# PKU-MARL/HARL

Hardware: NVIDIA B200
Metric: env-steps/sec (whole box) HAPPO update loop (higher is better)
Workload: dtype f32

## Files before the change

harl_b200/_lib.py:

```python
import ctypes as C
import os

HERE = os.path.dirname(os.path.abspath(__file__))
LIB_PATH = os.path.join(HERE, "_C", "libharl_b200.so")

HB_MAX_LAYERS = 4
HB_MAX_AGENTS = 32
HB_MAX_TENSORS = 40

ACTIVATIONS = {"relu": 0, "tanh": 1, "sigmoid": 2, "leaky_relu": 3, "selu": 4, "hardswish": 5, "identity": 6}
HEAD_DISCRETE, HEAD_BOX, HEAD_VALUE = 0, 1, 2


class NetDesc(C.Structure):
    _fields_ = [
        ("in_dim", C.c_int32), ("n_layers", C.c_int32), ("hidden", C.c_int32 * HB_MAX_LAYERS),
        ("feature_norm", C.c_int32), ("activation", C.c_int32), ("rnn_layers", C.c_int32),
        ("head", C.c_int32), ("out_dim", C.c_int32), ("std_x_coef", C.c_float), ("std_y_coef", C.c_float),
    ]


class NetLayout(C.Structure):
    _fields_ = [
        ("n_tensors", C.c_int32), ("total", C.c_int32),
        ("offset", C.c_int32 * HB_MAX_TENSORS), ("rows", C.c_int32 * HB_MAX_TENSORS),
        ("cols", C.c_int32 * HB_MAX_TENSORS), ("names", (C.c_char * 48) * HB_MAX_TENSORS),
        ("prepared_total", C.c_int32),
    ]


class InsertArgs(C.Structure):
    _fields_ = [
        ("n_envs", C.c_int32), ("n_agents", C.c_int32), ("state_type_fp", C.c_int32),
        ("actor_rnn_row", C.c_int32), ("critic_rnn_row", C.c_int32),
        ("dones", C.c_void_p), ("bad_transition", C.c_void_p),
        ("actor_masks_next", C.c_void_p * HB_MAX_AGENTS), ("actor_active_next", C.c_void_p * HB_MAX_AGENTS),
        ("actor_rnn_next", C.c_void_p * HB_MAX_AGENTS),
        ("critic_masks_next", C.c_void_p), ("critic_bad_next", C.c_void_p), ("critic_rnn_next", C.c_void_p),
        ("rewards", C.c_void_p), ("reward_stride_n", C.c_int64), ("reward_stride_a", C.c_int64),
        ("ep_return", C.c_void_p), ("done_sum", C.c_void_p),
    ]


class CollectArgs(C.Structure):
    _fields_ = [
        ("n_agents", C.c_int32), ("deterministic", C.c_int32), ("rows", C.c_int64), ("offset", C.c_uint64),
        ("actor_desc", C.POINTER(NetDesc) * HB_MAX_AGENTS), ("actor_prepared", C.c_void_p * HB_MAX_AGENTS),
        ("obs", C.c_void_p * HB_MAX_AGENTS), ("avail", C.c_void_p * HB_MAX_AGENTS),
        ("actions", C.c_void_p * HB_MAX_AGENTS), ("logp", C.c_void_p * HB_MAX_AGENTS),
        ("seed", C.c_uint64 * HB_MAX_AGENTS),
        ("critic_desc", C.POINTER(NetDesc)), ("critic_prepared", C.c_void_p), ("share_obs", C.c_void_p),
        ("critic_rows", C.c_int64), ("values", C.c_void_p), ("offset_base", C.c_void_p),
        ("actor_rnn", C.c_void_p * HB_MAX_AGENTS), ("actor_rnn_out", C.c_void_p * HB_MAX_AGENTS),
        ("actor_masks", C.c_void_p * HB_MAX_AGENTS),
        ("critic_rnn", C.c_void_p), ("critic_rnn_out", C.c_void_p), ("critic_masks", C.c_void_p),
    ]


class PPOHyper(C.Structure):
    _fields_ = [("clip_param", C.c_float), ("entropy_coef", C.c_float), ("use_policy_active_masks", C.c_int32),
                ("action_aggregation_prod", C.c_int32), ("use_clip", C.c_int32)]


class ActorBatch(C.Structure):
    _fields_ = [("obs", C.c_void_p), ("actions", C.c_void_p), ("old_logp", C.c_void_p), ("adv", C.c_void_p),
                ("factor", C.c_void_p), ("active", C.c_void_p), ("avail", C.c_void_p), ("index", C.c_void_p),
                ("rows", C.c_int64), ("rnn_states", C.c_void_p), ("masks", C.c_void_p), ("seq_len", C.c_int64)]


class ValueHyper(C.Structure):
    _fields_ = [("clip_param", C.c_float), ("huber_delta", C.c_float), ("value_loss_coef", C.c_float),
                ("use_huber_loss", C.c_int32), ("use_clipped_value_loss", C.c_int32)]


class CriticBatch(C.Structure):
    _fields_ = [("share_obs", C.c_void_p), ("value_preds", C.c_void_p), ("returns", C.c_void_p),
                ("index", C.c_void_p), ("rows", C.c_int64), ("rnn_states", C.c_void_p), ("masks", C.c_void_p),
                ("seq_len", C.c_int64)]


class AdamHyper(C.Structure):
    _fields_ = [("lr", C.c_float), ("beta1", C.c_float), ("beta2", C.c_float), ("eps", C.c_float),
                ("weight_decay", C.c_float), ("max_grad_norm", C.c_float), ("use_max_grad_norm", C.c_int32),
                ("step", C.c_int32)]


HB_MPE_MAX_AGENTS = 8


class CopySeg(C.Structure):
    _fields_ = [("dst", C.c_void_p), ("src", C.c_void_p), ("bytes", C.c_int64)]


def copy_segments(dsts, srcs, src_pinned=False, dst_pinned=False):
    n = len(dsts)
    if n == 0 or n > 16:
        return False
    segs = (CopySeg * n)()
    for i, (d, s) in enumerate(zip(dsts, srcs)):
        nbytes = d.numel() * d.element_size()
        if not ((d.is_cuda or dst_pinned or d.is_pinned()) and (s.is_cuda or src_pinned or s.is_pinned()) and (d.is_cuda or s.is_cuda)
                and d.is_contiguous() and s.is_contiguous() and d.dtype == s.dtype
                and d.numel() == s.numel() and nbytes % 4 == 0 and d.data_ptr() % 16 == 0 and s.data_ptr() % 16 == 0):
            return False
        segs[i].dst, segs[i].src, segs[i].bytes = d.data_ptr(), s.data_ptr(), nbytes
    call("hb_copy_segments", segs, n, stream_ptr())
    return True


class MpeArgs(C.Structure):
    _fields_ = [("n_envs", C.c_int32), ("n_agents", C.c_int32), ("n_landmarks", C.c_int32), ("continuous", C.c_int32),
                ("max_cycles", C.c_int32), ("reset_all", C.c_int32), ("seed", C.c_uint64),
                ("pos", C.c_void_p), ("vel", C.c_void_p), ("landmarks", C.c_void_p), ("step_count", C.c_void_p),
                ("episode", C.c_void_p), ("actions", C.c_void_p * HB_MPE_MAX_AGENTS),
                ("obs_out", C.c_void_p * HB_MPE_MAX_AGENTS), ("share_obs_out", C.c_void_p), ("rewards_out", C.c_void_p),
                ("rewards_na_out", C.c_void_p), ("dones_out", C.c_void_p), ("bad_out", C.c_void_p)]


P = C.c_void_p
SIGNATURES = {
    "hb_version": (C.c_int, []),
    "hb_last_error": (C.c_char_p, []),
    "hb_sync_check": (C.c_int, []),
    "hb_kernel_launch_count": (C.c_uint64, []),
    "hb_profile_begin": (C.c_int, [P]),
    "hb_profile_end": (C.c_int, [C.c_char_p, C.c_int]),
    "hb_set_gemm_impl": (C.c_int, [C.c_int]),
    "hb_get_gemm_impl": (C.c_int, []),
    "hb_set_fused_update": (C.c_int, [C.c_int]),
    "hb_get_fused_update": (C.c_int, []),
    "hb_fused_timing_enable": (C.c_int, [C.c_int]),
    "hb_fused_timing_read": (C.c_int, [P]),
    "hb_net_layout_of": (C.c_int, [C.POINTER(NetDesc), C.POINTER(NetLayout)]),
    "hb_net_prepare": (C.c_int, [C.POINTER(NetDesc), P, P, P]),
    "hb_workspace_bytes": (C.c_size_t, [C.POINTER(NetDesc), C.c_int64, C.c_int]),
    "hb_rollout_insert_masks": (C.c_int, [C.POINTER(InsertArgs), P]),
    "hb_rollout_collect": (C.c_int, [C.POINTER(CollectArgs), P, C.c_size_t, P]),
    "hb_counter_add": (C.c_int, [P, C.c_uint64, P]),
    "hb_policy_act": (C.c_int, [C.POINTER(NetDesc), P, P, C.c_int64, P, C.c_int, C.c_uint64, C.c_uint64, P, P, P,
                                C.c_size_t, P]),
    "hb_value_forward": (C.c_int, [C.POINTER(NetDesc), P, P, C.c_int64, P, P, C.c_size_t, P]),
    "hb_copy_segments": (C.c_int, [P, C.c_int32, P]),
    "hb_comm_create": (C.c_int, [C.c_int32, C.c_int32, C.c_size_t, C.POINTER(C.c_void_p), P]),
    "hb_comm_open_peers": (C.c_int, [P, P]),
    "hb_allreduce_bucket": (C.c_int, [P, P, C.c_int64, C.c_int32, P]),
    "hb_comm_status": (C.c_int, [P]),
    "hb_comm_destroy": (C.c_int, [P]),
    "hb_set_gae_impl": (C.c_int, [C.c_int]),
    "hb_get_gae_impl": (C.c_int, []),
    "hb_gae_returns": (C.c_int, [P, P, P, P, P, P, P, C.c_int32, C.c_int64, C.c_float, C.c_float, C.c_int, C.c_int,
                                 P, P]),
    "hb_masked_moments": (C.c_int, [P, P, C.c_int64, P, P]),
    "hb_normalize_by_moments": (C.c_int, [P, P, C.c_int64, P, P]),
    "hb_valuenorm_update": (C.c_int, [P, P, C.c_double, P]),
    "hb_valuenorm_apply": (C.c_int, [P, P, P, C.c_int64, C.c_int, P]),
    "hb_policy_evaluate": (C.c_int, [C.POINTER(NetDesc), P, C.POINTER(ActorBatch), P, P, P, C.c_int, P, C.c_size_t, P]),
    "hb_ppo_actor_grad": (C.c_int, [C.POINTER(NetDesc), P, P, C.POINTER(ActorBatch), C.POINTER(PPOHyper), P, P, P, P,
                                    C.c_size_t, P]),
    "hb_ppo_actor_grad_logp": (C.c_int, [C.POINTER(NetDesc), P, P, C.POINTER(ActorBatch), C.POINTER(PPOHyper), P, P, P, P, P,
                                         C.c_size_t, P]),
    "hb_value_grad": (C.c_int, [C.POINTER(NetDesc), P, P, C.POINTER(CriticBatch), C.POINTER(ValueHyper), P,
                                C.c_double, P, P, P, C.c_size_t, P]),
    "hb_clip_adam_step": (C.c_int, [C.POINTER(NetDesc), P, P, P, P, P, C.POINTER(AdamHyper), P, P]),
    "hb_policy_act_rnn": (C.c_int, [C.POINTER(NetDesc), P, P, C.c_int64, P, P, P, C.c_int, C.c_uint64, C.c_uint64, P, P, P,
                                    P, P, C.c_size_t, P]),
    "hb_value_forward_rnn": (C.c_int, [C.POINTER(NetDesc), P, P, C.c_int64, P, P, P, P, P, C.c_size_t, P]),
    "hb_set_trpo_jvp_impl": (C.c_int, [C.c_int]),
    "hb_get_trpo_jvp_impl": (C.c_int, []),
    "hb_set_rnn_impl": (C.c_int, [C.c_int]),
    "hb_get_rnn_impl": (C.c_int, []),
    "hb_trpo_workspace_bytes": (C.c_size_t, [C.POINTER(NetDesc), C.c_int64]),
    "hb_trpo_old_dist": (C.c_int, [C.POINTER(NetDesc), P, C.POINTER(ActorBatch), P, P, C.c_size_t, P]),
    "hb_trpo_fvp": (C.c_int, [C.POINTER(NetDesc), P, P, C.POINTER(ActorBatch), P, P, C.c_double, C.c_int, P, P,
                              C.c_size_t, P]),
    "hb_trpo_fvp_finish": (C.c_int, [C.POINTER(NetDesc), P, P, P, C.c_float, P]),
    "hb_trpo_eval": (C.c_int, [C.POINTER(NetDesc), P, C.POINTER(ActorBatch), C.POINTER(PPOHyper), P, P, P, P,
                               C.c_size_t, P]),
    "hb_trpo_cg_init": (C.c_int, [P, P, P, P, P, C.c_int, P]),
    "hb_trpo_cg_step": (C.c_int, [P, P, P, P, P, C.c_int, C.c_float, P]),
    "hb_trpo_full_step": (C.c_int, [P, P, P, C.c_float, P, P, C.c_int, P]),
    "hb_trpo_apply_step": (C.c_int, [P, P, P, C.c_float, C.c_int, P]),
    "hb_vec_scale": (C.c_int, [P, C.c_float, C.c_int, P]),
    "hb_mpe_spread_step": (C.c_int, [C.POINTER(MpeArgs), P]),
}

if not os.path.exists(LIB_PATH):
    raise ImportError(
        f"{LIB_PATH} is missing: build it with `python -m harl_b200.build` (or __graft_entry__.build()). "
        "harl_b200 has no CPU fallback.")

lib = C.CDLL(LIB_PATH)
for _name, (_res, _args) in SIGNATURES.items():
    _fn = getattr(lib, _name)
    _fn.restype = _res
    _fn.argtypes = _args

HB_ERR_UNSUPPORTED = -2
GEMM_IMPLS = {"fp32": 0, "3xtf32": 1}
if os.environ.get("HB_GEMM_IMPL"):
    lib.hb_set_gemm_impl(GEMM_IMPLS[os.environ["HB_GEMM_IMPL"]])
_NO_CHECK = {"hb_version", "hb_last_error", "hb_workspace_bytes", "hb_trpo_workspace_bytes", "hb_kernel_launch_count", "hb_profile_end", "hb_get_gemm_impl", "hb_get_rnn_impl", "hb_get_trpo_jvp_impl", "hb_get_fused_update", "hb_get_gae_impl", "hb_comm_status"}

call_count = 0


def check(rc, what=""):
    if rc == 0:
        return
    msg = lib.hb_last_error().decode(errors="replace")
    if rc == HB_ERR_UNSUPPORTED:
        raise NotImplementedError(f"harl_b200 {what}: {msg}")
    raise RuntimeError(f"harl_b200 {what} failed ({rc}): {msg}")


def call(name, *args):
    global call_count
    call_count += 1
    check(getattr(lib, name)(*args), name)


def ptr(t):
    if t is None:
        return None
    assert t.is_contiguous(), "harl_b200 kernels need contiguous tensors"
    return t.data_ptr()


def stream_ptr():
    import torch

    return torch.cuda.current_stream().cuda_stream
```

harl_b200/algorithms/actors/happo.py:

```python
import torch

from ... import _lib as L
from ... import dist
from ...common import seq_index
from ...nets import DeviceNet
from .on_policy_base import OnPolicyBase, to_device


class HAPPO(OnPolicyBase):
    use_clip = True

    def __init__(self, args, obs_space, act_space, device=torch.device("cpu")):
        super().__init__(args, obs_space, act_space, device)
        self.clip_param = args["clip_param"]
        self.ppo_epoch = args.get("ppo_epoch", args.get("a2c_epoch"))
        self.actor_num_mini_batch = args["actor_num_mini_batch"]
        self.entropy_coef = args["entropy_coef"]
        self.use_max_grad_norm = args["use_max_grad_norm"]
        self.max_grad_norm = args["max_grad_norm"]

    first_epoch_logp = True

    def _hyper(self):
        return L.PPOHyper(float(self.clip_param), float(self.entropy_coef), int(bool(self.use_policy_active_masks)),
                          int(self.action_aggregation == "prod"), int(self.use_clip))

    def _step(self, batch, norm3, scalars_row, logp_out=None):
        hooks = getattr(self, "grad_hooks", None)
        if hooks is not None:
            hooks[0]()
        self.actor.actor_grad(batch, self._hyper(), norm3, scalars_row, logp_out)
        if hooks is not None:
            hooks[1]()
        dist.all_reduce_sum_(self.actor.grad)
        self.actor.adam_step(self.cur_lr, self.opti_eps, self.weight_decay, self.max_grad_norm, self.use_max_grad_norm)

    def update(self, sample):
        (obs, _rnn, actions, _masks, active, old_lp, adv, avail, factor) = sample
        d = self.device
        obs, actions, active, old_lp, adv, factor, avail = (to_device(x, d) for x in
                                                             (obs, actions, active, old_lp, adv, factor, avail))
        rnn = mk = None
        seq_len = 0
        if self.recurrent:
            rnn = to_device(_rnn, d)
            rnn = rnn.reshape(rnn.shape[0], -1)
            mk = to_device(_masks, d).reshape(-1)
            seq_len = obs.shape[0] // rnn.shape[0]
        batch = DeviceNet.actor_batch(obs, actions, old_lp, adv.reshape(-1), factor.reshape(-1), active.reshape(-1), avail,
                                      rnn_states=rnn, masks=mk, seq_len=seq_len)
        norm3 = torch.zeros(3, dtype=torch.float64, device=d)
        norm3[2] = active.sum().double() if self.use_policy_active_masks else float(obs.shape[0])
        dist.all_reduce_sum_(norm3)
        scal = torch.zeros(4, dtype=torch.float64, device=d)
        self._step(batch, norm3, scal)
        dist.all_reduce_sum_(scal)
        s, n = scal.cpu().numpy(), norm3[2].item()
        return s[0] / n, s[1] / n, self.actor.grad_norm.item(), s[2] / s[3]

    def train(self, actor_buffer, advantages, state_type, moments=None, old_logp_out=None):
        self.old_logp_filled = False
        info = dict(policy_loss=0.0, dist_entropy=0.0, actor_grad_norm=0.0, ratio=0.0)
        d = self.device
        buf = actor_buffer
        T, N = buf.actions.shape[:2]
        rows = T * N
        adv = to_device(advantages, d).reshape(rows)
        active = buf.active_masks[:-1].reshape(rows)
        if moments is not None:
            m3, n_active = moments
        else:
            m3 = torch.zeros(3, dtype=torch.float64, device=d)
            L.call("hb_masked_moments", L.ptr(adv), L.ptr(active), rows, L.ptr(m3), L.stream_ptr())
            dist.all_reduce_sum_(m3)
            n_active = m3[2].item()
        if n_active == 0:
            return info
        if state_type == "EP":
            adv_n = torch.empty_like(adv)
            L.call("hb_normalize_by_moments", L.ptr(adv), L.ptr(adv_n), rows, L.ptr(m3), L.stream_ptr())
            adv = adv_n
        nmb = self.actor_num_mini_batch
        n_up = self.ppo_epoch * nmb
        scal = torch.zeros(n_up, 4, dtype=torch.float64, device=d)
        gnorm = torch.zeros(n_up, dtype=torch.float32, device=d)
        norms = torch.zeros(n_up, 3, dtype=torch.float64, device=d)
        fl = lambda a: a.reshape(rows, *a.shape[2:])
        obs, actions, old_lp = fl(buf.obs[:-1]), fl(buf.actions), fl(buf.action_log_probs)
        avail = None if buf.available_actions is None else fl(buf.available_actions[:-1])
        factor = None if buf.factor is None else buf.factor.reshape(rows)
        rnn = buf.rnn_states.reshape((T + 1) * N, -1) if self.recurrent else None
        masks = buf.masks.reshape((T + 1) * N) if self.recurrent else None
        mode = seq_index.mode_of(self.use_recurrent_policy, self.use_naive_recurrent_policy)
        world = dist.world_size()
        u = 0
        for _ in range(self.ppo_epoch):
            for idx, nrows, seq_len in seq_index.minibatches(T, N, nmb, mode, self.data_chunk_length, d):
                if idx is None or nrows == rows:
                    norms[u, 2] = n_active if self.use_policy_active_masks else float(rows * world)
                else:
                    if self.use_policy_active_masks:
                        norms[u, 2] = active[idx.long()].sum().double()
                    else:
                        norms[u, 2] = float(nrows)
                    dist.all_reduce_sum_(norms[u])
                batch = DeviceNet.actor_batch(obs, actions, old_lp, adv, factor, active, avail, idx, nrows,
                                              rnn_states=rnn, masks=masks, seq_len=seq_len)
                first = u == 0 and old_logp_out is not None and (idx is None) and nrows == rows
                self._step(batch, norms[u], scal[u], old_logp_out if first else None)
                self.old_logp_filled = self.old_logp_filled or first
                gnorm[u] = self.actor.grad_norm[0]
                u += 1
        dist.all_reduce_sum_(scal)
        s = scal.cpu().numpy()
        nr = norms[:, 2].cpu().numpy()
        info["policy_loss"] = float((s[:, 0] / nr).mean())
        info["dist_entropy"] = float((s[:, 1] / nr).mean())
        info["ratio"] = float((s[:, 2] / s[:, 3]).mean())
        info["actor_grad_norm"] = float(gnorm.mean().item())
        return info
```

harl_b200/algorithms/critics/v_critic.py:

```python
import torch

from ... import _lib as L
from ... import dist
from ...common import seq_index
from ...nets import DeviceNet
from ...utils.envs_tools import get_shape_from_obs_space
from ...utils.models_tools import linear_schedule_lr
from ..actors.on_policy_base import to_device


class VCritic:
    def __init__(self, args, cent_obs_space, device=torch.device("cpu")):
        self.args = args
        self.device = torch.device(device)
        self.tpdv = dict(dtype=torch.float32, device=self.device)
        self.clip_param = args["clip_param"]
        self.critic_epoch = args["critic_epoch"]
        self.critic_num_mini_batch = args["critic_num_mini_batch"]
        self.data_chunk_length = args["data_chunk_length"]
        self.value_loss_coef = args["value_loss_coef"]
        self.max_grad_norm = args["max_grad_norm"]
        self.huber_delta = args["huber_delta"]
        self.use_recurrent_policy = args["use_recurrent_policy"]
        self.use_naive_recurrent_policy = args["use_naive_recurrent_policy"]
        self.use_max_grad_norm = args["use_max_grad_norm"]
        self.use_clipped_value_loss = args["use_clipped_value_loss"]
        self.use_huber_loss = args["use_huber_loss"]
        self.use_policy_active_masks = args["use_policy_active_masks"]
        self.critic_lr = args["critic_lr"]
        self.opti_eps = args["opti_eps"]
        self.weight_decay = args["weight_decay"]
        self.share_obs_space = cent_obs_space
        shp = get_shape_from_obs_space(cent_obs_space)
        if len(shp) == 3:
            raise NotImplementedError("CNN state trunks are outside the B200 hot path")
        self.critic = DeviceNet(args, shp[0], L.HEAD_VALUE, 1, self.device)
        self.cur_lr = self.critic_lr

    def lr_decay(self, episode, episodes):
        self.cur_lr = linear_schedule_lr(episode, episodes, self.critic_lr)

    @property
    def recurrent(self):
        return bool(self.use_recurrent_policy or self.use_naive_recurrent_policy)

    def get_values(self, cent_obs, rnn_states_critic, masks, values_out=None, rnn_out=None):
        x = to_device(cent_obs, self.device)
        v = values_out if values_out is not None else torch.empty(x.shape[0], 1, **self.tpdv)
        if self.recurrent:
            rnn_in = to_device(rnn_states_critic, self.device)
            mk = to_device(masks, self.device).reshape(x.shape[0])
            rnn_new = rnn_out if rnn_out is not None else torch.empty_like(rnn_in)
            self.critic.values(x, v, rnn_in, mk, rnn_new)
            return v, rnn_new
        self.critic.values(x, v)
        rnn = rnn_states_critic if torch.is_tensor(rnn_states_critic) else to_device(rnn_states_critic, self.device)
        return v, rnn

    def _hyper(self):
        return L.ValueHyper(float(self.clip_param), float(self.huber_delta), float(self.value_loss_coef),
                            int(bool(self.use_huber_loss)), int(bool(self.use_clipped_value_loss)))

    def _step(self, share_obs, value_preds, returns, index, rows, global_rows, value_normalizer, scalars_row,
              rnn_states=None, masks=None, seq_len=0, whole=None):
        d = self.device
        if value_normalizer is not None:
            m3 = whole.get("m3") if whole is not None and index is None else None
            if m3 is None:
                m3 = torch.zeros(3, dtype=torch.float64, device=d)
                src = returns if index is None else returns[index.long()]
                L.call("hb_masked_moments", L.ptr(src.contiguous()), None, rows, L.ptr(m3), L.stream_ptr())
                dist.all_reduce_sum_(m3)
                if whole is not None and index is None:
                    whole["m3"] = m3
            value_normalizer.update_from_moments(m3)
        cb = DeviceNet.critic_batch(share_obs, value_preds, returns, index, rows, rnn_states, masks, seq_len)
        vn = value_normalizer.state if value_normalizer is not None else None
        self.critic.value_grad(cb, self._hyper(), vn, 1.0 / global_rows, scalars_row)
        if getattr(self, "after_grad_hook", None) is not None:
            self.after_grad_hook()
        dist.all_reduce_sum_(self.critic.grad)
        self.critic.adam_step(self.cur_lr, self.opti_eps, self.weight_decay, self.max_grad_norm, self.use_max_grad_norm)

    def update(self, sample, value_normalizer=None):
        share_obs, _rnn, value_preds, returns, _masks = sample
        d = self.device
        so, vp, rt = (to_device(x, d) for x in (share_obs, value_preds, returns))
        rows = so.shape[0]
        scal = torch.zeros(4, dtype=torch.float64, device=d)
        rnn = mk = None
        seq_len = 0
        if self.recurrent:
            rnn = to_device(_rnn, d)
            rnn = rnn.reshape(rnn.shape[0], -1)
            mk = to_device(_masks, d).reshape(-1)
            seq_len = rows // rnn.shape[0]
        self._step(so, vp.reshape(-1), rt.reshape(-1), None, rows, float(rows * dist.world_size()), value_normalizer, scal,
                   rnn, mk, seq_len)
        dist.all_reduce_sum_(scal)
        s = scal.cpu().numpy()
        return s[0] / s[1], self.critic.grad_norm.item()

    def train_steps(self, critic_buffer, value_normalizer=None):
        d = self.device
        buf = critic_buffer
        T = buf.episode_length
        rows = buf.value_preds[:-1].numel()
        Cn = rows // T
        so = buf.share_obs[:-1].reshape(rows, -1)
        vp = buf.value_preds[:-1].reshape(rows)
        rt = buf.returns[:-1].reshape(rows)
        rnn = buf.rnn_states_critic.reshape((T + 1) * Cn, -1) if self.recurrent else None
        masks = buf.masks.reshape((T + 1) * Cn) if self.recurrent else None
        mode = seq_index.mode_of(self.use_recurrent_policy, self.use_naive_recurrent_policy)
        nmb = self.critic_num_mini_batch
        n_up = self.critic_epoch * nmb
        scal = torch.zeros(n_up, 4, dtype=torch.float64, device=d)
        gnorm = torch.zeros(n_up, dtype=torch.float32, device=d)
        u = 0
        whole = {}
        for _ in range(self.critic_epoch):
            for idx, n, seq_len in seq_index.minibatches(T, Cn, nmb, mode, self.data_chunk_length, d):
                self._step(so, vp, rt, idx, n, float(n * dist.world_size()), value_normalizer, scal[u], rnn, masks, seq_len, whole)
                gnorm[u] = self.critic.grad_norm[0]
                u += 1
                yield u
        dist.all_reduce_sum_(scal)

        def finish():
            s = scal.cpu().numpy()
            return dict(value_loss=float((s[:, 0] / s[:, 1]).mean()), critic_grad_norm=float(gnorm.mean().item()))

        self.finish_train = finish

    def train(self, critic_buffer, value_normalizer=None, defer=False):
        for _ in self.train_steps(critic_buffer, value_normalizer):
            pass
        return self.finish_train if defer else self.finish_train()

    def prep_training(self):
        pass

    def prep_rollout(self):
        pass
```

harl_b200/csrc/capi.cu:

```cuda
#include <stdlib.h>

#include <atomic>

#include "common.cuh"
#include "kernels.cuh"
#include "rnn.cuh"
#include "trpo.cuh"

#include "fused_args.cuh"

namespace hb {

constexpr int64_t CHUNK_ROWS = (int64_t)1 << 20;

struct Work {
  float* x0;
  float* Z[HB_MAX_LAYERS];
  float* Y[HB_MAX_LAYERS];
  float* stats[HB_MAX_LAYERS];
  float* dA;
  float* dB;
  float* dwpart;
  int ptotal;
  RnnWork rnn;
// ... 148 lines not shown

static void head_base(const hb_net_desc* d, const PrepLayout& Q, const float* prep, HeadArgs* a) {
  memset(a, 0, sizeof(*a));
  a->h = Q.n[Q.n_layers - 1];
  a->out = d->out_dim;
  a->hw = prep + Q.hw;
  a->hbias = prep + Q.hbias;
  a->log_std = prep + Q.log_std;
  a->std_x = d->std_x_coef;
  a->std_y = d->std_y_coef;
}

static void head_batch(const hb_net_desc* d, const hb_actor_batch* b, int64_t c0, int64_t rows, HeadArgs* a) {
  const int ad = d->head == HB_HEAD_DISCRETE ? 1 : d->out_dim;
  const int64_t o = b->index ? 0 : c0;
  a->rows = rows;
  a->index = b->index ? b->index + c0 : nullptr;
  a->actions = b->actions ? b->actions + o * ad : nullptr;
  a->avail = b->avail ? b->avail + o * d->out_dim : nullptr;
  a->old_logp = b->old_logp ? b->old_logp + o * ad : nullptr;
  a->adv = b->adv ? b->adv + o : nullptr;
  a->factor = b->factor ? b->factor + o : nullptr;
  a->active = b->active ? b->active + o : nullptr;
}

}

extern "C" {

size_t hb_workspace_bytes(const hb_net_desc* d, int64_t rows, int mode) {
  hb::PrepLayout Q;
  hb::ParamLayout P;
  if (hb::make_layouts(d, &P, &Q, nullptr)) return 0;
  const int64_t ch = hb::chunk_of(d, rows);
  return hb::work_floats(Q, ch, mode, P.total) * sizeof(float);
}

static int policy_act_impl(const hb_net_desc* d, const float* prepared, const float* obs, int64_t rows,
                           const float* avail, const float* h_in, const float* masks, int deterministic, uint64_t seed,
                           uint64_t offset, const uint64_t* offset_base, float* actions, float* logp, float* h_out,
                           void* ws, size_t ws_bytes, void* stream) {
  using namespace hb;
  HB_CHECK_ARG(prepared && obs && actions && logp && rows >= 0, "bad argument");
  PrepLayout Q;
  int rc = check_net(d, nullptr, &Q, nullptr, 1);
  if (rc) return rc;
  HB_CHECK_ARG(!d->rnn_layers || (h_in && masks && h_out), "recurrent policy: rnn_states, masks and rnn_states_out are required");
  cudaStream_t st = (cudaStream_t)stream;
  const int64_t ch = chunk_of(d, rows);
  if (rows == 0) return HB_OK;
  if (!d->rnn_layers && fused_enabled()) {
    fz::ActArgs F;
    memset(&F, 0, sizeof(F));
    bool ok = false;
    if ((rc = fused_act_fill(&F.net[0], d, prepared, obs, avail, actions, logp, seed, rows, &ok))) return rc;
    if (ok) {
      F.n_nets = 1; F.H = d->hidden[0]; F.act = d->activation; F.deterministic = deterministic;
      F.offset = offset; F.offset_base = reinterpret_cast<const unsigned long long*>(offset_base);
      return launch_fused_act(F, st);
    }
  }
  Work w;
  if ((rc = carve(Q, ch, 0, ws, ws_bytes, &w))) return rc;
  const int ad = d->head == HB_HEAD_DISCRETE ? 1 : d->out_dim;
  for (int64_t c0 = 0; c0 < rows; c0 += ch) {
    const int64_t n = rows - c0 < ch ? rows - c0 : ch;
    SeqCtx seq = {h_in, masks, 1, h_out};
    const float* feat = nullptr;
    if ((rc = features_forward(d, Q, prepared, obs, nullptr, c0, n, d->rnn_layers ? &seq : nullptr, w, st, &feat))) return rc;
    HeadArgs a;
    head_base(d, Q, prepared, &a);
    a.feat = feat;
    a.rows = n;
    a.avail = avail ? avail + c0 * d->out_dim : nullptr;
    a.deterministic = deterministic;
    a.seed = seed;
    a.offset = offset + (uint64_t)c0 * 0x9E3779B97F4A7C15ull;
    a.offset_base = reinterpret_cast<const unsigned long long*>(offset_base);
    a.actions_out = actions + c0 * ad;
    a.logp_out = logp + c0 * ad;
    if ((rc = launch_policy_head(d->head, MODE_ACT, a, st))) return rc;
  }
  return HB_OK;
}

static int value_forward_impl(const hb_net_desc* d, const float* prepared, const float* cent_obs, int64_t rows,
                              const float* h_in, const float* masks, float* values, float* h_out, void* ws,
                              size_t ws_bytes, void* stream) {
  using namespace hb;
  HB_CHECK_ARG(prepared && cent_obs && values && rows >= 0, "bad argument");
  PrepLayout Q;
  int rc = check_net(d, nullptr, &Q, nullptr, 0);
  if (rc) return rc;
  HB_CHECK_ARG(!d->rnn_layers || (h_in && masks && h_out), "recurrent critic: rnn_states, masks and rnn_states_out are required");
  cudaStream_t st = (cudaStream_t)stream;
  if (rows == 0) return HB_OK;
  if (!d->rnn_layers && fused_enabled()) {
    fz::ActArgs F;
    memset(&F, 0, sizeof(F));
    bool ok = false;
    if ((rc = fused_act_fill(&F.net[0], d, prepared, cent_obs, nullptr, values, nullptr, 0ull, rows, &ok))) return rc;
    if (ok) {
      F.n_nets = 1; F.H = d->hidden[0]; F.act = d->activation;
      return launch_fused_act(F, st);
    }
  }
  const int64_t ch = chunk_of(d, rows);
  Work w;
  if ((rc = carve(Q, ch, 0, ws, ws_bytes, &w))) return rc;
  for (int64_t c0 = 0; c0 < rows; c0 += ch) {
    const int64_t n = rows - c0 < ch ? rows - c0 : ch;
    SeqCtx seq = {h_in, masks, 1, h_out};
    const float* feat = nullptr;
    if ((rc = features_forward(d, Q, prepared, cent_obs, nullptr, c0, n, d->rnn_layers ? &seq : nullptr, w, st, &feat))) return rc;
    ValueArgs a;
    memset(&a, 0, sizeof(a));
    a.feat = feat;
    a.h = Q.n[Q.n_layers - 1];
    a.hw = prepared + Q.hw;
    a.hbias = prepared + Q.hbias;
    a.rows = n;
    a.values_out = values + c0;
    if ((rc = launch_value_head(0, a, st))) return rc;
  }
  return HB_OK;
}

int hb_policy_act(const hb_net_desc* d, const float* prepared, const float* obs, int64_t rows, const float* avail,
                  int deterministic, uint64_t seed, uint64_t offset, float* actions, float* logp, void* ws,
                  size_t ws_bytes, void* stream) {
  return policy_act_impl(d, prepared, obs, rows, avail, nullptr, nullptr, deterministic, seed, offset, nullptr, actions,
                         logp, nullptr, ws, ws_bytes, stream);
}

int hb_policy_act_rnn(const hb_net_desc* d, const float* prepared, const float* obs, int64_t rows, const float* avail,
                      const float* rnn_states, const float* masks, int deterministic, uint64_t seed, uint64_t offset,
                      const uint64_t* offset_base, float* actions, float* logp, float* rnn_states_out, void* ws,
                      size_t ws_bytes, void* stream) {
  return policy_act_impl(d, prepared, obs, rows, avail, rnn_states, masks, deterministic, seed, offset, offset_base, actions,
                         logp, rnn_states_out, ws, ws_bytes, stream);
}

int hb_value_forward(const hb_net_desc* d, const float* prepared, const float* cent_obs, int64_t rows, float* values,
                     void* ws, size_t ws_bytes, void* stream) {
  return value_forward_impl(d, prepared, cent_obs, rows, nullptr, nullptr, values, nullptr, ws, ws_bytes, stream);
}

int hb_value_forward_rnn(const hb_net_desc* d, const float* prepared, const float* cent_obs, int64_t rows,
                         const float* rnn_states, const float* masks, float* values, float* rnn_states_out, void* ws,
                         size_t ws_bytes, void* stream) {
  return value_forward_impl(d, prepared, cent_obs, rows, rnn_states, masks, values, rnn_states_out, ws, ws_bytes, stream);
}

int hb_policy_evaluate(const hb_net_desc* d, const float* prepared, const hb_actor_batch* b, float* logp_out,
                       const float* logp_ref, float* factor_inout, int action_aggregation_prod, void* ws,
                       size_t ws_bytes, void* stream) {
  using namespace hb;
  HB_CHECK_ARG(prepared && b && b->obs && b->actions && b->rows >= 0, "bad argument");
  HB_CHECK_ARG(!factor_inout || (logp_ref && !b->index), "factor update needs logp_ref and an identity batch");
  PrepLayout Q;
  int rc = check_net(d, nullptr, &Q, nullptr, 1);
  if (rc) return rc;
  cudaStream_t st = (cudaStream_t)stream;
  const int64_t rows = b->rows;
  if (rows == 0) return HB_OK;
  if (Q.fz_ok && fused_enabled()) {
    ParamLayout P;
    if ((rc = make_layouts(d, &P, nullptr, nullptr))) return rc;
    fz::Args fa;
    memset(&fa, 0, sizeof(fa));
    fa.obs = b->obs; fa.index = b->index; fa.rows = rows;
    fa.actions = b->actions; fa.avail = b->avail;
    fa.logp_out = logp_out; fa.logp_ref = logp_ref; fa.factor_inout = factor_inout;
    fa.agg_prod = action_aggregation_prod;
    return launch_fused_update(d, Q, P, prepared, fa, 1, nullptr, st);
  }
  const int64_t ch = chunk_of(d, rows);
  Work w;
  if ((rc = carve(Q, ch, 0, ws, ws_bytes, &w))) return rc;
  const int ad = d->head == HB_HEAD_DISCRETE ? 1 : d->out_dim;
  for (int64_t c0 = 0; c0 < rows; c0 += ch) {
    const int64_t n = rows - c0 < ch ? rows - c0 : ch;
    SeqCtx seq = {b->rnn_states, b->masks, b->seq_len, nullptr};
    const float* feat = nullptr;
    if ((rc = features_forward(d, Q, prepared, b->obs, b->index, c0, n, d->rnn_layers ? &seq : nullptr, w, st, &feat))) return rc;
    HeadArgs a;
    head_base(d, Q, prepared, &a);
    head_batch(d, b, c0, n, &a);
    a.feat = feat;
    a.logp_out = logp_out ? logp_out + c0 * ad : nullptr;
    a.logp_ref = logp_ref ? logp_ref + c0 * ad : nullptr;
    a.factor_inout = factor_inout ? factor_inout + c0 : nullptr;
    a.agg_prod = action_aggregation_prod;
    if ((rc = launch_policy_head(d->head, MODE_EVAL, a, st))) return rc;
  }
  return HB_OK;
}

int hb_ppo_actor_grad(const hb_net_desc* d, const float* params, const float* prepared, const hb_actor_batch* b,
                      const hb_ppo_hyper* h, const double* norm3, float* grad, double* scalars, void* ws,
                      size_t ws_bytes, void* stream) {
  return hb_ppo_actor_grad_logp(d, params, prepared, b, h, norm3, grad, scalars, nullptr, ws, ws_bytes, stream);
}

int hb_ppo_actor_grad_logp(const hb_net_desc* d, const float* params, const float* prepared, const hb_actor_batch* b,
                           const hb_ppo_hyper* h, const double* norm3, float* grad, double* scalars, float* logp_out, void* ws,
                           size_t ws_bytes, void* stream) {
  using namespace hb;
  HB_CHECK_ARG(params && prepared && b && h && norm3 && grad && scalars, "NULL argument");
  HB_CHECK_ARG(b->obs && b->actions && b->old_logp && b->adv && b->active && b->rows >= 0, "incomplete batch");
  HB_CHECK_ARG(!logp_out || !b->index, "logp_out needs an identity batch (rows of the batch = rows of logp_out)");
  ParamLayout P;
  PrepLayout Q;
  hb_net_layout L;
  int rc = check_net(d, &P, &Q, &L, 1);
  if (rc) return rc;
  cudaStream_t st = (cudaStream_t)stream;
  if (Q.fz_ok && fused_enabled() && b->rows > 0) {
    const size_t need = (size_t)fused_max_slots() * L.total * sizeof(float);
    if (ws == nullptr || ws_bytes < need) { set_error("hb_ppo_actor_grad: workspace too small: need %zu bytes, have %zu", need, ws_bytes); return HB_ERR_WORKSPACE; }
    fz::Args fa;
    memset(&fa, 0, sizeof(fa));
    fa.obs = b->obs; fa.index = b->index; fa.rows = b->rows;
    fa.actions = b->actions; fa.avail = b->avail; fa.old_logp = b->old_logp; fa.adv = b->adv; fa.factor = b->factor; fa.active = b->active;
    fa.clip = h->clip_param; fa.entropy_coef = h->entropy_coef; fa.use_active = h->use_policy_active_masks;
    fa.use_clip = h->use_clip; fa.agg_prod = h->action_aggregation_prod;
    fa.part = (float*)ws; fa.part_stride = L.total; fa.scalars = scalars;
    fa.logp_out = logp_out;
    int slots = 0;
    if ((rc = launch_fused_update(d, Q, P, prepared, fa, 0, &slots, st))) return rc;
    return launch_fused_finish(d, P, params, grad, (const float*)ws, slots, L.total, norm3, 1.0, st);
  }
  if (logp_out && b->rows > 0) {
    rc = hb_policy_evaluate(d, prepared, b, logp_out, nullptr, nullptr, h->action_aggregation_prod, ws, ws_bytes, stream);
    if (rc) return rc;
  }
  cudaError_t ce = cudaMemsetAsync(grad, 0, (size_t)L.total * sizeof(float), st);
  if (ce != cudaSuccess) return cuda_fail(ce, "hb_ppo_actor_grad(memset)");
  const int64_t rows = b->rows;
  if (rows == 0) return HB_OK;
  const int64_t ch = chunk_of(d, rows);
  Work w;
  if ((rc = carve(Q, ch, 1, ws, ws_bytes, &w, L.total))) return rc;
  {
    ce = cudaMemsetAsync(w.dwpart, 0, (size_t)tc_dw_splits() * L.total * sizeof(float), st);
    if (ce != cudaSuccess) return cuda_fail(ce, "hb_ppo_actor_grad(memset split buffer)");
  }
  const bool rnn = d->rnn_layers != 0;
  for (int64_t c0 = 0; c0 < rows; c0 += ch) {
    const int64_t n = rows - c0 < ch ? rows - c0 : ch;
    SeqCtx seq = {b->rnn_states, b->masks, b->seq_len, nullptr};
    const float* feat = nullptr;
    if ((rc = features_forward(d, Q, prepared, b->obs, b->index, c0, n, rnn ? &seq : nullptr, w, st, &feat))) return rc;
    HeadArgs a;
    head_base(d, Q, prepared, &a);
    head_batch(d, b, c0, n, &a);
    a.feat = feat;
    a.agg_prod = h->action_aggregation_prod;
    a.clip = h->clip_param;
    a.entropy_coef = h->entropy_coef;
    a.use_active = h->use_policy_active_masks;
    a.use_clip = h->use_clip;
    a.norm3 = norm3;
    a.dfeat = w.dA;
    a.g_hw = grad + P.hw;
    a.g_hbias = grad + P.hbias;
    a.g_log_std = d->head == HB_HEAD_BOX ? grad + P.log_std : nullptr;
    a.scalars = scalars;
    a.ln_z = w.Z[Q.n_layers - 1]; a.ln_stats = w.stats[Q.n_layers - 1]; a.ln_w = prepared + Q.lnw[Q.n_layers - 1];
    a.g_ln_w = grad + P.lnw[Q.n_layers - 1]; a.g_ln_b = grad + P.lnb[Q.n_layers - 1]; a.ln_act = d->activation;
    if (rnn) {
      a.dfeat = w.rnn.dtop;
      a.ln_z = w.rnn.hs[d->rnn_layers - 1]; a.ln_stats = w.rnn.stats; a.ln_w = prepared + Q.rnn_lnw;
      a.g_ln_w = grad + P.rnn_lnw; a.g_ln_b = grad + P.rnn_lnb; a.ln_act = HB_ACT_IDENTITY;
    }
    a.part_delta = w.dwpart - grad; a.part_stride = w.ptotal;
    if ((rc = launch_policy_head(d->head, MODE_GRAD, a, st))) return rc;
    if (rnn && (rc = rnn_to_trunk_backward(d, P, Q, params, prepared, grad, n, &seq, w, st))) return rc;
    if ((rc = trunk_backward(d, P, Q, params, prepared, grad, n, w, st))) return rc;
  }
  if ((rc = launch_dw_reduce(grad, w.dwpart, L.total, st))) return rc;
  return launch_featnorm_fold(d, params, grad, st);
}

int hb_value_grad(const hb_net_desc* d, const float* params, const float* prepared, const hb_critic_batch* b,
                  const hb_value_hyper* h, const float* vn_state, double inv_count, float* grad, double* scalars,
                  void* ws, size_t ws_bytes, void* stream) {
  using namespace hb;
  HB_CHECK_ARG(params && prepared && b && h && grad && scalars, "NULL argument");
  HB_CHECK_ARG(b->share_obs && b->value_preds && b->returns && b->rows >= 0, "incomplete batch");
  ParamLayout P;
  PrepLayout Q;
  hb_net_layout L;
  int rc = check_net(d, &P, &Q, &L, 0);
  if (rc) return rc;
  cudaStream_t st = (cudaStream_t)stream;
  if (Q.fz_ok && fused_enabled() && b->rows > 0) {
    const size_t need = (size_t)fused_max_slots() * L.total * sizeof(float);
    if (ws == nullptr || ws_bytes < need) { set_error("hb_value_grad: workspace too small: need %zu bytes, have %zu", need, ws_bytes); return HB_ERR_WORKSPACE; }
    fz::Args fa;
    memset(&fa, 0, sizeof(fa));
    fa.obs = b->share_obs; fa.index = b->index; fa.rows = b->rows;
    fa.value_preds = b->value_preds; fa.returns = b->returns; fa.vn_state = vn_state;
    fa.clip = h->clip_param; fa.huber_delta = h->huber_delta; fa.vcoef = h->value_loss_coef;
    fa.use_huber = h->use_huber_loss; fa.use_clipped = h->use_clipped_value_loss;
    fa.part = (float*)ws; fa.part_stride = L.total; fa.scalars = scalars;
    int slots = 0;
    if ((rc = launch_fused_update(d, Q, P, prepared, fa, 0, &slots, st))) return rc;
    return launch_fused_finish(d, P, params, grad, (const float*)ws, slots, L.total, nullptr, inv_count, st);
  }
  cudaError_t ce = cudaMemsetAsync(grad, 0, (size_t)L.total * sizeof(float), st);
  if (ce != cudaSuccess) return cuda_fail(ce, "hb_value_grad(memset)");
  const int64_t rows = b->rows;
  if (rows == 0) return HB_OK;
  const int64_t ch = chunk_of(d, rows);
  Work w;
  if ((rc = carve(Q, ch, 1, ws, ws_bytes, &w, L.total))) return rc;
  {
    ce = cudaMemsetAsync(w.dwpart, 0, (size_t)tc_dw_splits() * L.total * sizeof(float), st);
    if (ce != cudaSuccess) return cuda_fail(ce, "hb_value_grad(memset split buffer)");
  }
  const bool rnn = d->rnn_layers != 0;
  for (int64_t c0 = 0; c0 < rows; c0 += ch) {
    const int64_t n = rows - c0 < ch ? rows - c0 : ch;
    SeqCtx seq = {b->rnn_states, b->masks, b->seq_len, nullptr};
    const float* feat = nullptr;
    if ((rc = features_forward(d, Q, prepared, b->share_obs, b->index, c0, n, rnn ? &seq : nullptr, w, st, &feat))) return rc;
    ValueArgs a;
    memset(&a, 0, sizeof(a));
    a.feat = feat;
    a.h = Q.n[Q.n_layers - 1];
    a.hw = prepared + Q.hw;
    a.hbias = prepared + Q.hbias;
    a.rows = n;
    const int64_t o = b->index ? 0 : c0;
    a.index = b->index ? b->index + c0 : nullptr;
    a.value_preds = b->value_preds + o;
    a.returns = b->returns + o;
    a.vn_state = vn_state;
    a.clip = h->clip_param;
    a.huber_delta = h->huber_delta;
    a.coef = (float)((double)h->value_loss_coef * inv_count);
    a.use_huber = h->use_huber_loss;
    a.use_clipped = h->use_clipped_value_loss;
    a.dfeat = w.dA;
    a.g_hw = grad + P.hw;
    a.g_hbias = grad + P.hbias;
    a.scalars = scalars;
    a.ln_z = w.Z[Q.n_layers - 1]; a.ln_stats = w.stats[Q.n_layers - 1]; a.ln_w = prepared + Q.lnw[Q.n_layers - 1];
    a.g_ln_w = grad + P.lnw[Q.n_layers - 1]; a.g_ln_b = grad + P.lnb[Q.n_layers - 1]; a.ln_act = d->activation;
    if (rnn) {
      a.dfeat = w.rnn.dtop;
      a.ln_z = w.rnn.hs[d->rnn_layers - 1]; a.ln_stats = w.rnn.stats; a.ln_w = prepared + Q.rnn_lnw;
      a.g_ln_w = grad + P.rnn_lnw; a.g_ln_b = grad + P.rnn_lnb; a.ln_act = HB_ACT_IDENTITY;
    }
    a.part_delta = w.dwpart - grad; a.part_stride = w.ptotal;
    if ((rc = launch_value_head(1, a, st))) return rc;
    if (rnn && (rc = rnn_to_trunk_backward(d, P, Q, params, prepared, grad, n, &seq, w, st))) return rc;
    if ((rc = trunk_backward(d, P, Q, params, prepared, grad, n, w, st))) return rc;
  }
  if ((rc = launch_dw_reduce(grad, w.dwpart, L.total, st))) return rc;
  return launch_featnorm_fold(d, params, grad, st);
}

namespace {
struct TrpoExtra { float* tprep; float* yd[2]; float* ttiles; };

size_t trpo_extra_floats(const hb::PrepLayout& Q, int64_t ch) {
  return (size_t)hb::round_up(Q.tk[0], 4) + 2 * (size_t)ch * hb::hmax_of(Q) + hb::rnn_jvp_floats(Q, ch) +
         (size_t)hb::round_up(Q.total - Q.tk[0], 4);
}

int trpo_jvp_default() {
  const char* e = getenv("HB_TRPO_JVP_IMPL");
  return e ? (atoi(e) != 0) : 1;
}
std::atomic<int> g_trpo_jvp_impl{trpo_jvp_default()};


}

size_t hb_trpo_workspace_bytes(const hb_net_desc* d, int64_t rows) {
  hb::PrepLayout Q;
  hb::ParamLayout P;
  if (hb::make_layouts(d, &P, &Q, nullptr)) return 0;
  const int64_t ch = hb::chunk_of(d, rows);
  return (hb::work_floats(Q, ch, 1, P.total) + trpo_extra_floats(Q, ch)) * sizeof(float);
}

int hb_trpo_old_dist(const hb_net_desc* d, const float* prepared, const hb_actor_batch* b, float* old_dist, void* ws,
                     size_t ws_bytes, void* stream) {
  using namespace hb;
  HB_CHECK_ARG(prepared && b && b->obs && old_dist && b->rows >= 0, "bad argument");
  PrepLayout Q;
  int rc = check_net(d, nullptr, &Q, nullptr, 1);
  if (rc) return rc;
  cudaStream_t st = (cudaStream_t)stream;
  const int64_t rows = b->rows;
  if (rows == 0) return HB_OK;
  const int64_t ch = chunk_of(d, rows);
  Work w;
  if ((rc = carve(Q, ch, 0, ws, ws_bytes, &w))) return rc;
  for (int64_t c0 = 0; c0 < rows; c0 += ch) {
    const int64_t n = rows - c0 < ch ? rows - c0 : ch;
    SeqCtx seq = {b->rnn_states, b->masks, b->seq_len, nullptr};
    const float* feat = nullptr;
    if ((rc = features_forward(d, Q, prepared, b->obs, b->index, c0, n, d->rnn_layers ? &seq : nullptr, w, st, &feat))) return rc;
    TrpoHeadArgs a;
    memset(&a, 0, sizeof(a));
    a.feat = feat;
    a.h = Q.n[Q.n_layers - 1]; a.out = d->out_dim;
    a.hw = prepared + Q.hw; a.hbias = prepared + Q.hbias; a.log_std = prepared + Q.log_std;
    a.std_x = d->std_x_coef; a.std_y = d->std_y_coef;
    a.rows = n;
    a.index = b->index ? b->index + c0 : nullptr;
    a.avail = b->avail ? b->avail + (b->index ? 0 : c0) * d->out_dim : nullptr;
    a.old_dist_out = old_dist + c0 * d->out_dim;
    if ((rc = launch_trpo_head(d->head, TR_OLD, a, st))) return rc;
  }
  return HB_OK;
}

int hb_trpo_fvp(const hb_net_desc* d, const float* params, const float* prepared, const hb_actor_batch* b,
                const float* old_dist, const float* v, double inv_rows, int reuse_forward, float* out, void* ws,
                size_t ws_bytes, void* stream) {
  using namespace hb;
  HB_CHECK_ARG(params && prepared && b && b->obs && old_dist && v && out && b->rows >= 0, "bad argument");
  ParamLayout P;
  PrepLayout Q;
  hb_net_layout L;
  int rc = check_net(d, &P, &Q, &L, 1);
  if (rc) return rc;
  cudaStream_t st = (cudaStream_t)stream;
  cudaError_t ce = cudaMemsetAsync(out, 0, (size_t)L.total * sizeof(float), st);
  if (ce != cudaSuccess) return cuda_fail(ce, "hb_trpo_fvp(memset)");
  const int64_t rows = b->rows;
  if (rows == 0) return HB_OK;
  const int64_t ch = chunk_of(d, rows);
  const bool rnn = d->rnn_layers != 0;
  const size_t base = work_floats(Q, ch, 1, L.total);
  if ((base + trpo_extra_floats(Q, ch)) * sizeof(float) > ws_bytes || ws == nullptr) {
    set_error("hb_trpo_fvp: workspace too small: need %zu bytes, have %zu", (base + trpo_extra_floats(Q, ch)) * sizeof(float), ws_bytes);
    return HB_ERR_WORKSPACE;
  }
  Work w;
  if ((rc = carve(Q, ch, 1, ws, base * sizeof(float), &w, L.total))) return rc;
  TrpoExtra x;
  x.tprep = (float*)ws + base;
  x.yd[0] = x.tprep + round_up(Q.tk[0], 4);
  x.yd[1] = x.yd[0] + (size_t)ch * hmax_of(Q);
  RnnJvpWork jw;
  carve_rnn_jvp(Q, ch, x.yd[1] + (size_t)ch * hmax_of(Q), &jw);
  x.ttiles = x.yd[1] + (size_t)ch * hmax_of(Q) + rnn_jvp_floats(Q, ch);
  const bool tc_jvp = g_trpo_jvp_impl.load(std::memory_order_relaxed) == 1 && gemm_impl() != 0;
  ce = cudaMemsetAsync(w.dwpart, 0, (size_t)tc_dw_splits() * L.total * sizeof(float), st);
// ... 183 lines not shown
```

harl_b200/csrc/fused_args.cuh:

```cuda
#pragma once
#include <cuda_fp16.h>

#include "common.cuh"

namespace hb {
namespace fz {

struct Args {
  int H, K0p, in_dim, out, act, nch0;
  const __half* img0; const __half* img1; const __half* img1b; const __half* imgh;
  const float* bias0; const float* bias1; const float* biash;
  const float* scales;
  const float* log_std; float std_x, std_y;
  const float* obs; const int32_t* index; long long rows;
  int stage_obs;
  const float* actions; const float* avail; const float* old_logp; const float* adv; const float* factor; const float* active;
  const float* value_preds; const float* returns; const float* vn_state;
  float clip, entropy_coef, huber_delta, vcoef;
  int use_active, use_clip, agg_prod, use_huber, use_clipped;
  float* part; long long part_stride;
  int pw0, pb0, pw1, pb1, phw, phb, plogstd;
  double* scalars;
  float* logp_out; const float* logp_ref; float* factor_inout;
};

constexpr int ACT_MAX_NETS = 24;
struct ActNet {
  const float* prep; const float* obs; const float* avail;
  float* out0;
  float* out1;
  unsigned long long seed;
  long long rows;
  int in_dim, out, head, K0p, nch0;
  int o_w0, o_w1, o_hw, o_b0, o_b1, o_bh, o_sc, o_ls;
  float std_x, std_y;
  int tile0, stage;
};
struct ActArgs {
  int n_nets, H, act, deterministic, K0p_max, pad_;
  unsigned long long offset;
  const unsigned long long* offset_base;
  ActNet net[ACT_MAX_NETS];
};

}

bool fused_enabled();
struct hb_collect_args;
int launch_fused_act(fz::ActArgs& A, cudaStream_t st);
int fused_act_fill(fz::ActNet* n, const hb_net_desc* d, const float* prepared, const float* obs, const float* avail, float* out0,
                   float* out1, unsigned long long seed, long long rows, bool* ok);
void set_fused_enabled(int on);
inline int fused_max_slots() { return 148; }
int launch_fused_update(const hb_net_desc* d, const PrepLayout& Q, const ParamLayout& P, const float* prepared, fz::Args a, int mode,
                        int* grid_out, cudaStream_t st);
int launch_fused_finish(const hb_net_desc* d, const ParamLayout& P, const float* params, float* grad, const float* part, int slots,
                        long long stride, const double* norm3, double host_scale, cudaStream_t st);

int fused_timing_enable(int on);
int fused_timing_read(unsigned long long* out);

}
```

harl_b200/csrc/fused_update.cu:

```cuda
#include <cuda_fp16.h>

#include <atomic>

#include "common.cuh"
#include "head_rows.cuh"
#include "kernels.cuh"
#include "row_helpers.cuh"
#include "fused_args.cuh"
#include "umma.cuh"

namespace hb {

int launch_featnorm_fold_at(const float* params, float* grad, int w0, int b0, int gw, int gb, int N, int K, cudaStream_t st);

namespace fz {

constexpr float XS = 16.f;
constexpr float DZS = 16.f;
constexpr int TILE = 128;
constexpr int NH = 16;
constexpr int MAX_STAGES = 3;
constexpr int STAGE_BYTES = 16384;
constexpr int THREADS = 320;
enum { M_GRAD = 0, M_EVAL = 1 };
// ... 39 lines not shown
  const int A_ = ACT >= 0 ? ACT : act_rt;
  switch (A_) {
    case HB_ACT_RELU: return zpos ? 1.f : 0.f;
    case HB_ACT_TANH: return 1.f - a * a;
    case HB_ACT_SIGMOID: return a * (1.f - a);
    case HB_ACT_LEAKY_RELU: return zpos ? 1.f : 0.01f;
    case HB_ACT_SELU: {
      const float al = 1.6732632423543772848170429916717f, s = 1.0507009873554804934193349852946f;
      return zpos ? s : a + s * al;
    }
    default: return 1.f;
  }
}
template <int ACT>
__device__ __forceinline__ float act_f(int act_rt, float z) {
  if (ACT >= 0) return act_fwd<(ACT >= 0 ? ACT : 0)>(z);
  return act_fwd_rt(act_rt, z);
}

struct RowPair {
  float* xch;
  int half, r, bar_id;
  __device__ __forceinline__ void put(int slot, float v) const { xch[(half * TILE + r) * 2 + slot] = v; }
  __device__ __forceinline__ void sync() const { asm volatile("bar.sync %0, 64;" ::"r"(bar_id) : "memory"); }
  __device__ __forceinline__ float total(int slot, float mine) const {
    const float other = xch[((half ^ 1) * TILE + r) * 2 + slot];
    return half == 0 ? mine + other : other + mine;
  }
};


struct NoMid { __device__ __forceinline__ void operator()() const {} };
template <int ACT, typename Mid = NoMid>
__device__ __forceinline__ void fwd_epilogue(int act_rt, uint32_t tacc, int H, const float* __restrict__ sbias, float descale,
                                             unsigned char* img, uint32_t img_bytes, int wch, const RowPair& P, float& mu, float& rstd,
                                             uint32_t (&mask)[2], Mid mid = Mid()) {
  const int r = P.r, nc = H >> 1, cb = P.half * nc;
  const float inv_n = 1.f / (float)H;
  uint32_t va[16], vb[16];
  float s0 = 0.f, s1 = 0.f, q0 = 0.f, q1 = 0.f;
  uint32_t mk0 = 0u, mk1 = 0u;
  um::tmem_ld16_issue(tacc + cb, va);
#define HB_STEP(CC, CUR, NXT)                                                                              \
  if ((CC) * 16 < nc) {                                                                                    \
    um::tmem_ld_wait16(CUR);                                                                               \
    if (((CC) + 1) * 16 < nc) um::tmem_ld16_issue(tacc + cb + ((CC) + 1) * 16, NXT);                      \
    uint32_t m_ = 0u;                                                                                      \
    _Pragma("unroll") for (int q = 0; q < 2; ++q) {                                                        \
      const float4 ba = *reinterpret_cast<const float4*>(sbias + cb + (CC) * 16 + q * 8);                  \
      const float4 bb = *reinterpret_cast<const float4*>(sbias + cb + (CC) * 16 + q * 8 + 4);              \
      const float bq[8] = {ba.x, ba.y, ba.z, ba.w, bb.x, bb.y, bb.z, bb.w};                                \
      float x[8];                                                                                          \
      _Pragma("unroll") for (int j = 0; j < 8; ++j) {                                                      \
        const float z = fmaf(__uint_as_float(CUR[q * 8 + j]), descale, bq[j]);                             \
        m_ |= z > 0.f ? (1u << (q * 8 + j)) : 0u;                                                          \
        x[j] = act_f<ACT>(act_rt, z);                                                                      \
      }                                                                                                    \
      _Pragma("unroll") for (int j = 0; j < 8; j += 2) {                                                   \
        s0 += x[j]; s1 += x[j + 1];                                                                        \
        q0 = fmaf(x[j], x[j], q0); q1 = fmaf(x[j + 1], x[j + 1], q1);                                      \
      }                                                                                                    \
      uint4 hi, lo;                                                                                        \
      um::split8(x, hi, lo);                                                                               \
      const uint32_t off = img_off(r, (cb >> 3) + (CC) * 2 + q, wch);                                      \
      *reinterpret_cast<uint4*>(img + off) = hi;                                                           \
      *reinterpret_cast<uint4*>(img + img_bytes + off) = lo;                                               \
    }                                                                                                      \
    if ((CC) < 2) mk0 |= m_ << (16 * ((CC) & 1)); else mk1 |= m_ << (16 * ((CC) & 1));                     \
  }
  HB_STEP(0, va, vb) HB_STEP(1, vb, va) HB_STEP(2, va, vb) HB_STEP(3, vb, va)
#undef HB_STEP
  mask[0] = mk0; mask[1] = mk1;
  const float ps = s0 + s1, pq = q0 + q1;
  P.put(0, ps);
  P.put(1, pq);
  P.sync();
  mu = P.total(0, ps) * inv_n;
  rstd = rsqrtf(fmaxf(P.total(1, pq) * inv_n - mu * mu, 0.f) + 1e-5f);
  const float rs = rstd * XS, sh = -mu * rstd * XS;
  for (int c8 = 0; c8 < (nc >> 3); ++c8) {
    const uint32_t off = img_off(r, (cb >> 3) + c8, wch);
    float x[8];
    um::join8(*reinterpret_cast<const uint4*>(img + off), *reinterpret_cast<const uint4*>(img + img_bytes + off), x);
#pragma unroll
    for (int j = 0; j < 8; ++j) x[j] = fmaf(x[j], rs, sh);
    uint4 hi, lo;
    um::split8(x, hi, lo);
    *reinterpret_cast<uint4*>(img + off) = hi;
    *reinterpret_cast<uint4*>(img + img_bytes + off) = lo;
    if (c8 == (nc >> 4) - 1) mid();
  }
}

template <int ACT, typename Pre>
__device__ __forceinline__ void bwd_epilogue(int act_rt, uint32_t tacc, int H, float descale, unsigned char* img,
                                             uint32_t img_bytes, int wch, const RowPair& P, float mu, float rstd,
                                             const uint32_t (&mask)[2], bool row_ok, Pre pre) {
  const int r = P.r, nc = H >> 1, cb = P.half * nc;
  const float inv_n = 1.f / (float)H;
  float s1a = 0.f, s1b = 0.f, s2a = 0.f, s2b = 0.f;
  {
    uint32_t va[16], vb[16];
    um::tmem_ld16_issue(tacc + cb, va);
#define HB_STEP(CC, CUR, NXT)                                                                              \
    if ((CC) * 16 < nc) {                                                                                  \
      um::tmem_ld_wait16(CUR);                                                                             \
      if (((CC) + 1) * 16 < nc) um::tmem_ld16_issue(tacc + cb + ((CC) + 1) * 16, NXT);                    \
      _Pragma("unroll") for (int q = 0; q < 2; ++q) {                                                      \
        const uint32_t off = img_off(r, (cb >> 3) + (CC) * 2 + q, wch);                                    \
        float x[8];                                                                                        \
        um::join8(*reinterpret_cast<const uint4*>(img + off), *reinterpret_cast<const uint4*>(img + img_bytes + off), x); \
        _Pragma("unroll") for (int j = 0; j < 8; j += 2) {                                                 \
          const float g0 = __uint_as_float(CUR[q * 8 + j]), g1 = __uint_as_float(CUR[q * 8 + j + 1]);      \
          s1a += g0; s1b += g1;                                                                            \
          s2a = fmaf(g0, x[j], s2a); s2b = fmaf(g1, x[j + 1], s2b);                                        \
        }                                                                                                  \
      }                                                                                                    \
    }
    HB_STEP(0, va, vb) HB_STEP(1, vb, va) HB_STEP(2, va, vb) HB_STEP(3, vb, va)
#undef HB_STEP
  }
  const float p1 = s1a + s1b, p2 = s2a + s2b;
  P.put(0, p1);
  P.put(1, p2);
  P.sync();
  const float m1 = P.total(0, p1) * inv_n, m2 = P.total(1, p2) * inv_n * (1.f / (XS * XS));
  const float stdx = 1.f / (rstd * XS);
  const float k = row_ok ? rstd * descale * DZS : 0.f;
  pre();
  for (int cc = 0; cc * 16 < nc; ++cc) {
    uint32_t v[16];
    um::tmem_ld16_issue(tacc + cb + cc * 16, v);
    um::tmem_ld_wait16(v);
    const uint32_t mw = (cc < 2 ? mask[0] : mask[1]) >> (16 * (cc & 1));
#pragma unroll
    for (int q = 0; q < 2; ++q) {
      const uint32_t off = img_off(r, (cb >> 3) + cc * 2 + q, wch);
      float x[8], dz[8];
      um::join8(*reinterpret_cast<const uint4*>(img + off), *reinterpret_cast<const uint4*>(img + img_bytes + off), x);
#pragma unroll
      for (int j = 0; j < 8; ++j) {
        const float a = fmaf(x[j], stdx, mu);
        const float t = fmaf(-x[j], m2, __uint_as_float(v[q * 8 + j]) - m1);
        dz[j] = k * t * act_prime<ACT>(act_rt, a, (mw >> (q * 8 + j)) & 1u);
      }
      uint4 hi, lo;
      um::split8(dz, hi, lo);
      *reinterpret_cast<uint4*>(img + off) = hi;
      *reinterpret_cast<uint4*>(img + img_bytes + off) = lo;
    }
  }
}

__device__ __forceinline__ float huber_v(float e, float d, int use_huber, float* de) {
  if (!use_huber) { *de = e; return e * e / 2.f; }
  const float ae = fabsf(e);
  if (ae <= d) { *de = e; return e * e / 2.f; }
  *de = e > 0.f ? d : -d;
  return d * (ae - d / 2.f);
}

__device__ unsigned long long g_phase_cycles[148 * 16];
__device__ int g_phase_on;
struct PhaseClock {
  unsigned long long t;
  unsigned long long* acc;
  bool on;
  __device__ __forceinline__ void start(bool enable, unsigned long long* smem_acc) {
    on = enable; acc = smem_acc;
    if (on) { for (int i = 0; i < 16; ++i) acc[i] = 0ull; t = clock64(); }
  }
  __device__ __forceinline__ void lap(int slot) {
    if (on) { const unsigned long long n = clock64(); acc[slot] += n - t; t = n; }
  }
  __device__ __forceinline__ void flush() {
    if (on) for (int i = 0; i < 16; ++i) g_phase_cycles[blockIdx.x * 16 + i] += acc[i];
  }
};

template <int HEAD, int MODE, int ACT>
__global__ void __launch_bounds__(THREADS, 1) fused_update_kernel(const __grid_constant__ Args a) {
  extern __shared__ __align__(1024) unsigned char smem[];
  const int tid = threadIdx.x, warp = tid >> 5, lane = tid & 31;
  const int H = a.H, K0p = a.K0p;
  const int wch0 = K0p >> 3, wchx = 16, wchd = NH >> 3, wchh = H >> 3;
  const uint32_t x0_bytes = TILE * K0p * 2, x_bytes = TILE * 128 * 2, dl_bytes = TILE * NH * 2, wh_bytes = NH * H * 2;
  unsigned char* p = smem;
  unsigned char* X0 = p; p += 2 * x0_bytes;
  unsigned char* X1 = p; p += 2 * x_bytes;
  unsigned char* X2 = p; p += 2 * x_bytes;
  unsigned char* DL = p; p += 2 * dl_bytes;
  unsigned char* ONES = p; p += dl_bytes;
  unsigned char* WH = p; p += 2 * wh_bytes;
  const int STAGES = K0p <= 32 ? 3 : 2;
  unsigned char* ring = p; p += STAGES * STAGE_BYTES;
  float* sb0 = reinterpret_cast<float*>(p); p += 128 * 4;
  float* sb1 = reinterpret_cast<float*>(p); p += 128 * 4;
  float* sbh = reinterpret_cast<float*>(p); p += NH * 4;
  float* sstd = reinterpret_cast<float*>(p); p += 4 * NH * 4;
  float* sacc = reinterpret_cast<float*>(p); p += 2 * NH * 4;
  double* sred = reinterpret_cast<double*>(p); p += 4 * 4 * 8;
  float* xch = reinterpret_cast<float*>(p); p += 2 * TILE * 2 * 4;
  uint64_t* bars = reinterpret_cast<uint64_t*>(p); p += 12 * 8;
  unsigned long long* sclk = reinterpret_cast<unsigned long long*>(p); p += 16 * 8;
  uint32_t* tmem_slot = reinterpret_cast<uint32_t*>(p);
  uint64_t* w_full = bars;
  uint64_t* w_empty = bars + MAX_STAGES;
  uint64_t* e2m = bars + 2 * MAX_STAGES;
  uint64_t* m2e = e2m + 1;
  uint64_t* obs_free = e2m + 2;
  uint64_t* obs_full = e2m + 3;
  uint64_t* e2m_h = e2m + 4;
  uint64_t* m2e_b = e2m + 5;
  unsigned char* OBS = MODE == M_GRAD ? X2 : X1;
  const uint32_t obs_bytes = (uint32_t)TILE * (uint32_t)a.in_dim * 4u;
  const int aw = HEAD == HB_HEAD_BOX ? a.out : 1;
  uint32_t so = obs_bytes, o_act = 0, o_old = 0, o_adv = 0, o_fac = 0, o_w = 0, o_av = 0, o_vp = 0, o_ret = 0;
  if (HEAD != HB_HEAD_VALUE) {
    o_act = so; so += TILE * aw * 4;
    if (MODE == M_GRAD) {
      o_old = so; so += TILE * aw * 4;
      o_adv = so; so += TILE * 4;
      if (a.factor) { o_fac = so; so += TILE * 4; }
      if (a.use_active) { o_w = so; so += TILE * 4; }
    }
    if (HEAD == HB_HEAD_DISCRETE && a.avail != nullptr) { o_av = so; so += TILE * a.out * 4; }
  } else if (MODE == M_GRAD) {
    o_vp = so; so += TILE * 4;
    o_ret = so; so += TILE * 4;
  }
  const uint32_t stage_bytes = so;

  const long long ntiles = (a.rows + TILE - 1) / TILE;
  const int nch1 = H >> 5;
  constexpr bool GRAD = MODE == M_GRAD;

  if (H < 128) {
    for (int i = tid; i < (int)((2 * x_bytes) / 16); i += THREADS) {
      reinterpret_cast<uint4*>(X1)[i] = make_uint4(0, 0, 0, 0);
      reinterpret_cast<uint4*>(X2)[i] = make_uint4(0, 0, 0, 0);
    }
  }
  for (int i = tid; i < TILE * 2; i += THREADS)
    reinterpret_cast<uint4*>(ONES)[i] = ((i >> 3) & 1) ? make_uint4(0, 0, 0, 0) : make_uint4(0x00003C00u, 0, 0, 0);
  for (int i = tid; i < (int)((2 * wh_bytes) / 16); i += THREADS) reinterpret_cast<uint4*>(WH)[i] = reinterpret_cast<const uint4*>(a.imgh)[i];
  for (int i = tid; i < 128; i += THREADS) { sb0[i] = i < H ? a.bias0[i] : 0.f; sb1[i] = i < H ? a.bias1[i] : 0.f; }
  if (tid < NH) {
    sbh[tid] = a.biash[tid];
    sacc[tid] = sacc[NH + tid] = 0.f;
    float sd = 1.f, ls = 0.f, dsd = 0.f;
    if (HEAD == HB_HEAD_BOX && tid < a.out) {
      const float sig = 1.f / (1.f + expf(-a.log_std[tid] / a.std_x));
      sd = sig * a.std_y;
      ls = logf(sd);
      dsd = a.std_y * sig * (1.f - sig) / a.std_x;
    }
    sstd[tid] = sd; sstd[NH + tid] = ls; sstd[2 * NH + tid] = dsd; sstd[3 * NH + tid] = 1.f / (sd * sd);
  }
  if (tid < 16) sred[tid] = 0.0;
  if (tid == 0) {
    for (int i = 0; i < STAGES; ++i) { um::mbar_init(&w_full[i], 1); um::mbar_init(&w_empty[i], 1); }
    um::mbar_init(e2m, 8);
    um::mbar_init(e2m_h, 8);
    um::mbar_init(m2e_b, 1);
    um::mbar_init(m2e, 1);
    um::mbar_init(obs_free, 1);
    um::mbar_init(obs_full, 1);
    um::fence_mbarrier_init();
  }
  if (warp == 0) um::tmem_alloc(tmem_slot, TMEM_COLS);
  um::fence_async_smem();
  um::tc_fence_before();
  __syncthreads();
  um::tc_fence_after();
  const uint32_t tmem = *tmem_slot;
  const float ws0 = a.scales[0], ws1 = a.scales[1], wsh = a.scales[2];

  if (warp == 0) {
    if (lane == 0) {
      uint32_t it = 0, tl_ = 0;
      auto staged = [&](long long t) { return a.stage_obs && t < ntiles && (t + 1) * TILE <= a.rows; };
      auto load_obs = [&](long long t) {
        um::mbar_expect_tx(obs_full, stage_bytes);
        um::tma_bulk_g2s(OBS, a.obs + t * TILE * a.in_dim, obs_bytes, obs_full);
        const long long r0 = t * TILE;
        if (o_act) um::tma_bulk_g2s(OBS + o_act, a.actions + r0 * aw, TILE * aw * 4, obs_full);
        if (o_old) um::tma_bulk_g2s(OBS + o_old, a.old_logp + r0 * aw, TILE * aw * 4, obs_full);
        if (o_adv) um::tma_bulk_g2s(OBS + o_adv, a.adv + r0, TILE * 4, obs_full);
        if (o_fac) um::tma_bulk_g2s(OBS + o_fac, a.factor + r0, TILE * 4, obs_full);
        if (o_w) um::tma_bulk_g2s(OBS + o_w, a.active + r0, TILE * 4, obs_full);
        if (o_av) um::tma_bulk_g2s(OBS + o_av, a.avail + r0 * a.out, TILE * a.out * 4, obs_full);
        if (o_vp) um::tma_bulk_g2s(OBS + o_vp, a.value_preds + r0, TILE * 4, obs_full);
        if (o_ret) um::tma_bulk_g2s(OBS + o_ret, a.returns + r0, TILE * 4, obs_full);
      };
      if (staged(blockIdx.x)) load_obs(blockIdx.x);
      for (long long t = blockIdx.x; t < ntiles; t += gridDim.x, ++tl_) {
        for (int pass = 0; pass < (GRAD ? 3 : 2); ++pass) {
          const int layer = pass == 0 ? 0 : 1;
          const int nch = layer == 0 ? a.nch0 : nch1, kp = layer == 0 ? K0p : H;
          const unsigned char* src = reinterpret_cast<const unsigned char*>(pass == 0 ? a.img0 : (pass == 1 ? a.img1 : a.img1b));
          for (int ci = 0; ci < nch; ++ci, ++it) {
            const int c = (pass == 1 && nch == 4) ? ((ci & 1) * 2 + (ci >> 1)) : ci;
            const int kc = kp - 32 * c < 32 ? kp - 32 * c : 32;
            const uint32_t bytes = 2u * (uint32_t)H * (uint32_t)kc * 2u;
            const uint32_t st = it % STAGES, use = it / STAGES;
            if (use > 0) um::mbar_wait(&w_empty[st], (use - 1) & 1);
            um::mbar_expect_tx(&w_full[st], bytes);
            um::tma_bulk_g2s(ring + st * STAGE_BYTES, src + (size_t)c * (2u * H * 32u * 2u), bytes, &w_full[st]);
          }
        }
        um::mbar_wait(obs_free, tl_ & 1);
        if (staged(t + gridDim.x)) load_obs(t + gridDim.x);
      }
    }
    __syncwarp();
  } else if (warp == 1) {
    if (lane == 0) {
      uint32_t it = 0, pe = 0, peh = 0;
      bool first = true;
      const uint32_t X0a = um::smem_u32(X0), X1a = um::smem_u32(X1), X2a = um::smem_u32(X2), DLa = um::smem_u32(DL);
      const uint32_t ONa = um::smem_u32(ONES), WHa = um::smem_u32(WH), RGa = um::smem_u32(ring);
      for (long long t = blockIdx.x; t < ntiles; t += gridDim.x) {
        auto wait_e = [&]() { um::mbar_wait(e2m, pe); pe ^= 1; um::tc_fence_after(); };
        auto wait_eh = [&]() { um::mbar_wait(e2m_h, peh); peh ^= 1; um::tc_fence_after(); };
        auto chunk = [&](int kc, auto&& body) {
          const uint32_t st = it % STAGES, use = it / STAGES;
          um::mbar_wait(&w_full[st], use & 1);
          um::tc_fence_after();
          body(RGa + st * STAGE_BYTES, (uint32_t)H * (uint32_t)kc * 2u);
          um::commit(&w_empty[st]);
          ++it;
        };
        wait_e();
        for (int c = 0; c < a.nch0; ++c) {
          const int kc = K0p - 32 * c < 32 ? K0p - 32 * c : 32;
          chunk(kc, [&](uint32_t wb, uint32_t wimg) {
            gemm3(tmem + C_F, op_kmajor(X0a, x0_bytes, wch0, 4 * c), op_kmajor(wb, wimg, kc >> 3, 0), kc >> 4,
                  um::idesc_f16(H, 0, 0), c > 0);
          });
        }
        um::commit(m2e);
        wait_eh();
        if (nch1 == 4) {
          auto l1 = [&](int c, bool acc) {
            chunk(32, [&](uint32_t wb, uint32_t wimg) {
              gemm3(tmem + C_F, op_kmajor(X1a, x_bytes, wchx, 4 * c), op_kmajor(wb, wimg, 4, 0), 2, um::idesc_f16(H, 0, 0), acc);
            });
          };
          l1(0, false); l1(2, true);
          wait_e();
          l1(1, true); l1(3, true);
        } else {
          wait_e();
          for (int c = 0; c < nch1; ++c)
            chunk(32, [&](uint32_t wb, uint32_t wimg) {
              gemm3(tmem + C_F, op_kmajor(X1a, x_bytes, wchx, 4 * c), op_kmajor(wb, wimg, 4, 0), 2, um::idesc_f16(H, 0, 0), c > 0);
            });
        }
        um::commit(m2e);
        if (!GRAD) um::commit(obs_free);
        wait_eh();
        if (H == 128) {
          auto hd = [&](int q, bool acc) {
            gemm3(tmem + C_H, op_kmajor(X2a, x_bytes, wchx, 4 * q), op_kmajor(WHa, wh_bytes, wchh, 4 * q), 2, um::idesc_f16(NH, 0, 0), acc);
          };
          hd(0, false); hd(2, true);
          wait_e();
          hd(1, true); hd(3, true);
        } else {
          wait_e();
          gemm3(tmem + C_H, op_kmajor(X2a, x_bytes, wchx, 0), op_kmajor(WHa, wh_bytes, wchh, 0), H >> 4, um::idesc_f16(NH, 0, 0), false);
        }
        um::commit(m2e);
        if (GRAD) {
          wait_e();
          gemm3(tmem + C_F, op_kmajor(DLa, dl_bytes, wchd, 0), op_mnmajor(WHa, wh_bytes, wchh, 0), 1, um::idesc_f16(H, 0, 1), false);
          um::commit(m2e);
          gemm3(tmem + C_WH, op_mnmajor(X2a, x_bytes, wchx, 0), op_mnmajor(DLa, dl_bytes, wchd, 0), TILE >> 4,
                um::idesc_f16(NH, 1, 1), !first);
          gemm3(tmem + C_BH, op_mnmajor(DLa, dl_bytes, wchd, 0), op_mnmajor(ONa, dl_bytes, wchd, 0), TILE >> 4,
                um::idesc_f16(NH, 1, 1), !first, false);
          um::commit(m2e_b);
          wait_e();
          auto dx_chunk = [&](int c) {
            chunk(32, [&](uint32_t wb, uint32_t wimg) {
              gemm3(tmem + C_F, op_kmajor(X2a, x_bytes, wchx, 4 * c), op_mnmajor(wb, wimg, H >> 3, 0), 2,
                    um::idesc_f16(H, 0, 1), c > 0);
            });
          };
          const int nres = nch1 < STAGES ? nch1 : STAGES;
          for (int c = 0; c < nres; ++c) dx_chunk(c);
          gemm3(tmem + C_B1, op_mnmajor(X2a, x_bytes, wchx, 0), op_mnmajor(ONa, dl_bytes, wchd, 0), TILE >> 4,
                um::idesc_f16(NH, 1, 1), !first, false);
          for (int c = nres; c < nch1; ++c) dx_chunk(c);
          um::commit(m2e);
          gemm3(tmem + C_W1, op_mnmajor(X2a, x_bytes, wchx, 0), op_mnmajor(X1a, x_bytes, wchx, 0), TILE >> 4,
                um::idesc_f16(H, 1, 1), !first);
          um::commit(m2e_b);
          um::commit(obs_free);
          wait_e();
          gemm3(tmem + C_W0, op_mnmajor(X1a, x_bytes, wchx, 0), op_mnmajor(X0a, x0_bytes, wch0, 0), TILE >> 4,
                um::idesc_f16(K0p, 1, 1), !first);
          gemm3(tmem + C_B0, op_mnmajor(X1a, x_bytes, wchx, 0), op_mnmajor(ONa, dl_bytes, wchd, 0), TILE >> 4,
                um::idesc_f16(NH, 1, 1), !first, false);
          um::commit(m2e);
          first = false;
        }
      }
    }
    __syncwarp();
  } else {
    const int q = warp & 3, r = q * 32 + lane, half = (warp - 2) >> 2;
    const uint32_t tl = tmem + ((uint32_t)(q * 32) << 16);
    const RowPair RP{xch, half, r, 2 + q};
    uint32_t pm = 0, po = 0;
    auto wait_m = [&]() { um::mbar_wait(m2e, pm); pm ^= 1; um::tc_fence_after(); };
    auto signal = [&]() { um::fence_async_smem(); um::tc_fence_before(); __syncwarp(); if (lane == 0) um::mbar_arrive(e2m); };
    auto mid = [&]() { um::fence_async_smem(); um::tc_fence_before(); __syncwarp(); if (lane == 0) um::mbar_arrive(e2m_h); };
    uint32_t pmb = 0;
    auto wait_mb = [&]() { um::mbar_wait(m2e_b, pmb); pmb ^= 1; um::tc_fence_after(); };
    const int na = a.out;
    float s_loss = 0.f, s_ent = 0.f, s_ratio = 0.f, s_rows = 0.f;
    float vmean = 0.f, vstd = 1.f;
    if (HEAD == HB_HEAD_VALUE && a.vn_state != nullptr) {
      const float d = fmaxf(a.vn_state[2], 1e-5f);
      const float mu = a.vn_state[0] / d, msq = a.vn_state[1] / d;
      vmean = mu;
      vstd = sqrtf(fmaxf(msq - mu * mu, 1e-2f));
    }
    bool pending = false;
    PhaseClock pc;
    pc.start(g_phase_on != 0 && tid == 64, sclk);
    for (long long t = blockIdx.x; t < ntiles; t += gridDim.x) {
      const long long row = t * TILE + r;
      const bool ok = row < a.rows;
      const bool ld = ok && half == 0;
      const long long src = ld ? (a.index ? (long long)a.index[row] : row) : 0;
      const bool st_obs = a.stage_obs && (t + 1) * TILE <= a.rows;
      if (st_obs && half == 0) { um::mbar_wait(obs_full, po); po ^= 1; }
      const float* stg = reinterpret_cast<const float*>(OBS);
      const long long si = st_obs ? r : src;
      auto in = [&](const float* g, uint32_t off) -> const float* { return st_obs ? stg + (off >> 2) : g; };
      float in_act = 0.f, in_old = 0.f, in_adv = 0.f, in_fac = 1.f, in_w = 1.f, in_vp = 0.f, in_ret = 0.f;
      float in_actv[HEAD == HB_HEAD_BOX ? 8 : 1], in_oldv[HEAD == HB_HEAD_BOX ? 8 : 1];
      unsigned in_avm = 0xffffu;
      if (HEAD == HB_HEAD_DISCRETE) {
        if (ld) {
          in_act = in(a.actions, o_act)[si];
          if (GRAD) {
            in_old = in(a.old_logp, o_old)[si]; in_adv = in(a.adv, o_adv)[si];
            if (a.factor) in_fac = in(a.factor, o_fac)[si];
            if (a.use_active) in_w = in(a.active, o_w)[si];
          }
          if (a.avail != nullptr) {
            const float* av = in(a.avail, o_av) + si * a.out;
            in_avm = 0u;
#pragma unroll
            for (int j = 0; j < NH; ++j) in_avm |= (j < a.out && av[j < a.out ? j : 0] != 0.f) ? (1u << j) : 0u;
          }
        }
      } else if (HEAD == HB_HEAD_BOX) {
#pragma unroll
        for (int j = 0; j < (HEAD == HB_HEAD_BOX ? 8 : 1); ++j) {
          in_actv[j] = (ld && j < a.out) ? in(a.actions, o_act)[si * a.out + j] : 0.f;
          in_oldv[j] = (ld && GRAD && j < a.out) ? in(a.old_logp, o_old)[si * a.out + j] : 0.f;
        }
        if (ld && GRAD) {
          in_adv = in(a.adv, o_adv)[si];
          if (a.factor) in_fac = in(a.factor, o_fac)[si];
          if (a.use_active) in_w = in(a.active, o_w)[si];
        }
      } else if (ld && GRAD) {
        in_vp = in(a.value_preds, o_vp)[si]; in_ret = in(a.returns, o_ret)[si];
      }
      (void)in_vp; (void)in_ret; (void)in_act; (void)in_old; (void)in_actv; (void)in_oldv;
      {
        const long long tn = t + gridDim.x;
        const long long rown = tn * TILE + r;
        if (!a.stage_obs && a.index == nullptr && rown < a.rows && half == 0) {
          if (!a.stage_obs) {
            const float* on = a.obs + rown * a.in_dim;
            um::prefetch_l2(on);
            um::prefetch_l2(on + a.in_dim - 1);
          }
          if (lane == 0) {
            if (HEAD == HB_HEAD_VALUE) { if (GRAD) { um::prefetch_l2(a.value_preds + rown); um::prefetch_l2(a.returns + rown); } }
            else {
              if (HEAD == HB_HEAD_DISCRETE) um::prefetch_l2(a.actions + rown);
              if (GRAD) {
                um::prefetch_l2(a.adv + rown);
                if (HEAD == HB_HEAD_DISCRETE) um::prefetch_l2(a.old_logp + rown);
                if (a.factor) um::prefetch_l2(a.factor + rown);
                if (a.use_active) um::prefetch_l2(a.active + rown);
              }
            }
          }
          if (HEAD == HB_HEAD_DISCRETE && a.avail != nullptr) um::prefetch_l2(a.avail + rown * a.out);
          if (HEAD == HB_HEAD_BOX) { um::prefetch_l2(a.actions + rown * a.out); if (GRAD) um::prefetch_l2(a.old_logp + rown * a.out); }
        }
      }
      const float* o = st_obs ? stg + r * a.in_dim : a.obs + src * a.in_dim;
      float mean = 0.f, rs = 0.f;
      if (half == 0) {
        float s = 0.f;
        for (int k0 = 0; k0 < a.in_dim; k0 += 16) {
          float x[16];
#pragma unroll
          for (int j = 0; j < 16; ++j) x[j] = (ld && k0 + j < a.in_dim) ? o[k0 + j] : 0.f;
#pragma unroll
          for (int j = 0; j < 16; ++j) s += x[j];
        }
        mean = s / (float)a.in_dim;
        float qv = 0.f;
        for (int k0 = 0; k0 < a.in_dim; k0 += 16) {
          float x[16];
#pragma unroll
          for (int j = 0; j < 16; ++j) x[j] = (ld && k0 + j < a.in_dim) ? o[k0 + j] : 0.f;
#pragma unroll
          for (int j = 0; j < 16; ++j) { const float d = x[j] - mean; qv = k0 + j < a.in_dim ? fmaf(d, d, qv) : qv; }
        }
        rs = rsqrtf(qv / (float)a.in_dim + 1e-5f);
      }
      pc.lap(0);
      if (pending) { wait_m(); pending = false; }
      pc.lap(1);
      const float rsx = rs * XS;
      if (half == 0) {
        for (int k0 = 0; k0 < K0p; k0 += 16) {
          float x[16];
#pragma unroll
          for (int j = 0; j < 16; ++j) x[j] = (ld && k0 + j < a.in_dim) ? (o[k0 + j] - mean) * rsx : 0.f;
#pragma unroll
          for (int c = 0; c < 2; ++c) {
            const float xc[8] = {x[c * 8], x[c * 8 + 1], x[c * 8 + 2], x[c * 8 + 3], x[c * 8 + 4], x[c * 8 + 5], x[c * 8 + 6], x[c * 8 + 7]};
            uint4 hi, lo;
            um::split8(xc, hi, lo);
            const uint32_t off = img_off(r, (k0 >> 3) + c, wch0);
            *reinterpret_cast<uint4*>(X0 + off) = hi;
            *reinterpret_cast<uint4*>(X0 + x0_bytes + off) = lo;
          }
        }
      }
      signal();
      pc.lap(2);
      float mu0, rstd0, mu1, rstd1;
      uint32_t mask0[2] = {0, 0}, mask1[2] = {0, 0};
      wait_m();
      pc.lap(3);
      fwd_epilogue<ACT>(a.act, tl + C_F, H, sb0, 1.f / (XS * ws0), X1, x_bytes, wchx, RP, mu0, rstd0, mask0, mid);
      signal();
      pc.lap(4);
      wait_m();
      pc.lap(5);
      fwd_epilogue<ACT>(a.act, tl + C_F, H, sb1, 1.f / (XS * ws1), X2, x_bytes, wchx, RP, mu1, rstd1, mask1, mid);
      signal();
      pc.lap(6);
      wait_m();
      pc.lap(7);
      float dl[NH];
#pragma unroll
      for (int j = 0; j < NH; ++j) dl[j] = 0.f;
      if (half == 0) {
        float hv[NH];
        um::tmem_ld16(tl + C_H, hv);
        const float hdesc = 1.f / (XS * wsh);
        if (HEAD == HB_HEAD_DISCRETE) {
          float lg[NH], lp[NH], pj[NH];
#pragma unroll
          for (int j = 0; j < NH; ++j) lg[j] = hv[j] * hdesc;
          const unsigned avm = in_avm;
          const float ent = rows::categorical<NH>(lg, sbh, na, avm, lp, pj);
          const int act = ld ? (int)in_act : 0;
          const float lpa = rows::select<NH>(lp, act);
          if (MODE == M_EVAL) {
            if (ok) {
              if (a.logp_out) a.logp_out[row] = lpa;
              if (a.factor_inout) a.factor_inout[src] = a.factor_inout[src] * expf(lpa - a.logp_ref[src]);
            }
          } else {
            const float w = in_w, fac = in_fac, adv = in_adv, old = in_old;
            const float ratio = expf(lpa - old);
            float m;
            const float dm = dmin_dratio(ratio, adv, a.clip, a.use_clip, &m);
            const float okf = ok ? 1.f : 0.f;
            if (ok && a.logp_out) a.logp_out[row] = lpa;
            const float c_lp = -fac * w * dm * ratio * okf;
            const float c_h = a.entropy_coef * w * okf;
            if (ok) { s_loss += -fac * m * w; s_ent += ent * w; s_ratio += ratio; s_rows += 1.f; }
#pragma unroll
            for (int j = 0; j < NH; ++j) {
              const bool live = j < na && ((avm >> j) & 1u);
              dl[j] = live ? c_lp * ((j == act ? 1.f : 0.f) - pj[j]) + c_h * pj[j] * (lp[j] + ent) : 0.f;
            }
          }
        } else if (HEAD == HB_HEAD_BOX) {
          float lpj[NH], dlt[NH];
          float ent_row = 0.f;
#pragma unroll
          for (int j = 0; j < NH; ++j) {
            lpj[j] = 0.f; dlt[j] = 0.f;
            if (j < na) {
              const float mean_j = fmaf(hv[j], hdesc, sbh[j]);
              dlt[j] = (j < 8 ? in_actv[HEAD == HB_HEAD_BOX ? (j < 8 ? j : 0) : 0] : 0.f) - mean_j;
              lpj[j] = -(dlt[j] * dlt[j]) * 0.5f * sstd[3 * NH + j] - sstd[NH + j] - 0.5f * HB_LOG_2PI_F;
              ent_row += 0.5f + 0.5f * HB_LOG_2PI_F + sstd[NH + j];
            }
          }
          if (MODE == M_EVAL) {
            if (ok) {
              float agg = a.agg_prod ? 1.f : 0.f;
#pragma unroll
              for (int j = 0; j < NH; ++j) {
                if (j < na) {
                  if (a.logp_out) a.logp_out[row * na + j] = lpj[j];
                  if (a.factor_inout) {
                    const float e = expf(lpj[j] - a.logp_ref[src * na + j]);
                    agg = a.agg_prod ? agg * e : agg + e;
                  }
                }
              }
              if (a.factor_inout) a.factor_inout[src] = a.factor_inout[src] * (a.agg_prod ? agg : agg / (float)na);
            }
          } else {
            const float w = in_w, fac = in_fac, adv = in_adv;
            if (ok && a.logp_out) {
#pragma unroll
              for (int j = 0; j < NH; ++j)
                if (j < na) a.logp_out[row * na + j] = lpj[j];
            }
            float e[NH];
            float ratio = a.agg_prod ? 1.f : 0.f;
#pragma unroll
            for (int j = 0; j < NH; ++j) {
              e[j] = 0.f;
              if (j < na) {
                e[j] = expf(lpj[j] - (j < 8 ? in_oldv[HEAD == HB_HEAD_BOX ? (j < 8 ? j : 0) : 0] : 0.f));
                ratio = a.agg_prod ? ratio * e[j] : ratio + e[j];
              }
            }
            if (!a.agg_prod) ratio /= (float)na;
            float m;
            const float dm = dmin_dratio(ratio, adv, a.clip, a.use_clip, &m);
            const float okf = ok ? 1.f : 0.f;
            const float c_r = -fac * w * dm * okf;
            if (ok) { s_loss += -fac * m * w; s_ent += ent_row * w; s_ratio += ratio; s_rows += 1.f; }
#pragma unroll
            for (int j = 0; j < NH; ++j) {
              if (j < na) {
                const float sd = sstd[j], ivar = sstd[3 * NH + j];
                const float c_lp = c_r * (a.agg_prod ? ratio : e[j] / (float)na);
                const float dmean = c_lp * dlt[j] * ivar;
                const float dstd = c_lp * (dlt[j] * dlt[j] * ivar / sd - 1.f / sd) - a.entropy_coef * w * okf / sd;
                dl[j] = dmean;
                if (j < 8) dl[8 + j] = dstd * sstd[2 * NH + j];
              }
            }
          }
        } else {
          const float v = fmaf(hv[0], hdesc, sbh[0]);
          if (MODE == M_EVAL) {
            if (ok && a.logp_out) a.logp_out[row] = v;
          } else {
            const float vp = in_vp;
            float ret = in_ret;
            if (a.vn_state != nullptr) ret = (ret - vmean) / vstd;
            const float dv = v - vp;
            const float dc = fminf(fmaxf(dv, -a.clip), a.clip);
            const float vclip = vp + dc;
            const bool pass = dv >= -a.clip && dv <= a.clip;
            float de_c, de_o;
            const float l_c = huber_v(ret - vclip, a.huber_delta, a.use_huber, &de_c);
            const float l_o = huber_v(ret - v, a.huber_delta, a.use_huber, &de_o);
            const float g_o = -de_o, g_c = pass ? -de_c : 0.f;
            float loss = l_o, g = g_o;
            if (a.use_clipped) {
              if (l_c > l_o) { loss = l_c; g = g_c; }
              else if (l_c == l_o) { loss = l_o; g = 0.5f * (g_o + g_c); }
            }
            g = ok ? g * a.vcoef : 0.f;
            if (ok) { s_loss += loss; s_rows += 1.f; }
            dl[0] = g;
          }
        }
      }
      if (!GRAD) continue;
      if (half == 0) {
        float x[8];
        uint4 hi, lo;
#pragma unroll
        for (int ch = 0; ch < 2; ++ch) {
#pragma unroll
          for (int j = 0; j < 8; ++j) x[j] = dl[ch * 8 + j] * DZS;
          um::split8(x, hi, lo);
          const uint32_t off = img_off(r, ch, wchd);
          *reinterpret_cast<uint4*>(DL + off) = hi;
          *reinterpret_cast<uint4*>(DL + dl_bytes + off) = lo;
// ... 62 lines not shown
        const double s = sred[r] + sred[4 + r] + sred[8 + r] + sred[12 + r];
        if (HEAD == HB_HEAD_VALUE) { if (r == 0) atomicAdd(a.scalars, s); if (r == 3) atomicAdd(a.scalars + 1, s); }
        else atomicAdd(a.scalars + r, s);
      }
    }
  }
  um::tc_fence_before();
  __syncthreads();
  if (warp == 0) um::tmem_dealloc(tmem, TMEM_COLS);
}


constexpr uint32_t ACT_TMEM_COLS = 256;

template <int ACT>
__global__ void __launch_bounds__(THREADS, 1) fused_act_kernel(const __grid_constant__ ActArgs A) {
  extern __shared__ __align__(1024) unsigned char smem[];
  const int tid = threadIdx.x, warp = tid >> 5, lane = tid & 31;
  int ni = 0;
  for (int q = 1; q < A.n_nets; ++q) if ((int)blockIdx.x >= A.net[q].tile0) ni = q;
  const ActNet& N = A.net[ni];
  const long long t = (long long)blockIdx.x - N.tile0;
  const int H = A.H, K0p = N.K0p;
  const int wch0 = K0p >> 3, wchx = 16, wchh = H >> 3;
  const uint32_t x0_bytes = TILE * A.K0p_max * 2, x_bytes = TILE * 128 * 2, wh_bytes = NH * H * 2;
  unsigned char* p = smem;
  unsigned char* X0 = p; p += 2 * x0_bytes;
  unsigned char* X1 = p; p += 2 * x_bytes;
  unsigned char* X2 = p; p += 2 * x_bytes;
  unsigned char* WH = p; p += 2 * wh_bytes;
  unsigned char* ring = p; p += 2 * STAGE_BYTES;
  float* sb0 = reinterpret_cast<float*>(p); p += 128 * 4;
  float* sb1 = reinterpret_cast<float*>(p); p += 128 * 4;
  float* sbh = reinterpret_cast<float*>(p); p += NH * 4;
  float* xch = reinterpret_cast<float*>(p); p += 2 * TILE * 2 * 4;
  uint64_t* bars = reinterpret_cast<uint64_t*>(p); p += 8 * 8;
  uint32_t* tmem_slot = reinterpret_cast<uint32_t*>(p);
  uint64_t* w_full = bars;
  uint64_t* w_empty = bars + 2;
  uint64_t* e2m = bars + 4;
  uint64_t* m2e = bars + 5;
  uint64_t* obs_full = bars + 6;
  unsigned char* OBS = X2;
  constexpr int STG = 2;
  const __half* img0 = reinterpret_cast<const __half*>(N.prep + N.o_w0);
  const __half* img1 = reinterpret_cast<const __half*>(N.prep + N.o_w1);
  const int nch1 = H >> 5;
  const bool full = (t + 1) * TILE <= N.rows;
  const bool st_obs = N.stage && full;
  const uint32_t obs_bytes = (uint32_t)TILE * (uint32_t)N.in_dim * 4u;
  const uint32_t o_av = (N.head == HB_HEAD_DISCRETE && N.avail != nullptr) ? obs_bytes : 0u;
  const uint32_t stage_bytes = obs_bytes + (o_av ? (uint32_t)TILE * N.out * 4u : 0u);

  if (H < 128) {
    for (int i = tid; i < (int)((2 * x_bytes) / 16); i += THREADS) {
      reinterpret_cast<uint4*>(X1)[i] = make_uint4(0, 0, 0, 0);
      reinterpret_cast<uint4*>(X2)[i] = make_uint4(0, 0, 0, 0);
    }
  }
  for (int i = tid; i < (int)((2 * wh_bytes) / 16); i += THREADS)
    reinterpret_cast<uint4*>(WH)[i] = reinterpret_cast<const uint4*>(N.prep + N.o_hw)[i];
  for (int i = tid; i < 128; i += THREADS) { sb0[i] = i < H ? N.prep[N.o_b0 + i] : 0.f; sb1[i] = i < H ? N.prep[N.o_b1 + i] : 0.f; }
  if (tid < NH) sbh[tid] = N.prep[N.o_bh + tid];
  if (tid == 0) {
    for (int i = 0; i < STG; ++i) { um::mbar_init(&w_full[i], 1); um::mbar_init(&w_empty[i], 1); }
    um::mbar_init(e2m, 8);
    um::mbar_init(m2e, 1);
    um::mbar_init(obs_full, 1);
    um::fence_mbarrier_init();
  }
  if (warp == 0) um::tmem_alloc(tmem_slot, ACT_TMEM_COLS);
  um::fence_async_smem();
  um::tc_fence_before();
  __syncthreads();
  um::tc_fence_after();
  const uint32_t tmem = *tmem_slot;
  const float ws0 = N.prep[N.o_sc], ws1 = N.prep[N.o_sc + 1], wsh = N.prep[N.o_sc + 2];

  if (warp == 0) {
    if (lane == 0) {
      if (st_obs) {
        um::mbar_expect_tx(obs_full, stage_bytes);
        um::tma_bulk_g2s(OBS, N.obs + t * TILE * N.in_dim, obs_bytes, obs_full);
        if (o_av) um::tma_bulk_g2s(OBS + o_av, N.avail + t * TILE * N.out, TILE * N.out * 4, obs_full);
      }
      uint32_t it = 0;
      for (int pass = 0; pass < 2; ++pass) {
        const int nch = pass == 0 ? N.nch0 : nch1, kp = pass == 0 ? K0p : H;
        const unsigned char* src = reinterpret_cast<const unsigned char*>(pass == 0 ? img0 : img1);
        for (int c = 0; c < nch; ++c, ++it) {
          const int kc = kp - 32 * c < 32 ? kp - 32 * c : 32;
          const uint32_t bytes = 2u * (uint32_t)H * (uint32_t)kc * 2u;
          const uint32_t st = it % STG, use = it / STG;
          if (use > 0) um::mbar_wait(&w_empty[st], (use - 1) & 1);
          um::mbar_expect_tx(&w_full[st], bytes);
          um::tma_bulk_g2s(ring + st * STAGE_BYTES, src + (size_t)c * (2u * H * 32u * 2u), bytes, &w_full[st]);
        }
      }
    }
    __syncwarp();
  } else if (warp == 1) {
    if (lane == 0) {
      uint32_t it = 0, pe = 0;
      const uint32_t X0a = um::smem_u32(X0), X1a = um::smem_u32(X1), X2a = um::smem_u32(X2), WHa = um::smem_u32(WH), RGa = um::smem_u32(ring);
      auto wait_e = [&]() { um::mbar_wait(e2m, pe); pe ^= 1; um::tc_fence_after(); };
      auto chunk = [&](int kc, auto&& body) {
        const uint32_t st = it % STG, use = it / STG;
        um::mbar_wait(&w_full[st], use & 1);
        um::tc_fence_after();
        body(RGa + st * STAGE_BYTES, (uint32_t)H * (uint32_t)kc * 2u);
        um::commit(&w_empty[st]);
        ++it;
      };
      wait_e();
      for (int c = 0; c < N.nch0; ++c) {
        const int kc = K0p - 32 * c < 32 ? K0p - 32 * c : 32;
        chunk(kc, [&](uint32_t wb, uint32_t wimg) {
          gemm3(tmem + C_F, op_kmajor(X0a, x0_bytes, wch0, 4 * c), op_kmajor(wb, wimg, kc >> 3, 0), kc >> 4, um::idesc_f16(H, 0, 0), c > 0);
        });
      }
      um::commit(m2e);
      wait_e();
      for (int c = 0; c < nch1; ++c)
        chunk(32, [&](uint32_t wb, uint32_t wimg) {
          gemm3(tmem + C_F, op_kmajor(X1a, x_bytes, wchx, 4 * c), op_kmajor(wb, wimg, 4, 0), 2, um::idesc_f16(H, 0, 0), c > 0);
        });
      um::commit(m2e);
      wait_e();
      gemm3(tmem + 128, op_kmajor(X2a, x_bytes, wchx, 0), op_kmajor(WHa, wh_bytes, wchh, 0), H >> 4, um::idesc_f16(NH, 0, 0), false);
      um::commit(m2e);
    }
    __syncwarp();
  } else {
    const int q = warp & 3, r = q * 32 + lane, half = (warp - 2) >> 2;
    const uint32_t tl = tmem + ((uint32_t)(q * 32) << 16);
    const RowPair RP{xch, half, r, 2 + q};
    uint32_t pm = 0;
    auto wait_m = [&]() { um::mbar_wait(m2e, pm); pm ^= 1; um::tc_fence_after(); };
    auto signal = [&]() { um::fence_async_smem(); um::tc_fence_before(); __syncwarp(); if (lane == 0) um::mbar_arrive(e2m); };
    const long long row = t * TILE + r;
    const bool ok = row < N.rows;
    const bool ld = ok && half == 0;
    const int na = N.out;
    if (st_obs && half == 0) um::mbar_wait(obs_full, 0);
    const float* stg = reinterpret_cast<const float*>(OBS);
    unsigned avm = 0xffffu;
    if (N.head == HB_HEAD_DISCRETE && N.avail != nullptr && ld) {
      const float* av = st_obs ? stg + (o_av >> 2) + r * na : N.avail + row * na;
      avm = 0u;
#pragma unroll
      for (int j = 0; j < NH; ++j) avm |= (j < na && av[j < na ? j : 0] != 0.f) ? (1u << j) : 0u;
    }
    const float* o = st_obs ? stg + r * N.in_dim : N.obs + (ok ? row : 0) * N.in_dim;
    float mean = 0.f, rs = 0.f;
    if (half == 0) {
      float s = 0.f;
      for (int k0 = 0; k0 < N.in_dim; k0 += 16) {
        float x[16];
#pragma unroll
        for (int j = 0; j < 16; ++j) x[j] = (ld && k0 + j < N.in_dim) ? o[k0 + j] : 0.f;
#pragma unroll
        for (int j = 0; j < 16; ++j) s += x[j];
      }
      mean = s / (float)N.in_dim;
      float qv = 0.f;
      for (int k0 = 0; k0 < N.in_dim; k0 += 16) {
        float x[16];
#pragma unroll
        for (int j = 0; j < 16; ++j) x[j] = (ld && k0 + j < N.in_dim) ? o[k0 + j] : 0.f;
#pragma unroll
        for (int j = 0; j < 16; ++j) { const float d = x[j] - mean; qv = k0 + j < N.in_dim ? fmaf(d, d, qv) : qv; }
      }
      rs = rsqrtf(qv / (float)N.in_dim + 1e-5f);
      const float rsx = rs * XS;
      for (int k0 = 0; k0 < K0p; k0 += 16) {
        float x[16];
#pragma unroll
        for (int j = 0; j < 16; ++j) x[j] = (ld && k0 + j < N.in_dim) ? (o[k0 + j] - mean) * rsx : 0.f;
#pragma unroll
        for (int c = 0; c < 2; ++c) {
          const float xc[8] = {x[c * 8], x[c * 8 + 1], x[c * 8 + 2], x[c * 8 + 3], x[c * 8 + 4], x[c * 8 + 5], x[c * 8 + 6], x[c * 8 + 7]};
          uint4 hi, lo;
          um::split8(xc, hi, lo);
          const uint32_t off = img_off(r, (k0 >> 3) + c, wch0);
          *reinterpret_cast<uint4*>(X0 + off) = hi;
          *reinterpret_cast<uint4*>(X0 + x0_bytes + off) = lo;
        }
      }
    }
    signal();
    float mu0, rstd0, mu1, rstd1;
    uint32_t mask0[2], mask1[2];
    wait_m();
    fwd_epilogue<ACT>(A.act, tl + C_F, H, sb0, 1.f / (XS * ws0), X1, x_bytes, wchx, RP, mu0, rstd0, mask0);
    signal();
    wait_m();
    fwd_epilogue<ACT>(A.act, tl + C_F, H, sb1, 1.f / (XS * ws1), X2, x_bytes, wchx, RP, mu1, rstd1, mask1);
    signal();
    wait_m();
    if (half == 0) {
      float hv[NH];
      um::tmem_ld16(tl + 128, hv);
      const float hdesc = 1.f / (XS * wsh);
      const unsigned long long off = A.offset + (A.offset_base ? *A.offset_base : 0ull);
      if (N.head == HB_HEAD_VALUE) {
        if (ok) N.out0[row] = fmaf(hv[0], hdesc, sbh[0]);
      } else if (N.head == HB_HEAD_DISCRETE) {
        float lg[NH], lp[NH], pj[NH];
#pragma unroll
        for (int j = 0; j < NH; ++j) lg[j] = hv[j] * hdesc;
        rows::categorical<NH>(lg, sbh, na, avm, lp, pj);
        const int pick = rows::categorical_pick<NH>(pj, na, A.deterministic != 0, A.deterministic ? 0.f : rows::row_uniform(row, N.seed, off));
        const float lpp = rows::select<NH>(lp, pick);
        if (ok) { N.out0[row] = (float)pick; N.out1[row] = lpp; }
      } else {
        const float* log_std = N.prep + N.o_ls;
#pragma unroll
        for (int j = 0; j < 8; ++j) {
          if (j < na) {
            const float mean_j = fmaf(hv[j], hdesc, sbh[j]);
            const float sig = 1.f / (1.f + expf(-log_std[j] / N.std_x));
            const float sd = sig * N.std_y, lsd = logf(sd);
            float act = mean_j;
            if (!A.deterministic) {
              const uint4 rnd = philox4x32(make_uint4((uint32_t)row, (uint32_t)((unsigned long long)row >> 32), (uint32_t)j, (uint32_t)off),
                                           make_uint2((uint32_t)N.seed, (uint32_t)(N.seed >> 32) ^ (uint32_t)(off >> 32)));
              const float u1 = u01(rnd.x), u2 = u01(rnd.y);
              act = mean_j + sd * (sqrtf(-2.f * logf(u1)) * cospif(2.f * u2));
            }
            if (ok) {
              const float dv = act - mean_j;
              N.out0[row * na + j] = act;
              N.out1[row * na + j] = -(dv * dv) / (2.f * sd * sd) - lsd - 0.5f * HB_LOG_2PI_F;
            }
          }
        }
      }
    }
  }
  um::tc_fence_before();
  __syncthreads();
  if (warp == 0) um::tmem_dealloc(tmem, ACT_TMEM_COLS);
}

struct PackJob {
  const float* W; const float* gamma; const float* beta; const float* b;
  int N, K, Nimg, Kp, KC, RC;
  __half* img; float* bias_out; float* scale_out;
  int cta0, ctas;
};
struct PackJobs { PackJob j[4]; int n; };

__global__ void __launch_bounds__(256) fused_pack_kernel(PackJobs jobs) {
  __shared__ float smax[8];
  __shared__ float sscale;
  int ji = 0;
  for (int q = 1; q < jobs.n; ++q) if ((int)blockIdx.x >= jobs.j[q].cta0) ji = q;
  const PackJob& J = jobs.j[ji];
  const int cta = blockIdx.x - J.cta0;
  const float* __restrict__ W = J.W;
  const float* __restrict__ gamma = J.gamma;
  const int N = J.N, K = J.K, Nimg = J.Nimg, Kp = J.Kp, KC = J.KC, RC = J.RC;
  __half* __restrict__ img = J.img;
  float mx = 0.f;
  for (int i = threadIdx.x; i < N * K; i += 256) mx = fmaxf(mx, fabsf(W[i] * (gamma ? gamma[i % K] : 1.f)));
  mx = warp_max(mx);
  if ((threadIdx.x & 31) == 0) smax[threadIdx.x >> 5] = mx;
  __syncthreads();
  if (threadIdx.x == 0) {
    float m = 0.f;
    for (int i = 0; i < 8; ++i) m = fmaxf(m, smax[i]);
    int ex = 0;
    if (m > 0.f) frexpf(m, &ex);
    ex = ex < -20 ? -20 : (ex > 20 ? 20 : ex);
    sscale = m > 0.f ? exp2f((float)(8 - ex)) : 1.f;
    if (cta == 0 && J.scale_out != nullptr) *J.scale_out = sscale;
  }
  __syncthreads();
  const float sc = sscale;
  const int total = Nimg * Kp;
  for (int i = cta * 256 + threadIdx.x; i < total; i += J.ctas * 256) {
    const int n = i / Kp, k = i % Kp;
    const float v = (n < N && k < K) ? W[n * K + k] * (gamma ? gamma[k] : 1.f) * sc : 0.f;
    const __half hi = __float2half_rn(v);
    const __half lo = __float2half_rn(v - __half2float(hi));
    if (RC > 0) {
      const int c = n / RC, nl = n % RC;
      const size_t chunk0 = (size_t)c * (2u * RC * Kp);
      const size_t e = (size_t)((nl >> 3) * (Kp >> 3) + (k >> 3)) * 64 + (nl & 7) * 8 + (k & 7);
      img[chunk0 + e] = hi;
      img[chunk0 + (size_t)RC * Kp + e] = lo;
      continue;
    }
    const int c = k / KC, kl = k % KC;
    const int kc = Kp - KC * c < KC ? Kp - KC * c : KC;
    const size_t chunk0 = (size_t)c * (2u * Nimg * KC);
    const size_t e = (size_t)((n >> 3) * (kc >> 3) + (kl >> 3)) * 64 + (n & 7) * 8 + (kl & 7);
    img[chunk0 + e] = hi;
    img[chunk0 + (size_t)Nimg * kc + e] = lo;
  }
  if (J.bias_out != nullptr) {
    const int warp = threadIdx.x >> 5, lane = threadIdx.x & 31;
    for (int n = cta * 8 + warp; n < Nimg; n += J.ctas * 8) {
      float v = 0.f;
      if (n < N && J.beta)
        for (int k = lane; k < K; k += 32) v += W[n * K + k] * J.beta[k];
      for (int o = 16; o > 0; o >>= 1) v += __shfl_xor_sync(0xffffffffu, v, o);
      if (lane == 0) J.bias_out[n] = n < N ? J.b[n] + v : 0.f;
    }
  }
}

struct Regions { int n; int off[8]; int len[8]; float scale[8]; };
constexpr int SR_GROUPS = 8, SR_MAXPER = 16;
__global__ void __launch_bounds__(32 * SR_GROUPS, 6) fused_slot_reduce_kernel(float* __restrict__ grad, const float* __restrict__ part, int slots,
                                                                           long long stride, int total, const __grid_constant__ Regions R,
                                                                           const double* __restrict__ norm3, double host_scale) {
  __shared__ float sm[SR_GROUPS][32];
  const int lane = threadIdx.x & 31, g = threadIdx.x >> 5;
  const int i = blockIdx.x * 32 + lane;
  const int per = (slots + SR_GROUPS - 1) / SR_GROUPS;
  const int s0 = g * per, s1 = s0 + per < slots ? s0 + per : slots;
  float acc = 0.f;
  if (i < total) {
    for (int sb = s0; sb < s1; sb += SR_MAXPER) {
      float v[SR_MAXPER];
#pragma unroll
      for (int u = 0; u < SR_MAXPER; ++u) v[u] = sb + u < s1 ? part[(long long)(sb + u) * stride + i] : 0.f;
#pragma unroll
      for (int u = 0; u < SR_MAXPER; ++u) acc += v[u];
    }
  }
  sm[g][lane] = acc;
  __syncthreads();
  if (g != 0 || i >= total) return;
  float sc = 0.f;
  bool in = false;
  for (int q = 0; q < R.n; ++q)
    if (i >= R.off[q] && i < R.off[q] + R.len[q]) { sc = R.scale[q]; in = true; }
  if (!in) { grad[i] = 0.f; return; }
  float t = 0.f;
#pragma unroll
  for (int q = 0; q < SR_GROUPS; ++q) t += sm[q][lane];
  const double nrm = host_scale * (norm3 ? 1.0 / norm3[2] : 1.0);
  grad[i] = (float)((double)t * (double)sc * nrm);
}

struct Folds { int n; int w[3], b[3], gw[3], gb[3], N[3], K[3], col0[3]; };
__global__ void __launch_bounds__(128) fused_unfold_kernel(const float* __restrict__ params, float* __restrict__ grad, Folds F, int cols) {
  const int warp = (blockIdx.x * blockDim.x + threadIdx.x) >> 5, lane = threadIdx.x & 31;
  if (warp >= cols) return;
  int f = 0;
  for (int q = 1; q < F.n; ++q) if (warp >= F.col0[q]) f = q;
  const int k = warp - F.col0[f], N = F.N[f], K = F.K[f];
  const float gam = params[F.gw[f] + k], bet = params[F.gb[f] + k];
  double dg = 0.0, dbt = 0.0;
  for (int n = lane; n < N; n += 32) {
    const float w = params[F.w[f] + n * K + k];
    const float G = grad[F.w[f] + n * K + k];
    const float gb = grad[F.b[f] + n];
    dg += (double)w * (double)G;
    dbt += (double)w * (double)gb;
    grad[F.w[f] + n * K + k] = fmaf(gam, G, bet * gb);
  }
  dg = warp_sum_d(dg);
  dbt = warp_sum_d(dbt);
  if (lane == 0) { grad[F.gw[f] + k] = (float)dg; grad[F.gb[f] + k] = (float)dbt; }
}

static std::atomic<int> g_enabled{-1};

}

int fused_timing_enable(int on) {
  static const unsigned long long zeros[148 * 16] = {0};
  cudaError_t e = cudaMemcpyToSymbol(fz::g_phase_cycles, zeros, sizeof(zeros));
  if (e == cudaSuccess) e = cudaMemcpyToSymbol(fz::g_phase_on, &on, sizeof(int));
  return e == cudaSuccess ? HB_OK : cuda_fail(e, "fused_timing_enable");
}
int fused_timing_read(unsigned long long* out) {
  cudaError_t e = cudaDeviceSynchronize();
  if (e == cudaSuccess) e = cudaMemcpyFromSymbol(out, fz::g_phase_cycles, sizeof(unsigned long long) * 148 * 16);
  return e == cudaSuccess ? HB_OK : cuda_fail(e, "fused_timing_read");
}

bool fused_enabled() {
  int v = fz::g_enabled.load(std::memory_order_relaxed);
  if (v < 0) {
    const char* e = getenv("HB_FUSED");
    v = (e != nullptr && atoi(e) == 0) ? 0 : 1;
    fz::g_enabled.store(v);
  }
  return v != 0 && gemm_impl() != 0;
}
void set_fused_enabled(int v) { fz::g_enabled.store(v ? 1 : 0); }

bool fused_shape_ok(const hb_net_desc* d) {
  if (d->rnn_layers != 0 || d->n_layers != 2 || d->hidden[0] != d->hidden[1]) return false;
  const int H = d->hidden[0];
  if (H != 32 && H != 64 && H != 128) return false;
  if (!d->feature_norm || d->in_dim < 1 || d->in_dim > 64) return false;
  if (d->activation == HB_ACT_HARDSWISH) return false;
  if (d->out_dim < 1 || d->out_dim > (d->head == HB_HEAD_BOX ? 8 : fz::NH)) return false;
  return true;
}

int launch_fused_pack(const hb_net_desc* d, const ParamLayout& P, const PrepLayout& Q, const float* params, float* prepared,
                      cudaStream_t st) {
  const int H = d->hidden[0];
  float* sc = prepared + Q.fz_scale;
  fz::PackJobs jobs;
  memset(&jobs, 0, sizeof(jobs));
  int cta = 0;
  auto add = [&](const float* W, const float* g, const float* be, const float* b, int N, int K, int Nimg, int Kp, int KC, int RC,
                 float* img, float* bias_out, float* scale_out, int ctas) {
    fz::PackJob& J = jobs.j[jobs.n++];
    J.W = W; J.gamma = g; J.beta = be; J.b = b; J.N = N; J.K = K; J.Nimg = Nimg; J.Kp = Kp; J.KC = KC; J.RC = RC;
    J.img = reinterpret_cast<__half*>(img); J.bias_out = bias_out; J.scale_out = scale_out; J.cta0 = cta; J.ctas = ctas;
    cta += ctas;
  };
  add(params + P.w[0], params + P.fn_w, params + P.fn_b, params + P.b[0], H, d->in_dim, H, Q.fz_k0p, 32, 0, prepared + Q.fz_w[0],
      prepared + Q.fz_bias[0], sc + 0, 8);
  add(params + P.w[1], params + P.lnw[0], params + P.lnb[0], params + P.b[1], H, H, H, H, 32, 0, prepared + Q.fz_w[1],
      prepared + Q.fz_bias[1], sc + 1, 16);
  add(params + P.w[1], params + P.lnw[0], params + P.lnb[0], params + P.b[1], H, H, H, H, 32, 32, prepared + Q.fz_w1b, nullptr, nullptr, 16);
  add(params + P.hw, params + P.lnw[1], params + P.lnb[1], params + P.hbias, d->out_dim, H, fz::NH, H, H, 0, prepared + Q.fz_hw,
      prepared + Q.fz_hbias, sc + 2, 4);
  fz::fused_pack_kernel<<<cta, 256, 0, st>>>(jobs);
  HB_LAUNCH_DONE(st, "fused_pack");
  return HB_OK;
}


int fused_act_fill(fz::ActNet* n, const hb_net_desc* d, const float* prepared, const float* obs, const float* avail, float* out0,
                   float* out1, unsigned long long seed, long long rows, bool* ok) {
  PrepLayout Q;
  int rc = make_layouts(d, nullptr, &Q, nullptr);
  if (rc) return rc;
  *ok = Q.fz_ok != 0 && (d->head != HB_HEAD_BOX || d->out_dim <= 8);
  if (!*ok) return HB_OK;
  n->prep = prepared; n->obs = obs; n->avail = avail; n->out0 = out0; n->out1 = out1; n->seed = seed; n->rows = rows;
  n->in_dim = d->in_dim; n->out = d->out_dim; n->head = d->head; n->K0p = Q.fz_k0p; n->nch0 = Q.fz_chunks[0];
  n->o_w0 = Q.fz_w[0]; n->o_w1 = Q.fz_w[1]; n->o_hw = Q.fz_hw; n->o_b0 = Q.fz_bias[0]; n->o_b1 = Q.fz_bias[1]; n->o_bh = Q.fz_hbias;
  n->o_sc = Q.fz_scale; n->o_ls = Q.log_std; n->std_x = d->std_x_coef; n->std_y = d->std_y_coef;
  const uintptr_t bits = reinterpret_cast<uintptr_t>(obs) | reinterpret_cast<uintptr_t>(avail);
  n->stage = (bits & 15) == 0 ? 1 : 0;
  return HB_OK;
}

int launch_fused_act(fz::ActArgs& A, cudaStream_t st) {
  int tiles = 0, k0 = 16;
  for (int i = 0; i < A.n_nets; ++i) {
    A.net[i].tile0 = tiles;
    tiles += (int)((A.net[i].rows + fz::TILE - 1) / fz::TILE);
    k0 = A.net[i].K0p > k0 ? A.net[i].K0p : k0;
  }
  A.K0p_max = k0;
  if (tiles == 0) return HB_OK;
  const size_t smem = 2 * (size_t)fz::TILE * k0 * 2 + 2 * 2 * (size_t)fz::TILE * 128 * 2 + 2 * (size_t)fz::NH * A.H * 2 + 2 * fz::STAGE_BYTES +
                      2 * 128 * 4 + fz::NH * 4 + 2 * fz::TILE * 2 * 4 + 8 * 8 + 16 + 1024;
#define HB_FZA(ACTV)                                                                                  \
  {                                                                                                   \
    auto kern = fz::fused_act_kernel<ACTV>;                                                           \
    cudaFuncSetAttribute(kern, cudaFuncAttributeMaxDynamicSharedMemorySize, (int)smem);               \
    kern<<<tiles, fz::THREADS, smem, st>>>(A);                                                        \
  }
  if (A.act == HB_ACT_RELU) HB_FZA(HB_ACT_RELU)
  else if (A.act == HB_ACT_TANH) HB_FZA(HB_ACT_TANH)
  else HB_FZA(-1)
#undef HB_FZA
  HB_LAUNCH_DONE(st, "fused_act");
  return HB_OK;
}

size_t fused_smem_bytes(int H, int K0p) {
  size_t b = 2 * (size_t)fz::TILE * K0p * 2 + 2 * 2 * (size_t)fz::TILE * 128 * 2 + 3 * (size_t)fz::TILE * fz::NH * 2 +
             2 * (size_t)fz::NH * H * 2 + (size_t)(K0p <= 32 ? 3 : 2) * fz::STAGE_BYTES;
  b += 2 * 128 * 4 + fz::NH * 4 + 4 * fz::NH * 4 + 2 * fz::NH * 4 + 16 * 8 + 2 * fz::TILE * 2 * 4 + 10 * 8 + 16 * 8 + 16;
  return b + 1024;
}

template <int HEAD, int MODE>
static int launch_fused_act(const fz::Args& a, int grid, size_t smem, cudaStream_t st) {
#define HB_FZ(ACTV)                                                                                   \
  {                                                                                                   \
    auto kern = fz::fused_update_kernel<HEAD, MODE, ACTV>;                                            \
    cudaFuncSetAttribute(kern, cudaFuncAttributeMaxDynamicSharedMemorySize, (int)smem);               \
    kern<<<grid, fz::THREADS, smem, st>>>(a);                                                         \
  }
  if (a.act == HB_ACT_RELU) HB_FZ(HB_ACT_RELU)
  else if (a.act == HB_ACT_TANH) HB_FZ(HB_ACT_TANH)
  else HB_FZ(-1)
#undef HB_FZ
  return HB_OK;
}

int launch_fused_update(const hb_net_desc* d, const PrepLayout& Q, const ParamLayout& P, const float* prepared, fz::Args a, int mode,
                        int* grid_out, cudaStream_t st) {
  const int H = d->hidden[0];
  a.H = H; a.K0p = Q.fz_k0p; a.in_dim = d->in_dim; a.out = d->out_dim; a.act = d->activation; a.nch0 = Q.fz_chunks[0];
  a.img0 = reinterpret_cast<const __half*>(prepared + Q.fz_w[0]);
  a.img1 = reinterpret_cast<const __half*>(prepared + Q.fz_w[1]);
  a.img1b = reinterpret_cast<const __half*>(prepared + Q.fz_w1b);
  a.imgh = reinterpret_cast<const __half*>(prepared + Q.fz_hw);
  a.bias0 = prepared + Q.fz_bias[0]; a.bias1 = prepared + Q.fz_bias[1]; a.biash = prepared + Q.fz_hbias;
  a.scales = prepared + Q.fz_scale;
  a.log_std = prepared + Q.log_std; a.std_x = d->std_x_coef; a.std_y = d->std_y_coef;
  a.pw0 = P.w[0]; a.pb0 = P.b[0]; a.pw1 = P.w[1]; a.pb1 = P.b[1]; a.phw = P.hw; a.phb = P.hbias; a.plogstd = P.log_std;
  {
    const void* ptrs[] = {a.obs, a.actions, a.old_logp, a.adv, a.factor, a.active, a.avail, a.value_preds, a.returns};
    uintptr_t bits = 0;
    for (const void* q : ptrs) bits |= reinterpret_cast<uintptr_t>(q);
    a.stage_obs = (a.index == nullptr && (bits & 15) == 0) ? 1 : 0;
  }
  const long long ntiles = (a.rows + fz::TILE - 1) / fz::TILE;
  const int grid = (int)(ntiles < 148 ? ntiles : 148);
  if (grid_out) *grid_out = grid;
  const size_t smem = fused_smem_bytes(H, Q.fz_k0p);
  int rc;
  if (d->head == HB_HEAD_DISCRETE) rc = mode == 0 ? launch_fused_act<HB_HEAD_DISCRETE, fz::M_GRAD>(a, grid, smem, st) : launch_fused_act<HB_HEAD_DISCRETE, fz::M_EVAL>(a, grid, smem, st);
  else if (d->head == HB_HEAD_BOX) rc = mode == 0 ? launch_fused_act<HB_HEAD_BOX, fz::M_GRAD>(a, grid, smem, st) : launch_fused_act<HB_HEAD_BOX, fz::M_EVAL>(a, grid, smem, st);
  else rc = mode == 0 ? launch_fused_act<HB_HEAD_VALUE, fz::M_GRAD>(a, grid, smem, st) : launch_fused_act<HB_HEAD_VALUE, fz::M_EVAL>(a, grid, smem, st);
  if (rc) return rc;
  HB_LAUNCH_DONE(st, shape_label(mode == 0 ? (d->head == HB_HEAD_VALUE ? "fused_critic_update" : "fused_actor_update") : "fused_evaluate",
                                 a.rows, H, d->in_dim));
  return HB_OK;
}

int launch_fused_finish(const hb_net_desc* d, const ParamLayout& P, const float* params, float* grad, const float* part, int slots,
                        long long stride, const double* norm3, double host_scale, cudaStream_t st) {
  const int H = d->hidden[0];
  fz::Regions R;
  memset(&R, 0, sizeof(R));
  const float sw = 1.f / (fz::DZS * fz::XS), sb = 1.f / fz::DZS;
  int n = 0;
  auto add = [&](int off, int len, float s) { R.off[n] = off; R.len[n] = len; R.scale[n] = s; ++n; };
  add(P.w[0], H * d->in_dim, sw); add(P.b[0], H, sb);
  add(P.w[1], H * H, sw);         add(P.b[1], H, sb);
  add(P.hw, d->out_dim * H, sw);  add(P.hbias, d->out_dim, sb);
  if (d->head == HB_HEAD_BOX) add(P.log_std, d->out_dim, sb);
  R.n = n;
  fz::fused_slot_reduce_kernel<<<(P.total + 31) / 32, 32 * fz::SR_GROUPS, 0, st>>>(grad, part, slots, stride, P.total, R, norm3, host_scale);
  HB_LAUNCH_DONE(st, "fused_slot_reduce");
  fz::Folds F;
  memset(&F, 0, sizeof(F));
  int cols = 0;
  auto fold = [&](int w, int b, int gw, int gb, int N, int K) {
    const int q = F.n++;
    F.w[q] = w; F.b[q] = b; F.gw[q] = gw; F.gb[q] = gb; F.N[q] = N; F.K[q] = K; F.col0[q] = cols;
    cols += K;
  };
  fold(P.w[0], P.b[0], P.fn_w, P.fn_b, H, d->in_dim);
  fold(P.w[1], P.b[1], P.lnw[0], P.lnb[0], H, H);
  fold(P.hw, P.hbias, P.lnw[1], P.lnb[1], d->out_dim, H);
  fz::fused_unfold_kernel<<<(cols * 32 + 127) / 128, 128, 0, st>>>(params, grad, F, cols);
  HB_LAUNCH_DONE(st, "ln_affine_grad_fold");
  return HB_OK;
}

}
```

harl_b200/nets.py:

```python
import ctypes as C
from collections import OrderedDict

import torch

from . import _lib as L

_WORKSPACES = {}


def workspace(device, nbytes):
    key = (str(device), torch.cuda.current_stream(device).cuda_stream)
    ws = _WORKSPACES.get(key)
    if ws is None or ws.numel() < nbytes:
        ws = torch.empty(int(nbytes), dtype=torch.uint8, device=device)
        _WORKSPACES[key] = ws
    return ws


def _is_matrix(name):
    if name.startswith("rnn.rnn.weight") or name in (
            "act.action_out.linear.weight", "act.action_out.fc_mean.weight", "v_out.weight"):
        return True
    if name.startswith("base.mlp.fc.") and name.endswith(".weight"):
        return int(name.split(".")[3]) % 3 == 0
# ... 18 lines not shown
    d.head = head
    d.out_dim = int(out_dim)
    d.std_x_coef = float(args.get("std_x_coef", 1.0))
    d.std_y_coef = float(args.get("std_y_coef", 0.5))
    return d


class DeviceNet:
    def __init__(self, args, in_dim, head, out_dim, device, init=True):
        self.args = args
        self.device = torch.device(device)
        self.desc = make_desc(args, in_dim, head, out_dim)
        lay = L.NetLayout()
        L.check(L.lib.hb_net_layout_of(C.byref(self.desc), C.byref(lay)), "hb_net_layout_of")
        self.total = lay.total
        self.entries = OrderedDict()
        for i in range(lay.n_tensors):
            name = lay.names[i].value.decode()
            rows, cols = lay.rows[i], lay.cols[i]
            self.entries[name] = (lay.offset[i], (rows, cols) if _is_matrix(name) else (cols,))
        kw = dict(dtype=torch.float32, device=self.device)
        self.params = torch.zeros(self.total, **kw)
        self.grad = torch.zeros(self.total, **kw)
        self.exp_avg = torch.zeros(self.total, **kw)
        self.exp_avg_sq = torch.zeros(self.total, **kw)
        self.prepared = torch.zeros(lay.prepared_total, **kw)
        self.grad_norm = torch.zeros(1, **kw)
        self.adam_steps = 0
        self.head = head
        self.out_dim = int(out_dim)
        self.act_width = 1 if head == L.HEAD_DISCRETE else int(out_dim)
        if init:
            self.reset_parameters()

    def views(self, flat=None):
        flat = self.params if flat is None else flat
        out = OrderedDict()
        for name, (off, shape) in self.entries.items():
            n = 1
            for s in shape:
                n *= s
            out[name] = flat[off:off + n].view(*shape)
        return out

    def state_dict(self):
        return OrderedDict((k, v.clone()) for k, v in self.views().items())

    def load_state_dict(self, sd):
        v = self.views()
        missing = [k for k in v if k not in sd]
        if missing:
            raise KeyError(f"missing keys {missing}")
        with torch.no_grad():
            for k, dst in v.items():
                src = torch.as_tensor(sd[k], dtype=torch.float32)
                dst.copy_(src.reshape(dst.shape))
        self.prepare()

    def reset_parameters(self):
        a = self.args
        init = getattr(torch.nn.init, a["initialization_method"])
        gain = torch.nn.init.calculate_gain(a["activation_func"])
        d = self.desc
        sd = {}
        if d.feature_norm:
            sd["base.feature_norm.weight"] = torch.ones(d.in_dim)
            sd["base.feature_norm.bias"] = torch.zeros(d.in_dim)
        prev = d.in_dim
        for li in range(d.n_layers):
            h = d.hidden[li]
            lin = torch.nn.Linear(prev, h)
            init(lin.weight.data, gain=gain)
            sd[f"base.mlp.fc.{3 * li}.weight"] = lin.weight.data
            sd[f"base.mlp.fc.{3 * li}.bias"] = torch.zeros(h)
            sd[f"base.mlp.fc.{3 * li + 2}.weight"] = torch.ones(h)
            sd[f"base.mlp.fc.{3 * li + 2}.bias"] = torch.zeros(h)
            prev = h
        if d.rnn_layers:
            gru = torch.nn.GRU(prev, prev, num_layers=d.rnn_layers)
            for name, p in gru.named_parameters():
                if "bias" in name:
                    torch.nn.init.constant_(p, 0)
                elif "weight" in name:
                    init(p)
                sd["rnn.rnn." + name] = p.data
            sd["rnn.norm.weight"] = torch.ones(prev)
            sd["rnn.norm.bias"] = torch.zeros(prev)
        if self.head == L.HEAD_DISCRETE:
            lin = torch.nn.Linear(prev, d.out_dim)
            init(lin.weight.data, gain=a["gain"])
            sd["act.action_out.linear.weight"] = lin.weight.data
            sd["act.action_out.linear.bias"] = torch.zeros(d.out_dim)
        elif self.head == L.HEAD_BOX:
            lin = torch.nn.Linear(prev, d.out_dim)
            init(lin.weight.data, gain=a["gain"])
            sd["act.action_out.fc_mean.weight"] = lin.weight.data
            sd["act.action_out.fc_mean.bias"] = torch.zeros(d.out_dim)
            sd["act.action_out.log_std"] = torch.ones(d.out_dim) * a["std_x_coef"]
        else:
            lin = torch.nn.Linear(prev, 1)
            init(lin.weight.data)
            sd["v_out.weight"] = lin.weight.data
            sd["v_out.bias"] = torch.zeros(1)
        v = self.views()
        with torch.no_grad():
            for k, dst in v.items():
                dst.copy_(sd[k].reshape(dst.shape))
        if self.device.type == "cuda":
            self.prepare()

    def _need_cuda(self):
        if self.device.type != "cuda":
            raise RuntimeError("harl_b200 kernels need a CUDA device (no CPU fallback)")

    def prepare(self):
        self._need_cuda()
        L.call("hb_net_prepare", C.byref(self.desc), L.ptr(self.params), L.ptr(self.prepared), L.stream_ptr())

    def _ws(self, rows, mode):
        n = L.lib.hb_workspace_bytes(C.byref(self.desc), int(rows), mode)
        ws = workspace(self.device, n)
        return ws, ws.numel()

    @property
    def recurrent(self):
        return self.desc.rnn_layers > 0

    def act(self, obs, avail, deterministic, seed, offset, actions_out, logp_out, rnn_states=None, masks=None,
            rnn_out=None):
        self._need_cuda()
        rows = obs.shape[0]
        ws, n = self._ws(rows, 0)
        if self.recurrent:
            L.call("hb_policy_act_rnn", C.byref(self.desc), L.ptr(self.prepared), L.ptr(obs), rows, L.ptr(avail),
                   L.ptr(rnn_states), L.ptr(masks), int(bool(deterministic)), int(seed) & (2**64 - 1),
                   int(offset) & (2**64 - 1), None, L.ptr(actions_out), L.ptr(logp_out), L.ptr(rnn_out), L.ptr(ws), n,
                   L.stream_ptr())
            return
        L.call("hb_policy_act", C.byref(self.desc), L.ptr(self.prepared), L.ptr(obs), rows, L.ptr(avail),
               int(bool(deterministic)), int(seed) & (2**64 - 1), int(offset) & (2**64 - 1), L.ptr(actions_out),
               L.ptr(logp_out), L.ptr(ws), n, L.stream_ptr())

    def values(self, cent_obs, values_out, rnn_states=None, masks=None, rnn_out=None):
        self._need_cuda()
        rows = cent_obs.shape[0]
        ws, n = self._ws(rows, 0)
        if self.recurrent:
            L.call("hb_value_forward_rnn", C.byref(self.desc), L.ptr(self.prepared), L.ptr(cent_obs), rows,
                   L.ptr(rnn_states), L.ptr(masks), L.ptr(values_out), L.ptr(rnn_out), L.ptr(ws), n, L.stream_ptr())
            return
        L.call("hb_value_forward", C.byref(self.desc), L.ptr(self.prepared), L.ptr(cent_obs), rows,
               L.ptr(values_out), L.ptr(ws), n, L.stream_ptr())

    @staticmethod
    def actor_batch(obs, actions, old_logp=None, adv=None, factor=None, active=None, avail=None, index=None, rows=None,
                    rnn_states=None, masks=None, seq_len=0):
        b = L.ActorBatch()
        b.obs, b.actions, b.old_logp, b.adv = L.ptr(obs), L.ptr(actions), L.ptr(old_logp), L.ptr(adv)
        b.factor, b.active, b.avail, b.index = L.ptr(factor), L.ptr(active), L.ptr(avail), L.ptr(index)
        b.rows = int(rows if rows is not None else (index.shape[0] if index is not None else actions.shape[0]))
        b.rnn_states, b.masks, b.seq_len = L.ptr(rnn_states), L.ptr(masks), int(seq_len)
        b._keep = (obs, actions, old_logp, adv, factor, active, avail, index, rnn_states, masks)
        return b

    @staticmethod
    def critic_batch(share_obs, value_preds, returns, index=None, rows=None, rnn_states=None, masks=None, seq_len=0):
        b = L.CriticBatch(L.ptr(share_obs), L.ptr(value_preds), L.ptr(returns), L.ptr(index),
                          int(rows if rows is not None else (index.shape[0] if index is not None else value_preds.numel())),
                          L.ptr(rnn_states), L.ptr(masks), int(seq_len))
        b._keep = (share_obs, value_preds, returns, index, rnn_states, masks)
        return b

    def evaluate(self, batch, logp_out=None, logp_ref=None, factor_inout=None, agg_prod=True):
        self._need_cuda()
        ws, n = self._ws(batch.rows, 0)
        L.call("hb_policy_evaluate", C.byref(self.desc), L.ptr(self.prepared), C.byref(batch), L.ptr(logp_out),
               L.ptr(logp_ref), L.ptr(factor_inout), int(bool(agg_prod)), L.ptr(ws), n, L.stream_ptr())

    def actor_grad(self, batch, hyper, norm3, scalars, logp_out=None):
        self._need_cuda()
        ws, n = self._ws(batch.rows, 1)
        L.call("hb_ppo_actor_grad_logp", C.byref(self.desc), L.ptr(self.params), L.ptr(self.prepared), C.byref(batch),
               C.byref(hyper), L.ptr(norm3), L.ptr(self.grad), L.ptr(scalars), L.ptr(logp_out), L.ptr(ws), n, L.stream_ptr())

    def value_grad(self, batch, hyper, vn_state, inv_count, scalars):
        self._need_cuda()
        ws, n = self._ws(batch.rows, 1)
        L.call("hb_value_grad", C.byref(self.desc), L.ptr(self.params), L.ptr(self.prepared), C.byref(batch),
               C.byref(hyper), L.ptr(vn_state), float(inv_count), L.ptr(self.grad), L.ptr(scalars), L.ptr(ws), n,
               L.stream_ptr())

    def adam_step(self, lr, eps, weight_decay, max_grad_norm, use_max_grad_norm, betas=(0.9, 0.999)):
        self._need_cuda()
        self.adam_steps += 1
        h = L.AdamHyper(float(lr), betas[0], betas[1], float(eps), float(weight_decay), float(max_grad_norm),
                        int(bool(use_max_grad_norm)), self.adam_steps)
        L.call("hb_clip_adam_step", C.byref(self.desc), L.ptr(self.params), L.ptr(self.grad), L.ptr(self.exp_avg),
               L.ptr(self.exp_avg_sq), L.ptr(self.prepared), C.byref(h), L.ptr(self.grad_norm), L.stream_ptr())

    def _trpo_ws(self, rows):
        n = L.lib.hb_trpo_workspace_bytes(C.byref(self.desc), int(rows))
        ws = workspace(self.device, n)
        return ws, ws.numel()

    def trpo_old_dist(self, batch, old_dist):
        self._need_cuda()
        ws, n = self._trpo_ws(batch.rows)
        L.call("hb_trpo_old_dist", C.byref(self.desc), L.ptr(self.prepared), C.byref(batch), L.ptr(old_dist), L.ptr(ws), n,
               L.stream_ptr())

    def trpo_fvp(self, batch, old_dist, vec, inv_rows, out, reuse_forward=False):
        self._need_cuda()
        ws, n = self._trpo_ws(batch.rows)
        L.call("hb_trpo_fvp", C.byref(self.desc), L.ptr(self.params), L.ptr(self.prepared), C.byref(batch),
               L.ptr(old_dist), L.ptr(vec), float(inv_rows), int(bool(reuse_forward)), L.ptr(out), L.ptr(ws), n,
               L.stream_ptr())

    def trpo_fvp_finish(self, vec, out, damping=0.1):
        L.call("hb_trpo_fvp_finish", C.byref(self.desc), L.ptr(self.params), L.ptr(vec), L.ptr(out), float(damping),
               L.stream_ptr())

    def trpo_eval(self, batch, hyper, old_dist, params_old, scalars):
        self._need_cuda()
        ws, n = self._trpo_ws(batch.rows)
        L.call("hb_trpo_eval", C.byref(self.desc), L.ptr(self.prepared), C.byref(batch), C.byref(hyper), L.ptr(old_dist),
               L.ptr(params_old), L.ptr(scalars), L.ptr(ws), n, L.stream_ptr())
```

harl_b200/runners/on_policy_ha_runner.py:

```python
import os

import torch

from .. import _lib as L
from .. import dist
from ..nets import DeviceNet
from .on_policy_base_runner import OnPolicyBaseRunner


class OnPolicyHARunner(OnPolicyBaseRunner):
    def train(self):
        T = self.algo_args["train"]["episode_length"]
        N = self.n_local
        dev = self.device
        rows = T * N
        cb = self.critic_buffer
        factor = torch.ones(T, N, 1, dtype=torch.float32, device=dev)
        advantages = cb.advantages
        if self.state_type == "FP":
            active = torch.stack([b.active_masks[:-1] for b in self.actor_buffer], dim=2).contiguous()
            m3 = torch.zeros(3, dtype=torch.float64, device=dev)
            L.call("hb_masked_moments", L.ptr(advantages), L.ptr(active), advantages.numel(), L.ptr(m3), L.stream_ptr())
            dist.all_reduce_sum_(m3)
            adv_n = torch.empty_like(advantages)
            L.call("hb_normalize_by_moments", L.ptr(advantages), L.ptr(adv_n), advantages.numel(), L.ptr(m3), L.stream_ptr())
            advantages = adv_n
        if self.fixed_order:
            agent_order = list(range(self.num_agents))
        else:
            agent_order = list(torch.randperm(self.num_agents).numpy())
        self.last_agent_order = agent_order
        if self.world > 1 and not self.fixed_order:
            o = torch.tensor([int(a) for a in agent_order], dtype=torch.int64, device=dev)
            o0 = o.clone()
            torch.distributed.broadcast(o0, src=0)
            assert torch.equal(o, o0), "agent order differs across ranks (unsynchronised torch CPU generator)"
        infos = []
        agg_prod = self.action_aggregation == "prod"
        critic_pending = None
        overlap = getattr(self, "overlap_critic_update", True)
        inter = os.environ.get("HB_CRITIC_INTERLEAVE")
        interleave = overlap and all(hasattr(a, "first_epoch_logp") for a in self.actor) and \
            (inter == "1" or (inter is None and self.world > 1))
        main = torch.cuda.current_stream(dev)
        if overlap:
            side = getattr(self, "_side_stream", None)
            if side is None:
                side = self._side_stream = torch.cuda.Stream(device=dev)
            side.wait_stream(main)
        if overlap and not interleave:
            with torch.cuda.stream(side):
                critic_pending = self.critic.train(cb, self.value_normalizer, defer=True)
        ch = None
        if interleave:
            ch = dict(gen=self.critic.train_steps(cb, self.value_normalizer), k=0, wait=None, done=False)

            def after_critic_big():
                ev = torch.cuda.Event()
                ev.record(side)
                ch["wait"] = ev

            def before_actor_big():
                if ch["wait"] is not None:
                    main.wait_event(ch["wait"])
                    ch["wait"] = None

            def after_actor_big():
                ch["k"] += 1
                if not ch["done"] and ch["k"] % 3 == 1:
                    ev = torch.cuda.Event()
                    ev.record(main)
                    with torch.cuda.stream(side):
                        side.wait_event(ev)
                        if next(ch["gen"], None) is None:
                            ch["done"] = True

            self.critic.after_grad_hook = after_critic_big
            for a in self.actor:
                a.grad_hooks = (before_actor_big, after_actor_big)
        adv_m3 = torch.zeros(self.num_agents, 3, dtype=torch.float64, device=dev)
        for a in range(self.num_agents):
            adv_a = advantages if self.state_type == "EP" else advantages[:, :, a].contiguous()
            L.call("hb_masked_moments", L.ptr(adv_a), L.ptr(self.actor_buffer[a].active_masks[:-1]), rows, L.ptr(adv_m3[a]),
                   L.stream_ptr())
        dist.all_reduce_sum_(adv_m3)
        n_active = adv_m3[:, 2].cpu().numpy()
        for agent_id in agent_order:
            buf, actor = self.actor_buffer[agent_id], self.actor[agent_id]
            buf.update_factor(factor)
            fl = lambda a: a.reshape(rows, *a.shape[2:])
            avail = None if buf.available_actions is None else fl(buf.available_actions[:-1])
            if actor.recurrent:
                sweep = DeviceNet.actor_batch(fl(buf.obs[:-1]), fl(buf.actions), avail=avail,
                                              rnn_states=buf.rnn_states.reshape((T + 1) * N, -1),
                                              masks=buf.masks.reshape((T + 1) * N), seq_len=T)
            else:
                sweep = DeviceNet.actor_batch(fl(buf.obs[:-1]), fl(buf.actions), avail=avail)
            old_logp = torch.empty(rows, actor.actor.act_width, dtype=torch.float32, device=dev)
            adv_a = advantages if self.state_type == "EP" else advantages[:, :, agent_id].contiguous()
            fuse = (getattr(actor, "first_epoch_logp", False) and not actor.recurrent and getattr(actor, "actor_num_mini_batch", 0) == 1
                    and n_active[agent_id] > 0 and getattr(self, "fuse_old_logp", True))
            if not fuse:
                if ch is not None:
                    before_actor_big()
                actor.actor.evaluate(sweep, logp_out=old_logp)
                if ch is not None:
                    after_actor_big()
                infos.append(actor.train(buf, adv_a, self.state_type, moments=(adv_m3[agent_id], float(n_active[agent_id]))))
            else:
                infos.append(actor.train(buf, adv_a, self.state_type, moments=(adv_m3[agent_id], float(n_active[agent_id])),
                                         old_logp_out=old_logp))
                assert actor.old_logp_filled
            if ch is not None:
                before_actor_big()
            actor.actor.evaluate(sweep, logp_ref=old_logp, factor_inout=factor.reshape(rows), agg_prod=agg_prod)
            if ch is not None:
                after_actor_big()
        if ch is not None:
            with torch.cuda.stream(side):
                for _ in ch["gen"]:
                    pass
            self.critic.after_grad_hook = None
            for a in self.actor:
                a.grad_hooks = None
            critic_pending = self.critic.finish_train
        if critic_pending is not None:
            torch.cuda.current_stream(dev).wait_stream(self._side_stream)
            critic_info = critic_pending()
        else:
            critic_info = self.critic.train(cb, self.value_normalizer)
        ordered = [None] * self.num_agents
        for pos, agent_id in enumerate(agent_order):
            ordered[agent_id] = infos[pos]
        return ordered, critic_info
```

include/harl_b200.h:

```cpp
#ifndef HARL_B200_H
#define HARL_B200_H

#include <stddef.h>
#include <stdint.h>

#ifdef __cplusplus
extern "C" {
#endif

#define HB_VERSION 100
#define HB_MAX_LAYERS 4
#define HB_MAX_AGENTS 32
#define HB_MAX_TENSORS 40

typedef enum hb_status {
  HB_OK = 0,
  HB_ERR_INVALID = -1,
  HB_ERR_UNSUPPORTED = -2,
  HB_ERR_WORKSPACE = -3,
  HB_ERR_CUDA = -4
} hb_status;

typedef enum hb_activation {
  HB_ACT_RELU = 0,
// ... 7 lines not shown

typedef enum hb_head {
  HB_HEAD_DISCRETE = 0,
  HB_HEAD_BOX = 1,
  HB_HEAD_VALUE = 2
} hb_head;

typedef struct hb_net_desc {
  int32_t in_dim;
  int32_t n_layers;
  int32_t hidden[HB_MAX_LAYERS];
  int32_t feature_norm;
  int32_t activation;
  int32_t rnn_layers;
  int32_t head;
  int32_t out_dim;
  float std_x_coef;
  float std_y_coef;
} hb_net_desc;

typedef struct hb_net_layout {
  int32_t n_tensors;
  int32_t total;
  int32_t offset[HB_MAX_TENSORS];
  int32_t rows[HB_MAX_TENSORS];
  int32_t cols[HB_MAX_TENSORS];
  char names[HB_MAX_TENSORS][48];
  int32_t prepared_total;
} hb_net_layout;

int hb_version(void);
const char* hb_last_error(void);
int hb_sync_check(void);

uint64_t hb_kernel_launch_count(void);
int hb_profile_begin(void* stream);
int hb_profile_end(char* out, int out_size);

int hb_set_gemm_impl(int impl);
int hb_get_gemm_impl(void);

int hb_set_fused_update(int on);
int hb_get_fused_update(void);
int hb_fused_timing_enable(int on);
int hb_fused_timing_read(unsigned long long* out);

int hb_net_layout_of(const hb_net_desc* d, hb_net_layout* out);
int hb_net_prepare(const hb_net_desc* d, const float* params, float* prepared, void* stream);
size_t hb_workspace_bytes(const hb_net_desc* d, int64_t rows, int mode);

typedef struct hb_insert_args {
  int32_t n_envs, n_agents, state_type_fp;
  int32_t actor_rnn_row, critic_rnn_row;
  const uint8_t* dones;
  const uint8_t* bad_transition;
  float* actor_masks_next[HB_MAX_AGENTS];
  float* actor_active_next[HB_MAX_AGENTS];
  float* actor_rnn_next[HB_MAX_AGENTS];
  float* critic_masks_next;
  float* critic_bad_next;
  float* critic_rnn_next;
  const float* rewards;
  int64_t reward_stride_n, reward_stride_a;
  float* ep_return;
  double* done_sum;
} hb_insert_args;
int hb_rollout_insert_masks(const hb_insert_args* a, void* stream);

int hb_policy_act(const hb_net_desc* d, const float* prepared, const float* obs, int64_t rows,
                  const float* avail, int deterministic, uint64_t seed, uint64_t offset,
                  float* actions, float* logp, void* ws, size_t ws_bytes, void* stream);

typedef struct hb_collect_args {
  int32_t n_agents, deterministic;
  int64_t rows;
  uint64_t offset;
  const hb_net_desc* actor_desc[HB_MAX_AGENTS];
  const float* actor_prepared[HB_MAX_AGENTS];
  const float* obs[HB_MAX_AGENTS];
  const float* avail[HB_MAX_AGENTS];
  float* actions[HB_MAX_AGENTS];
  float* logp[HB_MAX_AGENTS];
  uint64_t seed[HB_MAX_AGENTS];
  const hb_net_desc* critic_desc;
  const float* critic_prepared;
  const float* share_obs;
  int64_t critic_rows;
  float* values;
  const uint64_t* offset_base;
  const float* actor_rnn[HB_MAX_AGENTS];
  float* actor_rnn_out[HB_MAX_AGENTS];
  const float* actor_masks[HB_MAX_AGENTS];
  const float* critic_rnn;
  float* critic_rnn_out;
  const float* critic_masks;
} hb_collect_args;
int hb_rollout_collect(const hb_collect_args* a, void* ws, size_t ws_bytes, void* stream);
int hb_counter_add(uint64_t* counter, uint64_t inc, void* stream);

int hb_value_forward(const hb_net_desc* d, const float* prepared, const float* cent_obs,
                     int64_t rows, float* values, void* ws, size_t ws_bytes, void* stream);

int hb_gae_returns(const float* rewards, float* value_preds, const float* masks,
                   const float* bad_masks, const float* next_value, float* returns,
                   float* advantages, int32_t T, int64_t C, float gamma, float gamma_lambda,
                   int use_gae, int use_proper_time_limits, const float* vn_state, void* stream);

#define HB_COPY_MAX_SEGS 16
typedef struct hb_copy_seg {
  void* dst;
  const void* src;
  int64_t bytes;
} hb_copy_seg;
int hb_copy_segments(const hb_copy_seg* segs, int32_t n, void* stream);

int hb_comm_create(int32_t rank, int32_t world, size_t slot_bytes, void** comm_out, void* ipc_handle_out64);
int hb_comm_open_peers(void* comm, const void* all_handles);
int hb_allreduce_bucket(void* comm, void* buf, int64_t n, int32_t dtype, void* stream);
int hb_comm_status(void* comm);
int hb_comm_destroy(void* comm);

int hb_set_gae_impl(int impl);
int hb_get_gae_impl(void);

int hb_masked_moments(const float* x, const float* weight, int64_t n, double* out3, void* stream);
int hb_normalize_by_moments(const float* x, float* x_out, int64_t n, const double* moments3,
                            void* stream);

int hb_valuenorm_update(float* vn_state, const double* moments3, double beta, void* stream);
int hb_valuenorm_apply(const float* vn_state, const float* x, float* y, int64_t n,
                       int denormalize, void* stream);

typedef struct hb_ppo_hyper {
  float clip_param;
  float entropy_coef;
  int32_t use_policy_active_masks;
  int32_t action_aggregation_prod;
  int32_t use_clip;
} hb_ppo_hyper;

typedef struct hb_actor_batch {
  const float* obs;
  const float* actions;
  const float* old_logp;
  const float* adv;
  const float* factor;
  const float* active;
  const float* avail;
  const int32_t* index;
  int64_t rows;
  const float* rnn_states;
  const float* masks;
  int64_t seq_len;
} hb_actor_batch;

int hb_policy_evaluate(const hb_net_desc* d, const float* prepared, const hb_actor_batch* b,
                       float* logp_out, const float* logp_ref, float* factor_inout,
                       int action_aggregation_prod, void* ws, size_t ws_bytes, void* stream);

int hb_ppo_actor_grad(const hb_net_desc* d, const float* params, const float* prepared,
                      const hb_actor_batch* b, const hb_ppo_hyper* h, const double* norm3,
                      float* grad, double* scalars, void* ws, size_t ws_bytes, void* stream);

int hb_ppo_actor_grad_logp(const hb_net_desc* d, const float* params, const float* prepared, const hb_actor_batch* b,
                           const hb_ppo_hyper* h, const double* norm3, float* grad, double* scalars, float* logp_out,
                           void* ws, size_t ws_bytes, void* stream);

typedef struct hb_value_hyper {
  float clip_param;
  float huber_delta;
  float value_loss_coef;
  int32_t use_huber_loss;
  int32_t use_clipped_value_loss;
} hb_value_hyper;

typedef struct hb_critic_batch {
  const float* share_obs;
  const float* value_preds;
  const float* returns;
  const int32_t* index;
  int64_t rows;
  const float* rnn_states;
  const float* masks;
  int64_t seq_len;
} hb_critic_batch;

int hb_value_grad(const hb_net_desc* d, const float* params, const float* prepared,
                  const hb_critic_batch* b, const hb_value_hyper* h, const float* vn_state,
                  double inv_count, float* grad, double* scalars, void* ws, size_t ws_bytes,
                  void* stream);

typedef struct hb_adam_hyper {
  float lr, beta1, beta2, eps, weight_decay, max_grad_norm;
  int32_t use_max_grad_norm;
  int32_t step;
} hb_adam_hyper;
int hb_clip_adam_step(const hb_net_desc* d, float* params, const float* grad, float* exp_avg,
                      float* exp_avg_sq, float* prepared, const hb_adam_hyper* h,
                      float* grad_norm_out, void* stream);

int hb_policy_act_rnn(const hb_net_desc* d, const float* prepared, const float* obs, int64_t rows,
                      const float* avail, const float* rnn_states, const float* masks, int deterministic,
                      uint64_t seed, uint64_t offset, const uint64_t* offset_base, float* actions, float* logp,
                      float* rnn_states_out, void* ws, size_t ws_bytes, void* stream);
int hb_value_forward_rnn(const hb_net_desc* d, const float* prepared, const float* cent_obs, int64_t rows,
                         const float* rnn_states, const float* masks, float* values, float* rnn_states_out,
                         void* ws, size_t ws_bytes, void* stream);

int hb_set_rnn_impl(int impl);
int hb_get_rnn_impl(void);
int hb_set_trpo_jvp_impl(int impl);
int hb_get_trpo_jvp_impl(void);


size_t hb_trpo_workspace_bytes(const hb_net_desc* d, int64_t rows);

int hb_trpo_old_dist(const hb_net_desc* d, const float* prepared, const hb_actor_batch* b, float* old_dist,
                     void* ws, size_t ws_bytes, void* stream);

int hb_trpo_fvp(const hb_net_desc* d, const float* params, const float* prepared, const hb_actor_batch* b,
                const float* old_dist, const float* v, double inv_rows, int reuse_forward, float* out, void* ws,
                size_t ws_bytes, void* stream);
int hb_trpo_fvp_finish(const hb_net_desc* d, const float* params, const float* v, float* out, float damping,
                       void* stream);

int hb_trpo_eval(const hb_net_desc* d, const float* prepared, const hb_actor_batch* b, const hb_ppo_hyper* h,
                 const float* old_dist, const float* params_old, double* scalars, void* ws, size_t ws_bytes,
                 void* stream);

int hb_trpo_cg_init(const float* b, float* x, float* r, float* p, float* cg_state, int n, void* stream);
int hb_trpo_cg_step(float* p, const float* avp, float* x, float* r, float* cg_state, int n, float residual_tol,
                    void* stream);
int hb_trpo_full_step(const float* x, const float* fx, const float* g, float kl_threshold, float* full_step,
                      double* out3, int n, void* stream);
int hb_trpo_apply_step(float* params, const float* params0, const float* full_step, float fraction, int n,
                       void* stream);
int hb_vec_scale(float* x, float s, int n, void* stream);

#define HB_MPE_MAX_AGENTS 8
typedef struct hb_mpe_args {
  int32_t n_envs, n_agents, n_landmarks;
  int32_t continuous;
  int32_t max_cycles;
  int32_t reset_all;
  uint64_t seed;
  float* pos; float* vel; float* landmarks;
  int32_t* step_count; uint64_t* episode;
  const float* actions[HB_MPE_MAX_AGENTS];
  float* obs_out[HB_MPE_MAX_AGENTS];
  float* share_obs_out;
  float* rewards_out;
  float* rewards_na_out;
  uint8_t* dones_out; uint8_t* bad_out;
} hb_mpe_args;
int hb_mpe_spread_step(const hb_mpe_args* a, void* stream);

#ifdef __cplusplus
}
#endif
#endif
```

profiles/fused_phase_clock.py:

```python
import ctypes as C
import os
import sys

sys.path.insert(0, os.path.dirname(os.path.dirname(os.path.abspath(__file__))))
import numpy as np
import torch

from harl_b200 import _lib as L
from harl_b200.nets import DeviceNet
from harl_b200.utils.configs_tools import get_defaults_yaml_args

algo_args, _ = get_defaults_yaml_args("happo", "pettingzoo_mpe")
cfg = {**algo_args["model"], **algo_args["algo"]}
dev = torch.device("cuda:0")
torch.manual_seed(0)
net = DeviceNet(cfg, 18, L.HEAD_DISCRETE, 5, dev)
R = 819200
g = torch.Generator().manual_seed(1)
obs = torch.randn(R, 18, generator=g).to(dev)
acts = torch.randint(0, 5, (R, 1), generator=g).float().to(dev)
old = (-1.6 + 0.1 * torch.randn(R, 1, generator=g)).to(dev)
adv = torch.randn(R, generator=g).to(dev)
fac, active, avail = torch.ones(R, device=dev), torch.ones(R, device=dev), torch.ones(R, 5, device=dev)
batch = DeviceNet.actor_batch(obs, acts, old, adv, fac, active, avail)
hyper = L.PPOHyper(0.2, 0.01, 1, 1, 1)
norm3 = torch.tensor([0, 0, float(R)], dtype=torch.float64, device=dev)
scal = torch.zeros(4, dtype=torch.float64, device=dev)
for _ in range(3):
    net.actor_grad(batch, hyper, norm3, scal)
torch.cuda.synchronize()
L.call("hb_fused_timing_enable", 1)
e0, e1 = torch.cuda.Event(enable_timing=True), torch.cuda.Event(enable_timing=True)
e0.record()
net.actor_grad(batch, hyper, norm3, scal)
e1.record()
torch.cuda.synchronize()
tab = np.zeros((148, 16), np.uint64)
L.call("hb_fused_timing_read", tab.ctypes.data_as(C.c_void_p))
L.call("hb_fused_timing_enable", 0)
names = ["inputs+featnorm stats", "wait prev-tile bwd MMAs", "write X0", "wait L0 MMA", "L0 fwd epilogue", "wait L1 MMA",
         "L1 fwd epilogue", "wait head MMA", "head epilogue", "wait head-bwd MMA", "L1 bwd epilogue", "wait L1-bwd MMAs",
         "L0 bwd epilogue"]
tiles = R / 128 / 148
m = tab.astype(np.float64).mean(0)
print(f"fused_actor_update {e0.elapsed_time(e1) * 1e3:.1f} us for {R} rows; {tiles:.1f} tiles per CTA; cycles per tile (mean over CTAs):")
for i, n in enumerate(names):
    print(f"  {i:2d} {n:28s} {m[i] / tiles:9.0f}")
print(f"     {'sum':28s} {m[:13].sum() / tiles:9.0f}")
```

Before: 34.77 million.

## Precompute normalised split-TF32 observation images once per update and reuse across epochs

Adds a kernel that computes the per-row feature normalisation once and writes the input tile as hi/lo split images in the fused kernels' smem layout. Actor and critic fused update kernels can TMA-load these images straight into X0 instead of recomputing featnorm stats and split writes every epoch. It also skips the factor-update evaluate after the last agent in the HAPPO order. The cost is extra global memory for the image buffers, an additional precompute launch, and more mbarrier handshaking in the producer warp.

Measured after the change: 34.61 million (median of 6 runs). No clear change (-0.5%).

```diff
diff --git a/harl_b200/_lib.py b/harl_b200/_lib.py
--- a/harl_b200/_lib.py
+++ b/harl_b200/_lib.py
@@ -65,7 +65,8 @@
 class ActorBatch(C.Structure):
     _fields_ = [("obs", C.c_void_p), ("actions", C.c_void_p), ("old_logp", C.c_void_p), ("adv", C.c_void_p),
                 ("factor", C.c_void_p), ("active", C.c_void_p), ("avail", C.c_void_p), ("index", C.c_void_p),
-                ("rows", C.c_int64), ("rnn_states", C.c_void_p), ("masks", C.c_void_p), ("seq_len", C.c_int64)]
+                ("rows", C.c_int64), ("rnn_states", C.c_void_p), ("masks", C.c_void_p), ("seq_len", C.c_int64),
+                ("obs_images", C.c_void_p)]
 
 
 class ValueHyper(C.Structure):
@@ -76,7 +77,7 @@
 class CriticBatch(C.Structure):
     _fields_ = [("share_obs", C.c_void_p), ("value_preds", C.c_void_p), ("returns", C.c_void_p),
                 ("index", C.c_void_p), ("rows", C.c_int64), ("rnn_states", C.c_void_p), ("masks", C.c_void_p),
-                ("seq_len", C.c_int64)]
+                ("seq_len", C.c_int64), ("share_obs_images", C.c_void_p)]
 
 
 class AdamHyper(C.Structure):
@@ -154,6 +155,8 @@
     "hb_normalize_by_moments": (C.c_int, [P, P, C.c_int64, P, P]),
     "hb_valuenorm_update": (C.c_int, [P, P, C.c_double, P]),
     "hb_valuenorm_apply": (C.c_int, [P, P, P, C.c_int64, C.c_int, P]),
+    "hb_obs_images_bytes": (C.c_size_t, [C.POINTER(NetDesc), C.c_int64]),
+    "hb_obs_images": (C.c_int, [C.POINTER(NetDesc), P, C.c_int64, P, P]),
     "hb_policy_evaluate": (C.c_int, [C.POINTER(NetDesc), P, C.POINTER(ActorBatch), P, P, P, C.c_int, P, C.c_size_t, P]),
     "hb_ppo_actor_grad": (C.c_int, [C.POINTER(NetDesc), P, P, C.POINTER(ActorBatch), C.POINTER(PPOHyper), P, P, P, P,
                                     C.c_size_t, P]),
@@ -199,7 +202,7 @@
 GEMM_IMPLS = {"fp32": 0, "3xtf32": 1}
 if os.environ.get("HB_GEMM_IMPL"):
     lib.hb_set_gemm_impl(GEMM_IMPLS[os.environ["HB_GEMM_IMPL"]])
-_NO_CHECK = {"hb_version", "hb_last_error", "hb_workspace_bytes", "hb_trpo_workspace_bytes", "hb_kernel_launch_count", "hb_profile_end", "hb_get_gemm_impl", "hb_get_rnn_impl", "hb_get_trpo_jvp_impl", "hb_get_fused_update", "hb_get_gae_impl", "hb_comm_status"}
+_NO_CHECK = {"hb_version", "hb_last_error", "hb_workspace_bytes", "hb_trpo_workspace_bytes", "hb_obs_images_bytes", "hb_kernel_launch_count", "hb_profile_end", "hb_get_gemm_impl", "hb_get_rnn_impl", "hb_get_trpo_jvp_impl", "hb_get_fused_update", "hb_get_gae_impl", "hb_comm_status"}
 
 call_count = 0
 
diff --git a/harl_b200/algorithms/actors/happo.py b/harl_b200/algorithms/actors/happo.py
--- a/harl_b200/algorithms/actors/happo.py
+++ b/harl_b200/algorithms/actors/happo.py
@@ -58,7 +58,7 @@
         s, n = scal.cpu().numpy(), norm3[2].item()
         return s[0] / n, s[1] / n, self.actor.grad_norm.item(), s[2] / s[3]
 
-    def train(self, actor_buffer, advantages, state_type, moments=None, old_logp_out=None):
+    def train(self, actor_buffer, advantages, state_type, moments=None, old_logp_out=None, obs_images=None):
         self.old_logp_filled = False
         info = dict(policy_loss=0.0, dist_entropy=0.0, actor_grad_norm=0.0, ratio=0.0)
         d = self.device
@@ -105,7 +105,8 @@
                         norms[u, 2] = float(nrows)
                     dist.all_reduce_sum_(norms[u])
                 batch = DeviceNet.actor_batch(obs, actions, old_lp, adv, factor, active, avail, idx, nrows,
-                                              rnn_states=rnn, masks=masks, seq_len=seq_len)
+                                              rnn_states=rnn, masks=masks, seq_len=seq_len,
+                                              obs_images=obs_images if idx is None else None)
                 first = u == 0 and old_logp_out is not None and (idx is None) and nrows == rows
                 self._step(batch, norms[u], scal[u], old_logp_out if first else None)
                 self.old_logp_filled = self.old_logp_filled or first
diff --git a/harl_b200/algorithms/critics/v_critic.py b/harl_b200/algorithms/critics/v_critic.py
--- a/harl_b200/algorithms/critics/v_critic.py
+++ b/harl_b200/algorithms/critics/v_critic.py
@@ -62,7 +62,7 @@
                             int(bool(self.use_huber_loss)), int(bool(self.use_clipped_value_loss)))
 
     def _step(self, share_obs, value_preds, returns, index, rows, global_rows, value_normalizer, scalars_row,
-              rnn_states=None, masks=None, seq_len=0, whole=None):
+              rnn_states=None, masks=None, seq_len=0, whole=None, obs_images=None):
         d = self.device
         if value_normalizer is not None:
             m3 = whole.get("m3") if whole is not None and index is None else None
@@ -74,7 +74,8 @@
                 if whole is not None and index is None:
                     whole["m3"] = m3
             value_normalizer.update_from_moments(m3)
-        cb = DeviceNet.critic_batch(share_obs, value_preds, returns, index, rows, rnn_states, masks, seq_len)
+        cb = DeviceNet.critic_batch(share_obs, value_preds, returns, index, rows, rnn_states, masks, seq_len,
+                                    obs_images if index is None else None)
         vn = value_normalizer.state if value_normalizer is not None else None
         self.critic.value_grad(cb, self._hyper(), vn, 1.0 / global_rows, scalars_row)
         if getattr(self, "after_grad_hook", None) is not None:
@@ -119,9 +120,16 @@
         gnorm = torch.zeros(n_up, dtype=torch.float32, device=d)
         u = 0
         whole = {}
+        imgs = None
+        if nmb == 1 and not self.recurrent:
+            bufs = self.__dict__.setdefault("_obs_images", {})
+            key = torch.cuda.current_stream(d).cuda_stream
+            imgs = self.critic.obs_images(so, bufs.get(key))
+            bufs[key] = imgs
         for _ in range(self.critic_epoch):
             for idx, n, seq_len in seq_index.minibatches(T, Cn, nmb, mode, self.data_chunk_length, d):
-                self._step(so, vp, rt, idx, n, float(n * dist.world_size()), value_normalizer, scal[u], rnn, masks, seq_len, whole)
+                self._step(so, vp, rt, idx, n, float(n * dist.world_size()), value_normalizer, scal[u], rnn, masks, seq_len, whole,
+                           imgs)
                 gnorm[u] = self.critic.grad_norm[0]
                 u += 1
                 yield u
diff --git a/harl_b200/csrc/capi.cu b/harl_b200/csrc/capi.cu
--- a/harl_b200/csrc/capi.cu
+++ b/harl_b200/csrc/capi.cu
@@ -324,12 +324,32 @@
   return value_forward_impl(d, prepared, cent_obs, rows, rnn_states, masks, values, rnn_states_out, ws, ws_bytes, stream);
 }
 
+size_t hb_obs_images_bytes(const hb_net_desc* d, int64_t rows) {
+  using namespace hb;
+  PrepLayout Q;
+  if (d == nullptr || rows < 0 || make_layouts(d, nullptr, &Q, nullptr) != HB_OK || !Q.fz_ok) return 0;
+  return fused_obs_images_bytes(rows, Q.fz_k0p);
+}
+
+int hb_obs_images(const hb_net_desc* d, const float* obs, int64_t rows, void* out, void* stream) {
+  using namespace hb;
+  HB_CHECK_ARG(d && obs && out && rows >= 0, "bad argument");
+  HB_CHECK_ARG((reinterpret_cast<uintptr_t>(out) & 15) == 0, "out must be 16-byte aligned");
+  PrepLayout Q;
+  int rc = make_layouts(d, nullptr, &Q, nullptr);
+  if (rc) return rc;
+  if (!Q.fz_ok) { set_error("hb_obs_images: net outside the fused kernels' shapes"); return HB_ERR_UNSUPPORTED; }
+  return launch_obs_images(obs, rows, d->in_dim, Q.fz_k0p, static_cast<unsigned char*>(out), (cudaStream_t)stream);
+}
+
 int hb_policy_evaluate(const hb_net_desc* d, const float* prepared, const hb_actor_batch* b, float* logp_out,
                        const float* logp_ref, float* factor_inout, int action_aggregation_prod, void* ws,
                        size_t ws_bytes, void* stream) {
   using namespace hb;
   HB_CHECK_ARG(prepared && b && b->obs && b->actions && b->rows >= 0, "bad argument");
   HB_CHECK_ARG(!factor_inout || (logp_ref && !b->index), "factor update needs logp_ref and an identity batch");
+  HB_CHECK_ARG(!b->obs_images || !b->index, "obs_images need an identity batch");
+  HB_CHECK_ARG((reinterpret_cast<uintptr_t>(b->obs_images) & 15) == 0, "obs_images must be 16-byte aligned");
   PrepLayout Q;
   int rc = check_net(d, nullptr, &Q, nullptr, 1);
   if (rc) return rc;
@@ -342,6 +362,7 @@
     fz::Args fa;
     memset(&fa, 0, sizeof(fa));
     fa.obs = b->obs; fa.index = b->index; fa.rows = rows;
+    fa.obs_images = static_cast<const unsigned char*>(b->obs_images);
     fa.actions = b->actions; fa.avail = b->avail;
     fa.logp_out = logp_out; fa.logp_ref = logp_ref; fa.factor_inout = factor_inout;
     fa.agg_prod = action_aggregation_prod;
@@ -382,6 +403,8 @@
   HB_CHECK_ARG(params && prepared && b && h && norm3 && grad && scalars, "NULL argument");
   HB_CHECK_ARG(b->obs && b->actions && b->old_logp && b->adv && b->active && b->rows >= 0, "incomplete batch");
   HB_CHECK_ARG(!logp_out || !b->index, "logp_out needs an identity batch (rows of the batch = rows of logp_out)");
+  HB_CHECK_ARG(!b->obs_images || !b->index, "obs_images need an identity batch");
+  HB_CHECK_ARG((reinterpret_cast<uintptr_t>(b->obs_images) & 15) == 0, "obs_images must be 16-byte aligned");
   ParamLayout P;
   PrepLayout Q;
   hb_net_layout L;
@@ -394,6 +417,7 @@
     fz::Args fa;
     memset(&fa, 0, sizeof(fa));
     fa.obs = b->obs; fa.index = b->index; fa.rows = b->rows;
+    fa.obs_images = static_cast<const unsigned char*>(b->obs_images);
     fa.actions = b->actions; fa.avail = b->avail; fa.old_logp = b->old_logp; fa.adv = b->adv; fa.factor = b->factor; fa.active = b->active;
     fa.clip = h->clip_param; fa.entropy_coef = h->entropy_coef; fa.use_active = h->use_policy_active_masks;
     fa.use_clip = h->use_clip; fa.agg_prod = h->action_aggregation_prod;
@@ -461,6 +485,8 @@
   using namespace hb;
   HB_CHECK_ARG(params && prepared && b && h && grad && scalars, "NULL argument");
   HB_CHECK_ARG(b->share_obs && b->value_preds && b->returns && b->rows >= 0, "incomplete batch");
+  HB_CHECK_ARG(!b->share_obs_images || !b->index, "share_obs_images need an identity batch");
+  HB_CHECK_ARG((reinterpret_cast<uintptr_t>(b->share_obs_images) & 15) == 0, "share_obs_images must be 16-byte aligned");
   ParamLayout P;
   PrepLayout Q;
   hb_net_layout L;
@@ -473,6 +499,7 @@
     fz::Args fa;
     memset(&fa, 0, sizeof(fa));
     fa.obs = b->share_obs; fa.index = b->index; fa.rows = b->rows;
+    fa.obs_images = static_cast<const unsigned char*>(b->share_obs_images);
     fa.value_preds = b->value_preds; fa.returns = b->returns; fa.vn_state = vn_state;
     fa.clip = h->clip_param; fa.huber_delta = h->huber_delta; fa.vcoef = h->value_loss_coef;
     fa.use_huber = h->use_huber_loss; fa.use_clipped = h->use_clipped_value_loss;
diff --git a/harl_b200/csrc/fused_args.cuh b/harl_b200/csrc/fused_args.cuh
--- a/harl_b200/csrc/fused_args.cuh
+++ b/harl_b200/csrc/fused_args.cuh
@@ -14,6 +14,7 @@
   const float* log_std; float std_x, std_y;
   const float* obs; const int32_t* index; long long rows;
   int stage_obs;
+  const unsigned char* obs_images;
   const float* actions; const float* avail; const float* old_logp; const float* adv; const float* factor; const float* active;
   const float* value_preds; const float* returns; const float* vn_state;
   float clip, entropy_coef, huber_delta, vcoef;
@@ -54,6 +55,8 @@
 inline int fused_max_slots() { return 148; }
 int launch_fused_update(const hb_net_desc* d, const PrepLayout& Q, const ParamLayout& P, const float* prepared, fz::Args a, int mode,
                         int* grid_out, cudaStream_t st);
+size_t fused_obs_images_bytes(long long rows, int K0p);
+int launch_obs_images(const float* obs, long long rows, int in_dim, int K0p, unsigned char* out, cudaStream_t st);
 int launch_fused_finish(const hb_net_desc* d, const ParamLayout& P, const float* params, float* grad, const float* part, int slots,
                         long long stride, const double* norm3, double host_scale, cudaStream_t st);
 
diff --git a/harl_b200/csrc/fused_update.cu b/harl_b200/csrc/fused_update.cu
--- a/harl_b200/csrc/fused_update.cu
+++ b/harl_b200/csrc/fused_update.cu
@@ -215,6 +215,45 @@
   }
 }
 
+__device__ __forceinline__ void featnorm_stats(const float* o, bool ld, int in_dim, float& mean, float& rs) {
+  float s = 0.f;
+  for (int k0 = 0; k0 < in_dim; k0 += 16) {
+    float x[16];
+#pragma unroll
+    for (int j = 0; j < 16; ++j) x[j] = (ld && k0 + j < in_dim) ? o[k0 + j] : 0.f;
+#pragma unroll
+    for (int j = 0; j < 16; ++j) s += x[j];
+  }
+  mean = s / (float)in_dim;
+  float qv = 0.f;
+  for (int k0 = 0; k0 < in_dim; k0 += 16) {
+    float x[16];
+#pragma unroll
+    for (int j = 0; j < 16; ++j) x[j] = (ld && k0 + j < in_dim) ? o[k0 + j] : 0.f;
+#pragma unroll
+    for (int j = 0; j < 16; ++j) { const float d = x[j] - mean; qv = k0 + j < in_dim ? fmaf(d, d, qv) : qv; }
+  }
+  rs = rsqrtf(qv / (float)in_dim + 1e-5f);
+}
+__device__ __forceinline__ void featnorm_write(const float* o, bool ld, int in_dim, int K0p, float mean, float rs, int r,
+                                               unsigned char* img, uint32_t img_bytes) {
+  const float rsx = rs * XS;
+  for (int k0 = 0; k0 < K0p; k0 += 16) {
+    float x[16];
+#pragma unroll
+    for (int j = 0; j < 16; ++j) x[j] = (ld && k0 + j < in_dim) ? (o[k0 + j] - mean) * rsx : 0.f;
+#pragma unroll
+    for (int c = 0; c < 2; ++c) {
+      const float xc[8] = {x[c * 8], x[c * 8 + 1], x[c * 8 + 2], x[c * 8 + 3], x[c * 8 + 4], x[c * 8 + 5], x[c * 8 + 6], x[c * 8 + 7]};
+      uint4 hi, lo;
+      um::split8(xc, hi, lo);
+      const uint32_t off = img_off(r, (k0 >> 3) + c, K0p >> 3);
+      *reinterpret_cast<uint4*>(img + off) = hi;
+      *reinterpret_cast<uint4*>(img + img_bytes + off) = lo;
+    }
+  }
+}
+
 __device__ __forceinline__ float huber_v(float e, float d, int use_huber, float* de) {
   if (!use_huber) { *de = e; return e * e / 2.f; }
   const float ae = fabsf(e);
@@ -264,7 +303,7 @@
   float* sacc = reinterpret_cast<float*>(p); p += 2 * NH * 4;
   double* sred = reinterpret_cast<double*>(p); p += 4 * 4 * 8;
   float* xch = reinterpret_cast<float*>(p); p += 2 * TILE * 2 * 4;
-  uint64_t* bars = reinterpret_cast<uint64_t*>(p); p += 12 * 8;
+  uint64_t* bars = reinterpret_cast<uint64_t*>(p); p += 14 * 8;
   unsigned long long* sclk = reinterpret_cast<unsigned long long*>(p); p += 16 * 8;
   uint32_t* tmem_slot = reinterpret_cast<uint32_t*>(p);
   uint64_t* w_full = bars;
@@ -275,8 +314,12 @@
   uint64_t* obs_full = e2m + 3;
   uint64_t* e2m_h = e2m + 4;
   uint64_t* m2e_b = e2m + 5;
+  uint64_t* x0_free = e2m + 6;
+  uint64_t* x0_full = e2m + 7;
   unsigned char* OBS = MODE == M_GRAD ? X2 : X1;
-  const uint32_t obs_bytes = (uint32_t)TILE * (uint32_t)a.in_dim * 4u;
+  const bool use_img = a.obs_images != nullptr;
+  const uint32_t obs_bytes = use_img ? 2u * x0_bytes : (uint32_t)TILE * (uint32_t)a.in_dim * 4u;
+  const bool hand = MODE == M_GRAD && use_img;
   const int aw = HEAD == HB_HEAD_BOX ? a.out : 1;
   uint32_t so = obs_bytes, o_act = 0, o_old = 0, o_adv = 0, o_fac = 0, o_w = 0, o_av = 0, o_vp = 0, o_ret = 0;
   if (HEAD != HB_HEAD_VALUE) {
@@ -329,6 +372,8 @@
     um::mbar_init(m2e, 1);
     um::mbar_init(obs_free, 1);
     um::mbar_init(obs_full, 1);
+    um::mbar_init(x0_free, 1);
+    um::mbar_init(x0_full, 1);
     um::fence_mbarrier_init();
   }
   if (warp == 0) um::tmem_alloc(tmem_slot, TMEM_COLS);
@@ -342,10 +387,14 @@
   if (warp == 0) {
     if (lane == 0) {
       uint32_t it = 0, tl_ = 0;
-      auto staged = [&](long long t) { return a.stage_obs && t < ntiles && (t + 1) * TILE <= a.rows; };
+      auto inputs_staged = [&](long long t) { return a.stage_obs && (t + 1) * TILE <= a.rows; };
+      auto staged = [&](long long t) { return t < ntiles && (use_img || inputs_staged(t)); };
       auto load_obs = [&](long long t) {
-        um::mbar_expect_tx(obs_full, stage_bytes);
-        um::tma_bulk_g2s(OBS, a.obs + t * TILE * a.in_dim, obs_bytes, obs_full);
+        const bool sc = inputs_staged(t);
+        um::mbar_expect_tx(obs_full, sc ? stage_bytes : obs_bytes);
+        if (use_img) um::tma_bulk_g2s(OBS, a.obs_images + t * (long long)obs_bytes, obs_bytes, obs_full);
+        else um::tma_bulk_g2s(OBS, a.obs + t * TILE * a.in_dim, obs_bytes, obs_full);
+        if (!sc) return;
         const long long r0 = t * TILE;
         if (o_act) um::tma_bulk_g2s(OBS + o_act, a.actions + r0 * aw, TILE * aw * 4, obs_full);
         if (o_old) um::tma_bulk_g2s(OBS + o_old, a.old_logp + r0 * aw, TILE * aw * 4, obs_full);
@@ -371,6 +420,11 @@
             um::mbar_expect_tx(&w_full[st], bytes);
             um::tma_bulk_g2s(ring + st * STAGE_BYTES, src + (size_t)c * (2u * H * 32u * 2u), bytes, &w_full[st]);
           }
+          if (hand && pass == 1) {
+            if (tl_ > 0) um::mbar_wait(x0_free, (tl_ - 1) & 1);
+            um::mbar_expect_tx(x0_full, obs_bytes);
+            um::tma_bulk_g2s(X0, a.obs_images + t * (long long)obs_bytes, obs_bytes, x0_full);
+          }
         }
         um::mbar_wait(obs_free, tl_ & 1);
         if (staged(t + gridDim.x)) load_obs(t + gridDim.x);
@@ -379,7 +433,7 @@
     __syncwarp();
   } else if (warp == 1) {
     if (lane == 0) {
-      uint32_t it = 0, pe = 0, peh = 0;
+      uint32_t it = 0, pe = 0, peh = 0, pimg = 0, px0 = 0;
       bool first = true;
       const uint32_t X0a = um::smem_u32(X0), X1a = um::smem_u32(X1), X2a = um::smem_u32(X2), DLa = um::smem_u32(DL);
       const uint32_t ONa = um::smem_u32(ONES), WHa = um::smem_u32(WH), RGa = um::smem_u32(ring);
@@ -394,15 +448,24 @@
           um::commit(&w_empty[st]);
           ++it;
         };
-        wait_e();
-        for (int c = 0; c < a.nch0; ++c) {
-          const int kc = K0p - 32 * c < 32 ? K0p - 32 * c : 32;
-          chunk(kc, [&](uint32_t wb, uint32_t wimg) {
-            gemm3(tmem + C_F, op_kmajor(X0a, x0_bytes, wch0, 4 * c), op_kmajor(wb, wimg, kc >> 3, 0), kc >> 4,
-                  um::idesc_f16(H, 0, 0), c > 0);
-          });
-        }
-        um::commit(m2e);
+        auto z0 = [&]() {
+          const uint32_t Z0a = use_img ? (GRAD ? X2a : X1a) : X0a;
+          if (use_img) { um::mbar_wait(obs_full, pimg); pimg ^= 1; }
+          for (int c = 0; c < a.nch0; ++c) {
+            const int kc = K0p - 32 * c < 32 ? K0p - 32 * c : 32;
+            chunk(kc, [&](uint32_t wb, uint32_t wimg) {
+              gemm3(tmem + C_F, op_kmajor(Z0a, x0_bytes, wch0, 4 * c), op_kmajor(wb, wimg, kc >> 3, 0), kc >> 4,
+                    um::idesc_f16(H, 0, 0), c > 0);
+            });
+          }
+          um::commit(m2e);
+        };
+        if (!hand) {
+          wait_e();
+          z0();
+        } else if (first) {
+          z0();
+        }
         wait_eh();
         if (nch1 == 4) {
           auto l1 = [&](int c, bool acc) {
@@ -462,12 +525,17 @@
           um::commit(m2e_b);
           um::commit(obs_free);
           wait_e();
+          if (hand) { um::mbar_wait(x0_full, px0); px0 ^= 1; um::tc_fence_after(); }
           gemm3(tmem + C_W0, op_mnmajor(X1a, x_bytes, wchx, 0), op_mnmajor(X0a, x0_bytes, wch0, 0), TILE >> 4,
                 um::idesc_f16(K0p, 1, 1), !first);
           gemm3(tmem + C_B0, op_mnmajor(X1a, x_bytes, wchx, 0), op_mnmajor(ONa, dl_bytes, wchd, 0), TILE >> 4,
                 um::idesc_f16(NH, 1, 1), !first, false);
+          first = false;
+          if (hand) {
+            um::commit(x0_free);
+            if (t + gridDim.x < ntiles) { z0(); continue; }
+          }
           um::commit(m2e);
-          first = false;
         }
       }
     }
@@ -541,7 +609,7 @@
         const long long tn = t + gridDim.x;
         const long long rown = tn * TILE + r;
         if (!a.stage_obs && a.index == nullptr && rown < a.rows && half == 0) {
-          if (!a.stage_obs) {
+          if (!use_img) {
             const float* on = a.obs + rown * a.in_dim;
             um::prefetch_l2(on);
             um::prefetch_l2(on + a.in_dim - 1);
@@ -562,49 +630,20 @@
           if (HEAD == HB_HEAD_BOX) { um::prefetch_l2(a.actions + rown * a.out); if (GRAD) um::prefetch_l2(a.old_logp + rown * a.out); }
         }
       }
-      const float* o = st_obs ? stg + r * a.in_dim : a.obs + src * a.in_dim;
-      float mean = 0.f, rs = 0.f;
-      if (half == 0) {
-        float s = 0.f;
-        for (int k0 = 0; k0 < a.in_dim; k0 += 16) {
-          float x[16];
-#pragma unroll
-          for (int j = 0; j < 16; ++j) x[j] = (ld && k0 + j < a.in_dim) ? o[k0 + j] : 0.f;
-#pragma unroll
-          for (int j = 0; j < 16; ++j) s += x[j];
-        }
-        mean = s / (float)a.in_dim;
-        float qv = 0.f;
-        for (int k0 = 0; k0 < a.in_dim; k0 += 16) {
-          float x[16];
-#pragma unroll
-          for (int j = 0; j < 16; ++j) x[j] = (ld && k0 + j < a.in_dim) ? o[k0 + j] : 0.f;
-#pragma unroll
-          for (int j = 0; j < 16; ++j) { const float d = x[j] - mean; qv = k0 + j < a.in_dim ? fmaf(d, d, qv) : qv; }
-        }
-        rs = rsqrtf(qv / (float)a.in_dim + 1e-5f);
-      }
-      pc.lap(0);
-      if (pending) { wait_m(); pending = false; }
-      pc.lap(1);
-      const float rsx = rs * XS;
-      if (half == 0) {
-        for (int k0 = 0; k0 < K0p; k0 += 16) {
-          float x[16];
-#pragma unroll
-          for (int j = 0; j < 16; ++j) x[j] = (ld && k0 + j < a.in_dim) ? (o[k0 + j] - mean) * rsx : 0.f;
-#pragma unroll
-          for (int c = 0; c < 2; ++c) {
-            const float xc[8] = {x[c * 8], x[c * 8 + 1], x[c * 8 + 2], x[c * 8 + 3], x[c * 8 + 4], x[c * 8 + 5], x[c * 8 + 6], x[c * 8 + 7]};
-            uint4 hi, lo;
-            um::split8(xc, hi, lo);
-            const uint32_t off = img_off(r, (k0 >> 3) + c, wch0);
-            *reinterpret_cast<uint4*>(X0 + off) = hi;
-            *reinterpret_cast<uint4*>(X0 + x0_bytes + off) = lo;
-          }
-        }
-      }
-      signal();
+      if (use_img) {
+        pc.lap(0);
+        if (hand) pending = false;
+        pc.lap(1);
+      } else {
+        const float* o = st_obs ? stg + r * a.in_dim : a.obs + src * a.in_dim;
+        float mean = 0.f, rs = 0.f;
+        if (half == 0) featnorm_stats(o, ld, a.in_dim, mean, rs);
+        pc.lap(0);
+        if (pending) { wait_m(); pending = false; }
+        pc.lap(1);
+        if (half == 0) featnorm_write(o, ld, a.in_dim, K0p, mean, rs, r, X0, x0_bytes);
+      }
+      if (!hand) signal();
       pc.lap(2);
       float mu0, rstd0, mu1, rstd1;
       uint32_t mask0[2] = {0, 0}, mask1[2] = {0, 0};
@@ -973,41 +1012,10 @@
       for (int j = 0; j < NH; ++j) avm |= (j < na && av[j < na ? j : 0] != 0.f) ? (1u << j) : 0u;
     }
     const float* o = st_obs ? stg + r * N.in_dim : N.obs + (ok ? row : 0) * N.in_dim;
-    float mean = 0.f, rs = 0.f;
     if (half == 0) {
-      float s = 0.f;
-      for (int k0 = 0; k0 < N.in_dim; k0 += 16) {
-        float x[16];
-#pragma unroll
-        for (int j = 0; j < 16; ++j) x[j] = (ld && k0 + j < N.in_dim) ? o[k0 + j] : 0.f;
-#pragma unroll
-        for (int j = 0; j < 16; ++j) s += x[j];
-      }
-      mean = s / (float)N.in_dim;
-      float qv = 0.f;
-      for (int k0 = 0; k0 < N.in_dim; k0 += 16) {
-        float x[16];
-#pragma unroll
-        for (int j = 0; j < 16; ++j) x[j] = (ld && k0 + j < N.in_dim) ? o[k0 + j] : 0.f;
-#pragma unroll
-        for (int j = 0; j < 16; ++j) { const float d = x[j] - mean; qv = k0 + j < N.in_dim ? fmaf(d, d, qv) : qv; }
-      }
-      rs = rsqrtf(qv / (float)N.in_dim + 1e-5f);
-      const float rsx = rs * XS;
-      for (int k0 = 0; k0 < K0p; k0 += 16) {
-        float x[16];
-#pragma unroll
-        for (int j = 0; j < 16; ++j) x[j] = (ld && k0 + j < N.in_dim) ? (o[k0 + j] - mean) * rsx : 0.f;
-#pragma unroll
-        for (int c = 0; c < 2; ++c) {
-          const float xc[8] = {x[c * 8], x[c * 8 + 1], x[c * 8 + 2], x[c * 8 + 3], x[c * 8 + 4], x[c * 8 + 5], x[c * 8 + 6], x[c * 8 + 7]};
-          uint4 hi, lo;
-          um::split8(xc, hi, lo);
-          const uint32_t off = img_off(r, (k0 >> 3) + c, wch0);
-          *reinterpret_cast<uint4*>(X0 + off) = hi;
-          *reinterpret_cast<uint4*>(X0 + x0_bytes + off) = lo;
-        }
-      }
+      float mean, rs;
+      featnorm_stats(o, ld, N.in_dim, mean, rs);
+      featnorm_write(o, ld, N.in_dim, K0p, mean, rs, r, X0, x0_bytes);
     }
     signal();
     float mu0, rstd0, mu1, rstd1;
@@ -1062,6 +1070,18 @@
   um::tc_fence_before();
   __syncthreads();
   if (warp == 0) um::tmem_dealloc(tmem, ACT_TMEM_COLS);
+}
+
+__global__ void __launch_bounds__(TILE) obs_images_kernel(const float* __restrict__ obs, long long rows, int in_dim, int K0p,
+                                                          unsigned char* __restrict__ out) {
+  const int r = threadIdx.x;
+  const long long row = (long long)blockIdx.x * TILE + r;
+  const bool ld = row < rows;
+  const float* o = obs + (ld ? row : 0) * in_dim;
+  const uint32_t img_bytes = (uint32_t)TILE * (uint32_t)K0p * 2u;
+  float mean, rs;
+  featnorm_stats(o, ld, in_dim, mean, rs);
+  featnorm_write(o, ld, in_dim, K0p, mean, rs, r, out + (size_t)blockIdx.x * 2u * img_bytes, img_bytes);
 }
 
 struct PackJob {
@@ -1294,10 +1314,22 @@
   return HB_OK;
 }
 
+size_t fused_obs_images_bytes(long long rows, int K0p) {
+  return (size_t)((rows + fz::TILE - 1) / fz::TILE) * 2u * fz::TILE * (size_t)K0p * 2u;
+}
+
+int launch_obs_images(const float* obs, long long rows, int in_dim, int K0p, unsigned char* out, cudaStream_t st) {
+  const long long ntiles = (rows + fz::TILE - 1) / fz::TILE;
+  if (ntiles == 0) return HB_OK;
+  fz::obs_images_kernel<<<(unsigned)ntiles, fz::TILE, 0, st>>>(obs, rows, in_dim, K0p, out);
+  HB_LAUNCH_DONE(st, "obs_images");
+  return HB_OK;
+}
+
 size_t fused_smem_bytes(int H, int K0p) {
   size_t b = 2 * (size_t)fz::TILE * K0p * 2 + 2 * 2 * (size_t)fz::TILE * 128 * 2 + 3 * (size_t)fz::TILE * fz::NH * 2 +
              2 * (size_t)fz::NH * H * 2 + (size_t)(K0p <= 32 ? 3 : 2) * fz::STAGE_BYTES;
-  b += 2 * 128 * 4 + fz::NH * 4 + 4 * fz::NH * 4 + 2 * fz::NH * 4 + 16 * 8 + 2 * fz::TILE * 2 * 4 + 10 * 8 + 16 * 8 + 16;
+  b += 2 * 128 * 4 + fz::NH * 4 + 4 * fz::NH * 4 + 2 * fz::NH * 4 + 16 * 8 + 2 * fz::TILE * 2 * 4 + 14 * 8 + 16 * 8 + 16;
   return b + 1024;
 }
 
diff --git a/harl_b200/nets.py b/harl_b200/nets.py
--- a/harl_b200/nets.py
+++ b/harl_b200/nets.py
@@ -194,23 +194,38 @@
         L.call("hb_value_forward", C.byref(self.desc), L.ptr(self.prepared), L.ptr(cent_obs), rows,
                L.ptr(values_out), L.ptr(ws), n, L.stream_ptr())
 
+    def obs_images(self, obs, out=None):
+        self._need_cuda()
+        rows = obs.shape[0]
+        if not L.lib.hb_get_fused_update() or self.recurrent:
+            return None
+        n = L.lib.hb_obs_images_bytes(C.byref(self.desc), int(rows))
+        if n == 0:
+            return None
+        if out is None or out.numel() < n:
+            out = torch.empty(n, dtype=torch.uint8, device=self.device)
+        L.call("hb_obs_images", C.byref(self.desc), L.ptr(obs), int(rows), L.ptr(out), L.stream_ptr())
+        return out
+
     @staticmethod
     def actor_batch(obs, actions, old_logp=None, adv=None, factor=None, active=None, avail=None, index=None, rows=None,
-                    rnn_states=None, masks=None, seq_len=0):
+                    rnn_states=None, masks=None, seq_len=0, obs_images=None):
         b = L.ActorBatch()
         b.obs, b.actions, b.old_logp, b.adv = L.ptr(obs), L.ptr(actions), L.ptr(old_logp), L.ptr(adv)
         b.factor, b.active, b.avail, b.index = L.ptr(factor), L.ptr(active), L.ptr(avail), L.ptr(index)
         b.rows = int(rows if rows is not None else (index.shape[0] if index is not None else actions.shape[0]))
         b.rnn_states, b.masks, b.seq_len = L.ptr(rnn_states), L.ptr(masks), int(seq_len)
-        b._keep = (obs, actions, old_logp, adv, factor, active, avail, index, rnn_states, masks)
+        b.obs_images = L.ptr(obs_images)
+        b._keep = (obs, actions, old_logp, adv, factor, active, avail, index, rnn_states, masks, obs_images)
         return b
 
     @staticmethod
-    def critic_batch(share_obs, value_preds, returns, index=None, rows=None, rnn_states=None, masks=None, seq_len=0):
+    def critic_batch(share_obs, value_preds, returns, index=None, rows=None, rnn_states=None, masks=None, seq_len=0,
+                     obs_images=None):
         b = L.CriticBatch(L.ptr(share_obs), L.ptr(value_preds), L.ptr(returns), L.ptr(index),
                           int(rows if rows is not None else (index.shape[0] if index is not None else value_preds.numel())),
-                          L.ptr(rnn_states), L.ptr(masks), int(seq_len))
-        b._keep = (share_obs, value_preds, returns, index, rnn_states, masks)
+                          L.ptr(rnn_states), L.ptr(masks), int(seq_len), L.ptr(obs_images))
+        b._keep = (share_obs, value_preds, returns, index, rnn_states, masks, obs_images)
         return b
 
     def evaluate(self, batch, logp_out=None, logp_ref=None, factor_inout=None, agg_prod=True):
diff --git a/harl_b200/runners/on_policy_ha_runner.py b/harl_b200/runners/on_policy_ha_runner.py
--- a/harl_b200/runners/on_policy_ha_runner.py
+++ b/harl_b200/runners/on_policy_ha_runner.py
@@ -85,17 +85,21 @@
                    L.stream_ptr())
         dist.all_reduce_sum_(adv_m3)
         n_active = adv_m3[:, 2].cpu().numpy()
-        for agent_id in agent_order:
+        img_buf = None
+        for pos, agent_id in enumerate(agent_order):
             buf, actor = self.actor_buffer[agent_id], self.actor[agent_id]
             buf.update_factor(factor)
             fl = lambda a: a.reshape(rows, *a.shape[2:])
             avail = None if buf.available_actions is None else fl(buf.available_actions[:-1])
             if actor.recurrent:
+                imgs = None
                 sweep = DeviceNet.actor_batch(fl(buf.obs[:-1]), fl(buf.actions), avail=avail,
                                               rnn_states=buf.rnn_states.reshape((T + 1) * N, -1),
                                               masks=buf.masks.reshape((T + 1) * N), seq_len=T)
             else:
-                sweep = DeviceNet.actor_batch(fl(buf.obs[:-1]), fl(buf.actions), avail=avail)
+                imgs = actor.actor.obs_images(fl(buf.obs[:-1]), img_buf) if getattr(actor, "first_epoch_logp", False) else None
+                img_buf = imgs if imgs is not None else img_buf
+                sweep = DeviceNet.actor_batch(fl(buf.obs[:-1]), fl(buf.actions), avail=avail, obs_images=imgs)
             old_logp = torch.empty(rows, actor.actor.act_width, dtype=torch.float32, device=dev)
             adv_a = advantages if self.state_type == "EP" else advantages[:, :, agent_id].contiguous()
             fuse = (getattr(actor, "first_epoch_logp", False) and not actor.recurrent and getattr(actor, "actor_num_mini_batch", 0) == 1
@@ -106,11 +110,15 @@
                 actor.actor.evaluate(sweep, logp_out=old_logp)
                 if ch is not None:
                     after_actor_big()
-                infos.append(actor.train(buf, adv_a, self.state_type, moments=(adv_m3[agent_id], float(n_active[agent_id]))))
+                kw = {} if imgs is None else dict(obs_images=imgs)
+                infos.append(actor.train(buf, adv_a, self.state_type, moments=(adv_m3[agent_id], float(n_active[agent_id])),
+                                         **kw))
             else:
                 infos.append(actor.train(buf, adv_a, self.state_type, moments=(adv_m3[agent_id], float(n_active[agent_id])),
-                                         old_logp_out=old_logp))
+                                         old_logp_out=old_logp, obs_images=imgs))
                 assert actor.old_logp_filled
+            if pos == len(agent_order) - 1:
+                break
             if ch is not None:
                 before_actor_big()
             actor.actor.evaluate(sweep, logp_ref=old_logp, factor_inout=factor.reshape(rows), agg_prod=agg_prod)
diff --git a/include/harl_b200.h b/include/harl_b200.h
--- a/include/harl_b200.h
+++ b/include/harl_b200.h
@@ -183,7 +183,11 @@
   const float* rnn_states;
   const float* masks;
   int64_t seq_len;
+  const void* obs_images;
 } hb_actor_batch;
+
+size_t hb_obs_images_bytes(const hb_net_desc* d, int64_t rows);
+int hb_obs_images(const hb_net_desc* d, const float* obs, int64_t rows, void* out, void* stream);
 
 int hb_policy_evaluate(const hb_net_desc* d, const float* prepared, const hb_actor_batch* b,
                        float* logp_out, const float* logp_ref, float* factor_inout,
@@ -214,6 +218,7 @@
   const float* rnn_states;
   const float* masks;
   int64_t seq_len;
+  const void* share_obs_images;
 } hb_critic_batch;
 
 int hb_value_grad(const hb_net_desc* d, const float* params, const float* prepared,
diff --git a/profiles/fused_phase_clock.py b/profiles/fused_phase_clock.py
--- a/profiles/fused_phase_clock.py
+++ b/profiles/fused_phase_clock.py
@@ -10,40 +10,62 @@
 from harl_b200.nets import DeviceNet
 from harl_b200.utils.configs_tools import get_defaults_yaml_args
 
+import argparse
+
+ap = argparse.ArgumentParser()
+ap.add_argument("--net", default="actor", choices=["actor", "critic"],
+                help="actor: Discrete head, in_dim 18 (fused_actor_update); critic: value head, in_dim 54 (fused_critic_update)")
+opt = ap.parse_args()
 algo_args, _ = get_defaults_yaml_args("happo", "pettingzoo_mpe")
 cfg = {**algo_args["model"], **algo_args["algo"]}
 dev = torch.device("cuda:0")
 torch.manual_seed(0)
-net = DeviceNet(cfg, 18, L.HEAD_DISCRETE, 5, dev)
 R = 819200
 g = torch.Generator().manual_seed(1)
-obs = torch.randn(R, 18, generator=g).to(dev)
-acts = torch.randint(0, 5, (R, 1), generator=g).float().to(dev)
-old = (-1.6 + 0.1 * torch.randn(R, 1, generator=g)).to(dev)
-adv = torch.randn(R, generator=g).to(dev)
-fac, active, avail = torch.ones(R, device=dev), torch.ones(R, device=dev), torch.ones(R, 5, device=dev)
-batch = DeviceNet.actor_batch(obs, acts, old, adv, fac, active, avail)
-hyper = L.PPOHyper(0.2, 0.01, 1, 1, 1)
-norm3 = torch.tensor([0, 0, float(R)], dtype=torch.float64, device=dev)
 scal = torch.zeros(4, dtype=torch.float64, device=dev)
-for _ in range(3):
-    net.actor_grad(batch, hyper, norm3, scal)
-torch.cuda.synchronize()
-L.call("hb_fused_timing_enable", 1)
-e0, e1 = torch.cuda.Event(enable_timing=True), torch.cuda.Event(enable_timing=True)
-e0.record()
-net.actor_grad(batch, hyper, norm3, scal)
-e1.record()
-torch.cuda.synchronize()
-tab = np.zeros((148, 16), np.uint64)
-L.call("hb_fused_timing_read", tab.ctypes.data_as(C.c_void_p))
-L.call("hb_fused_timing_enable", 0)
-names = ["inputs+featnorm stats", "wait prev-tile bwd MMAs", "write X0", "wait L0 MMA", "L0 fwd epilogue", "wait L1 MMA",
+if opt.net == "actor":
+    net = DeviceNet(cfg, 18, L.HEAD_DISCRETE, 5, dev)
+    obs = torch.randn(R, 18, generator=g).to(dev)
+    acts = torch.randint(0, 5, (R, 1), generator=g).float().to(dev)
+    old = (-1.6 + 0.1 * torch.randn(R, 1, generator=g)).to(dev)
+    adv = torch.randn(R, generator=g).to(dev)
+    fac, active, avail = torch.ones(R, device=dev), torch.ones(R, device=dev), torch.ones(R, 5, device=dev)
+    hyper = L.PPOHyper(0.2, 0.01, 1, 1, 1)
+    norm3 = torch.tensor([0, 0, float(R)], dtype=torch.float64, device=dev)
+
+    def step(images):
+        batch = DeviceNet.actor_batch(obs, acts, old, adv, fac, active, avail, obs_images=images)
+        net.actor_grad(batch, hyper, norm3, scal)
+else:
+    net = DeviceNet(cfg, 54, L.HEAD_VALUE, 1, dev)
+    obs = torch.randn(R, 54, generator=g).to(dev)
+    vp, ret = torch.randn(R, generator=g).to(dev), torch.randn(R, generator=g).to(dev)
+    hyper = L.ValueHyper(0.2, 10.0, 1.0, 1, 1)
+
+    def step(images):
+        net.value_grad(DeviceNet.critic_batch(obs, vp, ret, obs_images=images), hyper, None, 1.0 / R, scal)
+
+label = "fused_actor_update" if opt.net == "actor" else "fused_critic_update"
+names = ["inputs (+ featnorm stats)", "wait prev-tile bwd MMAs", "write / copy X0", "wait L0 MMA", "L0 fwd epilogue", "wait L1 MMA",
          "L1 fwd epilogue", "wait head MMA", "head epilogue", "wait head-bwd MMA", "L1 bwd epilogue", "wait L1-bwd MMAs",
          "L0 bwd epilogue"]
 tiles = R / 128 / 148
-m = tab.astype(np.float64).mean(0)
-print(f"fused_actor_update {e0.elapsed_time(e1) * 1e3:.1f} us for {R} rows; {tiles:.1f} tiles per CTA; cycles per tile (mean over CTAs):")
-for i, n in enumerate(names):
-    print(f"  {i:2d} {n:28s} {m[i] / tiles:9.0f}")
-print(f"     {'sum':28s} {m[:13].sum() / tiles:9.0f}")
+for title, images in (("in-kernel feature norm", None), ("pre-normalised images", net.obs_images(obs))):
+    for _ in range(3):
+        step(images)
+    torch.cuda.synchronize()
+    L.call("hb_fused_timing_enable", 1)
+    e0, e1 = torch.cuda.Event(enable_timing=True), torch.cuda.Event(enable_timing=True)
+    e0.record()
+    step(images)
+    e1.record()
+    torch.cuda.synchronize()
+    tab = np.zeros((148, 16), np.uint64)
+    L.call("hb_fused_timing_read", tab.ctypes.data_as(C.c_void_p))
+    L.call("hb_fused_timing_enable", 0)
+    m = tab.astype(np.float64).mean(0)
+    print(f"{label} ({title}) {e0.elapsed_time(e1) * 1e3:.1f} us for {R} rows; {tiles:.1f} tiles per CTA; cycles per tile "
+          "(mean over CTAs):")
+    for i, n in enumerate(names):
+        print(f"  {i:2d} {n:28s} {m[i] / tiles:9.0f}")
+    print(f"     {'sum':28s} {m[:13].sum() / tiles:9.0f}")
```
